# roitberg-group/lammps-ani

Hardware: AMD Instinct MI355X
Metric: MD ns/day for ANI-2x water box (0.5 fs steps; whole timestep loop: integrate + re-neighbour + ghost exchange + pair_style ani hot path) (higher is better)
Workload: dtype f32

## Files before the change

### include/ani_hip.h

```cpp
#ifndef ANI_HIP_H
#define ANI_HIP_H

#include <stdint.h>

#ifdef __cplusplus
extern "C" {
#endif

typedef struct ani_handle ani_handle;

#define ANI_HARTREE2KCALMOL 627.5094738898777

#define ANI_OK 0
#define ANI_ERR_ARG 1
#define ANI_ERR_MODEL 2
#define ANI_ERR_DEVICE 3
#define ANI_ERR_CAPACITY 4

int ani_create(const char* model_file, int local_rank, int use_num_models, int use_cuaev, int use_fullnbr,
               int use_single, ani_handle** out);

void ani_destroy(ani_handle* h);

const char* ani_last_error(const ani_handle* h);

int ani_num_models(const ani_handle* h);
int ani_use_num_models(const ani_handle* h);
int ani_num_species(const ani_handle* h);
int ani_aev_length(const ani_handle* h);
double ani_cutoff_radial(const ani_handle* h);
double ani_cutoff_angular(const ani_handle* h);

int ani_compute_full(ani_handle* h, int ntotal, int nlocal, const int64_t* species, const double* coordinates,
                     int64_t npairs, const int* ilist_unique, const int* jlist, const int* numneigh, int ago,
                     int eflag_atom, int vflag, double* out_energy, double* out_force, double* out_atomic_energies,
                     double* out_virial);

int ani_compute_half(ani_handle* h, int ntotal, int nlocal, const int64_t* species, const double* coordinates,
                     int64_t npairs_half, const int64_t* atom_index12, int ago, int eflag_atom, int vflag,
                     double* out_energy, double* out_force, double* out_atomic_energies, double* out_virial);

int ani_compute_full_device(ani_handle* h, int ntotal, int nlocal, const int* d_species, const double* d_x,
                            int64_t npairs, const int* d_ilist, const int* d_jlist, const int* d_numneigh, int ago,
                            int eflag_atom, int vflag, double* d_f, double* d_ev, double* d_eatom, void* stream);

int ani_request_atom_virial(ani_handle* h, double* out, int ncomp);

int ani_request_model_deviation(ani_handle* h, double* member_energy, double* atom_energy_dev, double* member_dforce,
                                double* atom_force_dev, double* summary);

int ani_set_ghost_fold(ani_handle* h, const int64_t* d_owner, const double* d_shift, int nghost, void* stream);
int ani_stage_ghost_fold(ani_handle* h, const int64_t* d_owner, const double* d_shift, int nghost);

int ani_step_begin(ani_handle* h, int ntotal, int nlocal, const double* d_x, int eflag_atom, int vflag, double* d_f, double* d_ev,
                   double* d_eatom, void* stream);
int ani_step_ghosts_ready(ani_handle* h, void* stream);
int ani_step_finish(ani_handle* h, void* stream);

int ani_build_list_device(ani_handle* h, int ntotal, int nlocal, const int* d_species, const double* d_x, double cutneigh,
                          const double* lo, const double* hi, int64_t* out_npairs, void* stream);

int ani_build_list(ani_handle* h, int ntotal, int nlocal, const int64_t* species, const double* coordinates, double cutneigh,
                   const double* lo, const double* hi, int64_t* out_npairs);
int ani_debug_list(ani_handle* h, const int** d_numneigh, const int** d_nbr_off, const int** d_jlist);

int ani_set_bond_table(ani_handle* h, const double* cut, int nspecies);
int ani_find_molecules_device(ani_handle* h, int ntotal, int nlocal, const double* d_x, const int64_t* d_owner, int* d_mol_of_atom,
                              int* d_formula, int formula_cap, int64_t* d_summary, void* stream);
int ani_find_molecules(ani_handle* h, int ntotal, int nlocal, const double* coordinates, const int64_t* owner, int* mol_of_atom,
                       int* formula, int formula_cap, int64_t* summary);
const char* ani_species_symbol(const ani_handle* h, int s);

int ani_rdf_configure(ani_handle* h, int nbins, double rmax, const int* pairs , int npair);
int ani_rdf_accumulate_device(ani_handle* h, int ntotal, int nlocal, const double* d_x, void* stream);
int ani_rdf_accumulate(ani_handle* h, int ntotal, int nlocal, const double* coordinates);
int ani_rdf_read(ani_handle* h, uint64_t* counts , uint64_t* centres , uint64_t* frames, int reset);

int ani_attach_comm(ani_handle* h, void* comm);

typedef struct {
  int nlocal, ntotal, nrows;
  int64_t npairs;
  const float* d_aev;
  const float* d_gaev;
  const int* d_row_of_centre;
  int species_count[16];
  int aev_stride;
  int aev_active_length;
  int error_flags;
} ani_debug_view;
int ani_host_register(const void* p, size_t bytes);
int ani_host_unregister(const void* p);

const char* ani_last_mlp_kernel(const ani_handle* h);
int ani_debug_get(ani_handle* h, ani_debug_view* out);
int ani_debug_colmap(ani_handle* h, int* out);
int ani_debug_deviation_parts(ani_handle* h, const void** d_parts, int64_t* member_stride);

int ani_set_option(ani_handle* h, const char* name, int value);
void ani_trace_push(const char* name);
void ani_trace_pop(void);
void ani_trace_mark(const char* name);

int ani_debug_fused_stamps(unsigned long long* out16, int reset);

int ani_debug_fused_schedule(int ntypes, const int* count, const double* cost, int bins, int* items_out, int* off_out,
                             double* makespan_out);
int ani_debug_fused_schedule_halves(int ntypes, const int* count, const double* cost, double half_ratio, int bins, int split_mode,
                                    int* split_out, int* items_out, int* off_out, int* n_items_out, double* makespan_out);

int ani_debug_read(ani_handle* h, const void* d_src, void* host_dst, uint64_t bytes);

int ani_phase_timing(ani_handle* h, int enable);
int ani_phase_times(ani_handle* h, double* ms5, int* ncalls);

#ifdef __cplusplus
}
#endif
#endif
```

### lammps-ani_amd/ani_hip.py

```python
from __future__ import annotations

import ctypes as C
import os
import subprocess

import numpy as np

_HERE = os.path.dirname(os.path.abspath(__file__))
_CSRC = os.path.join(_HERE, "csrc")
LIB_PATH = os.environ.get("ANI_HIP_LIB") or os.path.join(_CSRC, "libani_hip.so")
HARTREE2KCALMOL = 627.5094738898777

EXPORTS = ["ani_create", "ani_destroy", "ani_last_error", "ani_num_models", "ani_use_num_models", "ani_num_species",
           "ani_aev_length", "ani_cutoff_radial", "ani_cutoff_angular", "ani_compute_full", "ani_compute_half",
           "ani_compute_full_device", "ani_build_list_device", "ani_build_list", "ani_debug_list", "ani_debug_get", "ani_debug_read", "ani_debug_colmap", "ani_set_option", "ani_phase_timing", "ani_phase_times",
           "ani_trace_push", "ani_trace_pop", "ani_trace_mark", "ani_step_begin", "ani_step_ghosts_ready", "ani_step_finish",
           "ani_debug_fused_stamps", "ani_attach_comm", "ani_debug_fused_schedule", "ani_debug_fused_schedule_halves", "ani_last_mlp_kernel", "ani_host_register", "ani_host_unregister", "ani_set_ghost_fold", "ani_stage_ghost_fold",
           "ani_request_atom_virial", "ani_request_model_deviation", "ani_debug_deviation_parts",
           "ani_set_bond_table", "ani_find_molecules_device", "ani_find_molecules", "ani_species_symbol",
           "ani_rdf_configure", "ani_rdf_accumulate_device", "ani_rdf_accumulate", "ani_rdf_read"]
COMM_EXPORTS = ["ani_comm_get_unique_id", "ani_comm_create", "ani_comm_create_local", "ani_comm_destroy", "ani_comm_last_error", "ani_comm_rank",
                "ani_comm_size", "ani_comm_plan", "ani_comm_exchange_counts", "ani_comm_alltoallv", "ani_comm_set_epoch",
                "ani_comm_set_epoch_host", "ani_comm_set_ghost_order", "ani_comm_forward", "ani_comm_reverse", "ani_comm_reverse_send", "ani_comm_reverse_unpack",
                "ani_comm_allreduce_f64", "ani_comm_set_option", "ani_comm_get_stat"]


class AniError(RuntimeError):
    pass


class DebugView(C.Structure):
    _fields_ = [("nlocal", C.c_int), ("ntotal", C.c_int), ("nrows", C.c_int), ("npairs", C.c_int64),
                ("d_aev", C.c_void_p), ("d_gaev", C.c_void_p), ("d_row_of_centre", C.c_void_p),
                ("species_count", C.c_int * 16), ("aev_stride", C.c_int), ("aev_active_length", C.c_int), ("error_flags", C.c_int)]


class FireParams(C.Structure):
    _fields_ = [(n, C.c_double) for n in ("dt0", "dtmax", "dtmin", "dtgrow", "dtshrink", "alpha0", "alphashrink", "dmax", "etol",
                                          "ftol")] + [(n, C.c_int) for n in ("delaystep", "initialdelay", "halfstepback", "maxiter")]


FIRE_NSTATE = 16
FIRE_STATE_KEYS = ("iterations", "dt", "alpha", "last_negative", "e_prev", "e_cur", "P", "vv", "ff", "dtv", "uphill", "limited", "stop",
                   "e_first", "ff_first", "vmax")
FIRE_STOP_REASONS = ("running", "etol", "ftol", "maxiter", "non-finite")
SHAKE_NSTATS = 4
SHAKE_STATS_KEYS = ("unconverged", "max_iterations", "max_residual", "calls")
NH_NSTATE = 32
NH_MAXCHAIN = 8
NH_STATE_KEYS = ("half_steps", "k2", "s", "t_target", "ecouple", "tdof", "nonfinite")
THERMO_N = 16
THERMO_KEYS = ("pe", "ke", "temp", "press", "pxx", "pyy", "pzz", "pxy", "pxz", "pyz", "etotal", "ecouple", "econserve", "vol", "k2")


class NhParams(C.Structure):
    _fields_ = [("dt", C.c_double), ("t_period", C.c_double), ("drag", C.c_double), ("mtchain", C.c_int), ("nc_tchain", C.c_int)]


def nh_state_dict(rec, mtchain: int = NH_MAXCHAIN) -> dict:
    rec = np.asarray(rec, dtype=np.float64)
    out = dict(zip(NH_STATE_KEYS, rec[:7].tolist()))
    for k, name in enumerate(("eta", "eta_dot", "eta_dotdot")):
        out[name] = rec[8 + 8 * k: 8 + 8 * k + mtchain].copy()
    return out


NPT_NSTATE = 56
NPT_STATE_KEYS = ("half_steps", "omega_dot", "omega", "press", "p_target", "W", "fv", "mu")


class NptParams(C.Structure):
    _fields_ = [("dt", C.c_double), ("t_period", C.c_double), ("drag", C.c_double), ("p_period", C.c_double), ("mtchain", C.c_int),
                ("nc_tchain", C.c_int), ("mpchain", C.c_int), ("nc_pchain", C.c_int)]


def npt_state_dict(rec, mpchain: int = NH_MAXCHAIN) -> dict:
    rec = np.asarray(rec, dtype=np.float64)
    out = dict(zip(NPT_STATE_KEYS, rec[:8].tolist()))
    out.update(lo=rec[8:11].copy(), len=rec[11:14].copy(), ratio=rec[14:17].copy(), c=rec[17:20].copy(), v0=float(rec[20]),
               ecouple=float(rec[21]), nonfinite=float(rec[22]), natoms=float(rec[23]), ecouple_chain=float(rec[48]), vol=float(rec[49]))
    for k, name in enumerate(("eta", "eta_dot", "eta_dotdot")):
        out[name] = rec[24 + 8 * k: 24 + 8 * k + mpchain].copy()
    return out


RESTRAINT_NREC = 16
RESTRAINT_KINDS = {"distance": (0, 2), "angle": (1, 3), "torsion": (2, 4)}


def restraint_gather_table(atoms):
    atoms = np.asarray(atoms, dtype=np.int64).reshape(-1, 4)
    words = np.flatnonzero(atoms.reshape(-1) >= 0)
    owner = atoms.reshape(-1)[words]
    order = np.argsort(owner, kind="stable")
    touched, counts = np.unique(owner, return_counts=True)
    row_ptr = np.concatenate([[0], np.cumsum(counts)])
    return touched.astype(np.int32), row_ptr.astype(np.int32), words[order].astype(np.int32)


def restraint_state_dict(rec) -> dict:
    rec = np.asarray(rec, dtype=np.float64)
    return dict(evaluations=int(rec[0]), ebias=float(rec[1]), virial=rec[2:11].reshape(3, 3).copy(), nonfinite=int(rec[11]),
                max_delta=float(rec[12]), skipped=int(rec[13]))


def fire_params(dt0, etol, ftol, maxiter, **kw) -> FireParams:
    vals = dict(dt0=float(dt0), dtmax=10.0 * dt0, dtmin=0.02 * dt0, dtgrow=1.1, dtshrink=0.5, alpha0=0.25, alphashrink=0.99,
                dmax=0.1, etol=float(etol), ftol=float(ftol), delaystep=20, initialdelay=1, halfstepback=1, maxiter=int(maxiter))
    unknown = set(kw) - set(vals)
    if unknown:
        raise TypeError(f"unknown FIRE parameter(s): {sorted(unknown)}")
    vals.update(kw)
    p = FireParams()
    for name, ctype in FireParams._fields_:
        setattr(p, name, int(vals[name]) if ctype is C.c_int else float(vals[name]))
    return p


def build(force: bool = False) -> str:
    args = ["make", "-C", _CSRC, "-j8"]
    if force:
        args.append("-B")
    out = subprocess.run(args, check=True, stdout=subprocess.PIPE, stderr=subprocess.STDOUT, text=True).stdout
    build.last_commands = [ln for ln in out.splitlines() if ln.lstrip().startswith(("hipcc", "g++", "gcc"))]
    return LIB_PATH


build.last_commands = []


_lib = None


def lib():
    global _lib
    if _lib is None:
        if not os.path.exists(LIB_PATH):
            raise AniError(f"{LIB_PATH} is missing: build it (python -c 'import __graft_entry__ as g; g.build()'); "
                           "there is no fallback path")
        L = C.CDLL(LIB_PATH)
        L.ani_create.argtypes = [C.c_char_p, C.c_int, C.c_int, C.c_int, C.c_int, C.c_int, C.POINTER(C.c_void_p)]
        L.ani_destroy.argtypes = [C.c_void_p]
        L.ani_last_error.restype = C.c_char_p
        L.ani_last_error.argtypes = [C.c_void_p]
        for n in ("ani_num_models", "ani_use_num_models", "ani_num_species", "ani_aev_length"):
            getattr(L, n).argtypes = [C.c_void_p]
        for n in ("ani_cutoff_radial", "ani_cutoff_angular"):
            getattr(L, n).argtypes = [C.c_void_p]
            getattr(L, n).restype = C.c_double
        L.ani_compute_full.argtypes = [C.c_void_p, C.c_int, C.c_int, C.c_void_p, C.c_void_p, C.c_int64, C.c_void_p,
                                       C.c_void_p, C.c_void_p, C.c_int, C.c_int, C.c_int] + [C.c_void_p] * 4
        L.ani_compute_half.argtypes = [C.c_void_p, C.c_int, C.c_int, C.c_void_p, C.c_void_p, C.c_int64, C.c_void_p,
                                       C.c_int, C.c_int, C.c_int] + [C.c_void_p] * 4
        L.ani_compute_full_device.argtypes = [C.c_void_p, C.c_int, C.c_int, C.c_void_p, C.c_void_p, C.c_int64,
                                              C.c_void_p, C.c_void_p, C.c_void_p, C.c_int, C.c_int, C.c_int,
                                              C.c_void_p, C.c_void_p, C.c_void_p, C.c_void_p]
        L.ani_step_begin.argtypes = [C.c_void_p, C.c_int, C.c_int, C.c_void_p, C.c_int, C.c_int, C.c_void_p, C.c_void_p, C.c_void_p,
                                     C.c_void_p]
        L.ani_step_ghosts_ready.argtypes = [C.c_void_p, C.c_void_p]
        L.ani_step_finish.argtypes = [C.c_void_p, C.c_void_p]
        L.ani_build_list_device.argtypes = [C.c_void_p, C.c_int, C.c_int, C.c_void_p, C.c_void_p, C.c_double,
                                            C.c_void_p, C.c_void_p, C.POINTER(C.c_int64), C.c_void_p]
        L.ani_build_list.argtypes = [C.c_void_p, C.c_int, C.c_int, C.c_void_p, C.c_void_p, C.c_double, C.c_void_p,
                                     C.c_void_p, C.POINTER(C.c_int64)]
        L.ani_debug_list.argtypes = [C.c_void_p] + [C.POINTER(C.c_void_p)] * 3
        L.ani_debug_get.argtypes = [C.c_void_p, C.POINTER(DebugView)]
        L.ani_debug_read.argtypes = [C.c_void_p, C.c_void_p, C.c_void_p, C.c_uint64]
        L.ani_debug_colmap.argtypes = [C.c_void_p, C.c_void_p]
        L.ani_set_option.argtypes = [C.c_void_p, C.c_char_p, C.c_int]
        L.ani_last_mlp_kernel.argtypes = [C.c_void_p]
        L.ani_set_ghost_fold.argtypes = [C.c_void_p, C.c_void_p, C.c_void_p, C.c_int, C.c_void_p]
        L.ani_stage_ghost_fold.argtypes = [C.c_void_p, C.c_void_p, C.c_void_p, C.c_int]
        L.ani_request_atom_virial.argtypes = [C.c_void_p, C.c_void_p, C.c_int]
        L.ani_request_model_deviation.argtypes = [C.c_void_p] + [C.c_void_p] * 5
        L.ani_debug_deviation_parts.argtypes = [C.c_void_p, C.POINTER(C.c_void_p), C.POINTER(C.c_int64)]
        L.ani_set_bond_table.argtypes = [C.c_void_p, C.c_void_p, C.c_int]
        L.ani_find_molecules_device.argtypes = [C.c_void_p, C.c_int, C.c_int, C.c_void_p, C.c_void_p, C.c_void_p, C.c_void_p, C.c_int,
                                                C.c_void_p, C.c_void_p]
        L.ani_find_molecules.argtypes = [C.c_void_p, C.c_int, C.c_int, C.c_void_p, C.c_void_p, C.c_void_p, C.c_void_p, C.c_int,
                                         C.c_void_p]
        L.ani_species_symbol.argtypes = [C.c_void_p, C.c_int]
        L.ani_species_symbol.restype = C.c_char_p
        L.ani_rdf_configure.argtypes = [C.c_void_p, C.c_int, C.c_double, C.c_void_p, C.c_int]
        L.ani_rdf_accumulate_device.argtypes = [C.c_void_p, C.c_int, C.c_int, C.c_void_p, C.c_void_p]
        L.ani_rdf_accumulate.argtypes = [C.c_void_p, C.c_int, C.c_int, C.c_void_p]
        L.ani_rdf_read.argtypes = [C.c_void_p, C.c_void_p, C.c_void_p, C.c_void_p, C.c_int]
        L.ani_host_register.argtypes = [C.c_void_p, C.c_size_t]
        L.ani_host_unregister.argtypes = [C.c_void_p]
        L.ani_last_mlp_kernel.restype = C.c_char_p
        L.ani_md_initial_integrate.argtypes = [C.c_void_p, C.c_void_p, C.c_void_p, C.c_void_p, C.c_double, C.c_int, C.c_void_p,
                                               C.c_void_p, C.c_void_p]
        L.ani_md_final_integrate.argtypes = [C.c_void_p, C.c_void_p, C.c_void_p, C.c_int, C.c_int, C.c_void_p, C.c_void_p,
                                             C.c_void_p, C.c_uint64, C.c_uint64, C.c_void_p]
        L.ani_md_final_initial_integrate.argtypes = [C.c_void_p, C.c_void_p, C.c_void_p, C.c_void_p, C.c_double, C.c_int, C.c_int,
                                                     C.c_void_p, C.c_void_p, C.c_void_p, C.c_uint64, C.c_uint64, C.c_void_p,
                                                     C.c_void_p, C.c_void_p]
        L.ani_md_wrap_positions.argtypes = [C.c_void_p, C.c_int, C.c_void_p, C.c_void_p, C.c_int, C.c_void_p]
        L.ani_md_ghost_shell_count.argtypes = [C.c_void_p, C.c_int, C.c_void_p, C.c_void_p, C.c_int, C.c_void_p, C.c_void_p, C.c_void_p,
                                               C.c_void_p]
        L.ani_md_ghost_shell_fill.argtypes = [C.c_void_p, C.c_int, C.c_void_p, C.c_void_p, C.c_void_p, C.c_int, C.c_void_p, C.c_void_p,
                                              C.c_void_p, C.c_void_p]
        L.ani_md_append_ghosts.argtypes = [C.c_void_p, C.c_void_p, C.c_int, C.c_void_p, C.c_void_p, C.c_int, C.c_void_p]
        L.ani_md_check.argtypes = [C.c_void_p, C.c_void_p, C.c_void_p, C.c_void_p]
        L.ani_md_forward_ghosts.argtypes = [C.c_void_p, C.c_void_p, C.c_void_p, C.c_int, C.c_int, C.c_void_p]
        L.ani_md_reverse_ghosts.argtypes = [C.c_void_p, C.c_void_p, C.c_int, C.c_int, C.c_void_p]
        L.ani_md_reverse_ghosts_ordered.argtypes = [C.c_void_p, C.c_void_p, C.c_void_p, C.c_int, C.c_int, C.c_void_p]
        L.ani_md_pack_ghosts.argtypes = [C.c_void_p, C.c_void_p, C.c_void_p, C.c_int, C.c_void_p, C.c_void_p]
        L.ani_md_unpack_reverse.argtypes = [C.c_void_p, C.c_void_p, C.c_int, C.c_void_p, C.c_void_p]
        L.ani_md_fire_work_size.argtypes = [C.c_int]
        L.ani_md_fire_init.argtypes = [C.c_void_p, C.c_void_p, C.c_int, C.POINTER(FireParams), C.c_void_p]
        L.ani_md_fire_iterate.argtypes = [C.c_void_p, C.c_void_p, C.c_void_p, C.c_void_p, C.c_int, C.c_void_p, C.POINTER(FireParams),
                                          C.c_void_p, C.c_void_p, C.c_void_p, C.c_void_p, C.c_void_p]
        L.ani_md_fire_check.argtypes = [C.c_void_p, C.c_void_p, C.c_void_p, C.c_void_p, C.c_void_p]
        L.ani_md_shake_positions.argtypes = [C.c_void_p, C.c_void_p, C.c_void_p, C.c_void_p, C.c_int, C.c_void_p, C.c_double,
                                             C.c_double, C.c_int, C.c_void_p, C.c_int, C.c_void_p, C.c_void_p, C.c_void_p, C.c_void_p]
        L.ani_md_rattle_velocities.argtypes = [C.c_void_p, C.c_void_p, C.c_void_p, C.c_void_p, C.c_int, C.c_void_p, C.c_void_p,
                                               C.c_int, C.c_void_p]
        L.ani_md_nh_work_size.argtypes = [C.c_int]
        L.ani_md_nh_init.argtypes = [C.c_void_p, C.c_void_p]
        L.ani_md_nh_kinetic.argtypes = [C.c_void_p, C.c_void_p, C.c_int, C.c_void_p, C.c_void_p]
        L.ani_md_nh_chain.argtypes = [C.c_void_p, C.c_void_p, C.c_int, C.c_double, C.c_double, C.POINTER(NhParams), C.c_void_p]
        L.ani_md_nh_scale.argtypes = [C.c_void_p, C.c_int, C.c_void_p, C.c_void_p]
        L.ani_md_nh_initial_integrate.argtypes = [C.c_void_p, C.c_void_p, C.c_void_p, C.c_void_p, C.c_double, C.c_int, C.c_void_p,
                                                  C.c_void_p, C.c_void_p, C.c_void_p]
        L.ani_md_nh_final_integrate.argtypes = [C.c_void_p, C.c_void_p, C.c_void_p, C.c_void_p, C.c_int, C.c_void_p, C.c_void_p]
        L.ani_md_thermo_work_size.argtypes = [C.c_int]
        L.ani_md_thermo.argtypes = [C.c_void_p, C.c_void_p, C.c_int, C.c_void_p, C.c_int, C.c_double, C.c_double, C.c_void_p,
                                    C.c_void_p, C.c_void_p, C.c_void_p]
        L.ani_md_npt_init.argtypes = [C.c_void_p, C.c_void_p, C.c_void_p, C.c_int, C.c_void_p]
        L.ani_md_npt_chain.argtypes = [C.c_int, C.c_void_p, C.c_void_p, C.c_void_p, C.c_int, C.c_void_p, C.c_double, C.c_double,
                                       C.c_double, C.POINTER(NptParams), C.c_void_p]
        L.ani_md_npt_initial_integrate.argtypes = [C.c_void_p, C.c_void_p, C.c_void_p, C.c_void_p, C.c_double, C.c_int, C.c_void_p,
                                                   C.c_void_p, C.c_void_p, C.c_void_p, C.c_void_p, C.c_int, C.c_void_p]
        L.ani_md_npt_final_integrate.argtypes = [C.c_void_p, C.c_void_p, C.c_void_p, C.c_void_p, C.c_int, C.c_void_p, C.c_void_p,
                                                 C.c_void_p]
        L.ani_md_npt_check.argtypes = [C.c_void_p, C.c_void_p, C.c_void_p, C.c_void_p, C.c_void_p]
        L.ani_md_restraints_eval.argtypes = [C.c_void_p, C.c_int, C.c_void_p, C.c_void_p, C.c_void_p, C.c_void_p, C.c_int, C.c_void_p,
                                             C.c_void_p, C.c_int, C.c_void_p, C.c_void_p, C.c_void_p, C.c_void_p, C.c_void_p]
        L.ani_md_restraints_apply.argtypes = [C.c_void_p, C.c_int, C.c_void_p, C.c_int, C.c_void_p, C.c_void_p, C.c_void_p, C.c_int,
                                              C.c_void_p, C.c_void_p, C.c_void_p, C.c_void_p, C.c_void_p, C.c_void_p, C.c_int,
                                              C.c_void_p, C.c_double, C.c_void_p, C.c_void_p]
        L.ani_comm_get_unique_id.argtypes = [C.c_void_p]
        L.ani_comm_create.argtypes = [C.c_int, C.c_int, C.c_void_p, C.c_int, C.POINTER(C.c_void_p)]
        L.ani_comm_destroy.argtypes = [C.c_void_p]
        L.ani_comm_last_error.restype = C.c_char_p
        L.ani_comm_last_error.argtypes = [C.c_void_p]
        L.ani_comm_rank.argtypes = [C.c_void_p]
        L.ani_comm_size.argtypes = [C.c_void_p]
        L.ani_comm_plan.argtypes = [C.c_int] + [C.c_void_p] * 6
        L.ani_comm_exchange_counts.argtypes = [C.c_void_p] * 4
        L.ani_comm_alltoallv.argtypes = [C.c_void_p] * 5 + [C.c_int, C.c_void_p]
# ... 135 lines not shown
                                            f.ctypes.data, ea.ctypes.data, vir.ctypes.data)
        else:
            il = np.ascontiguousarray(inp.ilist, dtype=np.int32)
            nn = np.ascontiguousarray(inp.numneigh, dtype=np.int32)
            jl = np.ascontiguousarray(inp.jlist, dtype=np.int32)
            rc = self._lib.ani_compute_full(self._h, nt, nl, species.ctypes.data, x.ctypes.data, inp.npairs,
                                            il.ctypes.data, jl.ctypes.data, nn.ctypes.data, ago, int(eflag_atom),
                                            int(vflag), e.ctypes.data, f.ctypes.data, ea.ctypes.data, vir.ctypes.data)
        self._check(rc)
        out = dict(energy=float(e[0]), force=f, eatom=ea, virial=vir.reshape(3, 3))
        if av is not None:
            out["atom_virial"] = av
        if dv is not None:
            out["deviation"] = dv
        return out

    def compute_device(self, ntotal, nlocal, d_species, d_x, npairs, d_ilist, d_jlist, d_numneigh, ago, d_f, d_ev,
                       d_eatom=None, eflag_atom=False, vflag=False, stream=None, d_atom_virial=None, ncomp=9, d_deviation=None):
        if d_atom_virial is not None:
            self.request_atom_virial(d_atom_virial, ncomp)
        if d_deviation is not None:
            self.request_model_deviation(**d_deviation)
        rc = self._lib.ani_compute_full_device(self._h, ntotal, nlocal, d_species, d_x, npairs, d_ilist, d_jlist,
                                               d_numneigh, ago, int(eflag_atom), int(vflag), d_f, d_ev, d_eatom, stream)
        self._check(rc)

    def step_begin(self, ntotal, nlocal, d_x, d_f, d_ev, d_eatom=None, eflag_atom=False, vflag=False, stream=None,
                   d_atom_virial=None, ncomp=9):
        if d_atom_virial is not None:
            self.request_atom_virial(d_atom_virial, ncomp)
        self._check(self._lib.ani_step_begin(self._h, ntotal, nlocal, d_x, int(eflag_atom), int(vflag), d_f, d_ev, d_eatom, stream))

    def step_ghosts_ready(self, stream=None):
        self._check(self._lib.ani_step_ghosts_ready(self._h, stream))

    def step_finish(self, stream=None):
        self._check(self._lib.ani_step_finish(self._h, stream))

    def build_list_device(self, ntotal, nlocal, d_species, d_x, cutneigh, lo, hi, stream=None) -> int:
        lo = np.ascontiguousarray(lo, dtype=np.float64)
        hi = np.ascontiguousarray(hi, dtype=np.float64)
        n = C.c_int64()
        self._check(self._lib.ani_build_list_device(self._h, ntotal, nlocal, d_species, d_x, float(cutneigh),
                                                    lo.ctypes.data, hi.ctypes.data, C.byref(n), stream))
        return n.value

    def build_list(self, species, x, nlocal: int, cutneigh: float, lo=None, hi=None) -> int:
        species = np.ascontiguousarray(species, dtype=np.int64)
        x = np.ascontiguousarray(x, dtype=np.float64)
        if lo is None:
            lo = [x[:, k].min() - 0.25 for k in range(3)]
        if hi is None:
            hi = [x[:, k].max() + 0.25 for k in range(3)]
        lo = np.ascontiguousarray(lo, dtype=np.float64)
        hi = np.ascontiguousarray(hi, dtype=np.float64)
        n = C.c_int64()
        self._check(self._lib.ani_build_list(self._h, x.shape[0], nlocal, species.ctypes.data, x.ctypes.data, float(cutneigh),
                                             lo.ctypes.data, hi.ctypes.data, C.byref(n)))
        return n.value

    def debug_list(self, nlocal: int):
        pn, po, pj = C.c_void_p(), C.c_void_p(), C.c_void_p()
        self._check(self._lib.ani_debug_list(self._h, C.byref(pn), C.byref(po), C.byref(pj)))
        nn = self.debug_read(pn, (nlocal,), np.int32)
        if nlocal == 0:
            return nn, np.zeros(0, np.int32)
        off = self.debug_read(po, (nlocal + 1,), np.int32)
        span = self.debug_read(pj, (int((off[:-1] + nn).max()),), np.int32)
        if np.array_equal(off[1:] - off[:-1], nn):
            return nn, span[: int(nn.sum())]
        idx = np.repeat(off[:-1] - np.concatenate([[0], np.cumsum(nn)[:-1]]), nn) + np.arange(int(nn.sum()))
        return nn, span[idx]

    def debug_view(self) -> DebugView:
        v = DebugView()
        self._check(self._lib.ani_debug_get(self._h, C.byref(v)))
        return v

    def debug_read(self, d_ptr, shape, dtype) -> np.ndarray:
        out = np.empty(shape, dtype=dtype)
        self._check(self._lib.ani_debug_read(self._h, d_ptr, out.ctypes.data, out.nbytes))
        return out

    def colmap(self) -> np.ndarray:
        v = self.debug_view()
        out = np.zeros(v.aev_active_length, dtype=np.int32)
        self._check(self._lib.ani_debug_colmap(self._h, out.ctypes.data))
        return out

    def set_option(self, name: str, value: int):
        self._check(self._lib.ani_set_option(self._h, name.encode(), int(value)))

    def set_ghost_fold(self, d_owner, d_shift, nghost: int, stream=None):
        self._check(self._lib.ani_set_ghost_fold(self._h, d_owner, d_shift, int(nghost), stream))

    def stage_ghost_fold(self, d_owner, d_shift, nghost: int):
        self._check(self._lib.ani_stage_ghost_fold(self._h, d_owner, d_shift, int(nghost)))

    def species_symbols(self):
        return [self._lib.ani_species_symbol(self._h, s).decode() for s in range(self._lib.ani_num_species(self._h))]

    def set_bond_table(self, table):
        if table is None:
            self._check(self._lib.ani_set_bond_table(self._h, None, 0))
            return
        if isinstance(table, dict):
            sym = self.species_symbols()
            t = np.zeros((len(sym), len(sym)))
            for (a, b), v in table.items():
                if a not in sym or b not in sym:
                    raise AniError(f"set_bond_table: the model has no species {a if a not in sym else b!r} (it has {sym})")
                t[sym.index(a), sym.index(b)] = t[sym.index(b), sym.index(a)] = float(v)
            table = t
        t = np.ascontiguousarray(table, dtype=np.float64)
        if t.ndim != 2 or t.shape[0] != t.shape[1]:
            raise AniError(f"set_bond_table: a square table is needed, got shape {t.shape}")
        self._check(self._lib.ani_set_bond_table(self._h, t.ctypes.data, int(t.shape[0])))

    def find_molecules(self, inp_or_x, owner=None, formula_cap: int = 4096, nlocal=None):
        if hasattr(inp_or_x, "nlocal"):
            x, nl = inp_or_x.x, inp_or_x.nlocal
        else:
            x = inp_or_x
            nl = len(x) if nlocal is None else int(nlocal)
        x = np.ascontiguousarray(x, dtype=np.float64)
        nt = x.shape[0]
        S = self._lib.ani_num_species(self._h)
        own = None
        if owner is not None:
            own = np.ascontiguousarray(owner, dtype=np.int64)
            assert own.shape == (nt - nl,)
        mol = np.full(nl, -1, dtype=np.int32)
        rows = np.zeros((int(formula_cap), S + 1), dtype=np.int32)
        summ = np.zeros(6, dtype=np.int64)
        self._check(self._lib.ani_find_molecules(self._h, nt, nl, x.ctypes.data, own.ctypes.data if own is not None else None,
                                                 mol.ctypes.data, rows.ctypes.data, int(formula_cap), summ.ctypes.data))
        return mol, formula_dict(rows[: int(summ[1])], self.species_symbols()), summ

    def find_molecules_device(self, ntotal, nlocal, d_x, d_owner=None, d_mol_of_atom=None, d_formula=None, formula_cap: int = 0,
                              d_summary=None, stream=None):
        self._check(self._lib.ani_find_molecules_device(self._h, int(ntotal), int(nlocal), d_x, d_owner, d_mol_of_atom, d_formula,
                                                        int(formula_cap), d_summary, stream))

    def rdf_configure(self, nbins: int, rmax: float, pairs):
        if pairs is None or len(pairs) == 0:
            self._check(self._lib.ani_rdf_configure(self._h, int(nbins), float(rmax), None, 0))
            self._rdf = None
            return
        sym = None
        idx = []
        for pr in pairs:
            a, b = pr
            for v in (a, b):
                if isinstance(v, str):
                    sym = sym or self.species_symbols()
                    if v not in sym:
                        raise AniError(f"rdf_configure: the model has no species {v!r} (it has {sym})")
                    v = sym.index(v)
                idx.append(int(v))
        p = np.ascontiguousarray(idx, dtype=np.int32).reshape(-1, 2)
        self._check(self._lib.ani_rdf_configure(self._h, int(nbins), float(rmax), p.ctypes.data, int(p.shape[0])))
        self._rdf = (int(nbins), float(rmax), p)

    def rdf_config(self):
        return getattr(self, "_rdf", None)

# ... 162 lines not shown
```

### lammps-ani_amd/csrc/ani_handle.h

```cpp
#pragma once
#include "../../include/ani_hip.h"
#include "../../include/ani_comm.h"

#include <hip/hip_runtime.h>
#ifndef ANI_NO_ROCTX
#include <rocprofiler-sdk-roctx/roctx.h>
#else
static inline void roctxRangePushA(const char*) {}
static inline void roctxRangePop() {}
static inline void roctxMarkA(const char*) {}
#endif

#include <algorithm>
#include <atomic>
#include <chrono>
#include <cmath>
#include <cstdio>
#include <cstdlib>
#include <cstring>
#include <string>
#include <vector>

#include "ani_kernels.h"
#include "ani_model.h"

namespace ani_host __attribute__((visibility("hidden"))) {
using namespace ani;

inline int round_up(int v, int m) { return (v + m - 1) / m * m; }

template <typename T>
struct DevBuf {
  T* p = nullptr;
  size_t cap = 0;
  hipError_t reserve(size_t n, bool zero = false) {
    if (n <= cap && p) return hipSuccess;
    if (p) (void)hipFree(p);
    p = nullptr;
    size_t want = std::max<size_t>(n + n / 2, 64);
    hipError_t e = hipMalloc((void**)&p, want * sizeof(T));
    if (e != hipSuccess) { cap = 0; return e; }
    cap = want;
    if (zero) {
      e = hipMemset(p, 0, want * sizeof(T));
      if (e == hipSuccess) e = hipStreamSynchronize(nullptr);
    }
    return e;
  }
  void release() { if (p) (void)hipFree(p); p = nullptr; cap = 0; }
};

struct TraceRange {
  explicit TraceRange(const char* name) { roctxRangePushA(name); }
  ~TraceRange() { roctxRangePop(); }
  TraceRange(const TraceRange&) = delete;
  TraceRange& operator=(const TraceRange&) = delete;
};

struct SpeciesNet {
  std::vector<float*> W;
  std::vector<float*> b;
  std::vector<float*> WT;
  float* W0c = nullptr;
  float* WT0c = nullptr;
  float* w_out = nullptr;
  float* b_out = nullptr;
  std::vector<int> w;
  std::vector<double*> W64, b64, WT64;
  double *W0c64 = nullptr, *WT0c64 = nullptr, *w_out64 = nullptr, *b_out64 = nullptr;
  struct Planes {
    std::vector<unsigned short*> W, WT;
    unsigned short *W0c = nullptr, *WT0c = nullptr;
  } sp[2];
  std::vector<float> wscale;
  struct Fused {
    unsigned char* stream = nullptr;
    float* consts = nullptr;
    long long ppm = 0;
    int cpm = 0;
  } fu[4];
  int fused_shape = -1;
};
inline MlpArith planes_arith(int i) { return i == 0 ? MLP_BF16X3 : MLP_F16X2; }

struct Options {
  int prune = 1;
  int mlp_pipeline = 0;
  int aev_fused = 1;
  int aev_sym_radial = 1;
  int aev_tickets_min = 40000;
  int mlp_fused_sched = 1;
  int mlp_fused_halves = 1;
  int mlp_fused = 1;
  int mlp_fused_gen = 1;
  int mlp_fused_rows = 0;
  int mlp_chain = 1;
  int profiling = 0;
  int dev_overwrite = 0;
  int mlp_arith = MLP_BF16X3;
  int rdf_lanes = 16, rdf_lds = 1;
  int nbr_onepass = 1, nbr_sorted_rows = 1, nbr_half_cells = 0;
  int reuse_upload = 0;
  int out_force_accumulate = 0;
};

struct FusedState {
  int mask[4] = {-2, -2, -2, -2};
  DevBuf<int> counter;
  DevBuf<int> sched;
  int sched_key[4] = {-1, -1, -1, -1};
  int sched_nitems = 0;
  DevBuf<float> gaev_parts;
};

struct DevOut { double *member_energy, *atom_energy_dev, *member_dforce, *atom_force_dev, *summary; };

struct Armed {
  double* av_out = nullptr;
  int av_ncomp = 0;
  void* av_acc = nullptr;
  double* split_av = nullptr;
  int split_av_ncomp = 0;
  DevBuf<float> avir;
  DevBuf<double> avir64;
  DevBuf<double> avout;
  DevOut dv_req{}, dv{};
  bool dv_on = false, dv_force = false, dv_dsq = false, dv_fold = false;
  DevBuf<double> gaev_parts64;
  DevBuf<float> dv_fbuf;
  DevBuf<double> dv_fbuf64;
  DevBuf<double> dv_tmp;
  DevBuf<double> dv_stage;
  DevBuf<double> dv_part;
  DevBuf<unsigned> dv_ticket;
};

struct MolFinder {
  bool have_bonds = false;
  DevBuf<double> bond_cut2;
  DevBuf<int> ints;
  DevBuf<unsigned long long> words;
  DevBuf<long long> owner, summary;
  DevBuf<int> out;
};

struct Rdf {
  int npair = 0, nbins = 0;
  double rmax = 0.0;
  DevBuf<int> ints;
  DevBuf<unsigned long long> words;
};

struct NbrBuild {
  int cap_hint = 0;
  DevBuf<int> ovf;
  DevBuf<float4> xq;
  DevBuf<int> cell_id, cell_count, cell_start, cursor, order;
  DevBuf<double> xs;
};

struct HostStaging {
  std::vector<int> species32;
  double* pinned_ev = nullptr;
  int* pinned_ints = nullptr;
  double* stage_force = nullptr;
  size_t stage_force_cap = 0;
  static constexpr int kForceChunks = 16;
  unsigned* stage_flags = nullptr;
  DevBuf<unsigned long long> copy_ctr;
  unsigned copy_epoch = 0;
  unsigned long long step = 0;
  const double* x64_from = nullptr;
  std::vector<int> half_num, half_j;
};

struct PhaseTiming {
  bool on = false;
  std::vector<hipEvent_t> evt_pool;
  size_t evt_used = 0;
  hipEvent_t* evt = nullptr;
  double phase_ms[5] = {0, 0, 0, 0, 0};
  int phase_calls = 0;
};

}

using namespace ani;
using namespace ani_host;

struct ani_handle {
  HostModel model;
  AevParams ap{};
  AevParams ap_run{};
  SpeciesMap cmap{};
  int active_mask = -1;
  Options opt;
  FusedState fused;
  Armed armed;
  MolFinder mol;
  Rdf rdf;
  NbrBuild nb;
  HostStaging host;
  PhaseTiming timing;
  const char* last_mlp_kernel = "";
  ChainPlan chain_plan;
  std::vector<int> colmap;
  int device = 0;
  bool use_cuaev = true, use_fullnbr = true, use_single = true;
  hipStream_t stream = nullptr;
  std::string err;
  std::vector<SpeciesNet> nets;

  bool have_list = false;
  DevBuf<int> row_flag, row_list, row_count;
  int n_boundary = 0;
  bool classes_valid = false;
  int split_phase = 0;
  hipStream_t side = nullptr;
  hipEvent_t ev_mlp = nullptr, ev_side = nullptr;
  struct { const double* d_x; int eflag_atom, vflag; double *d_f, *d_ev, *d_eatom; } split{};
  int nlocal = 0, ntotal = 0, nrows = 0;
  long long npairs = 0;
  int count[kMaxSpecies] = {0}, row_start[kMaxSpecies] = {0};

  ani_comm* comm = nullptr;
  int sticky_flags = 0;
  int max_numneigh = 0;
  DevBuf<int> species, ilist, numneigh, jlist, jraw, nbr_off, row_of_centre, centre_of_row, bucket_info, err_flag;
  DevBuf<int> row_of_atom;
  DevBuf<unsigned> sym_acc;
  int jraw_stride = 0;
  int jlist_row_stride = 0;
  const int64_t* stage_owner = nullptr;
  const double* stage_shift = nullptr;
  int stage_nghost = -1;
  bool origin_from_box = false;
  GhostFold fold;
  int fold_nghost = -1;
  DevBuf<int> fold_head, fold_next, fold_bad;
  bool warned_asymmetric = false;
  bool list_is_ours = false;
  bool list_symmetric = true;
  DevBuf<int> row_ctr;
  DevBuf<float4> xyzs, cl_xyz;
  DevBuf<int4> row_info, cl_hdr;
  DevBuf<int> cl_j;
  int cl_stride = 0;
  DevBuf<double> x64, f64, ev, eatom, virial_acc;
  DevBuf<double> origin;
  bool need_origin = true;
  DevBuf<double> rep_tables, erep;
  DevBuf<float> aev, gaev, act, e_rows, fbuf;
  DevBuf<double> aev64, gaev64, act64, e_rows64, fbuf64;
  std::vector<std::vector<double*>> Hbuf64;
  std::vector<std::vector<float*>> Hbuf, Gbuf;
  bool arena_valid = false;
};

#define HIP_TRY(h, expr)                                                                              \
  do {                                                                                                \
    hipError_t _e = (expr);                                                                           \
    if (_e != hipSuccess) {                                                                           \
      (h)->err = std::string(#expr) + ": " + hipGetErrorString(_e);                                   \
      return ANI_ERR_DEVICE;                                                                          \
    }                                                                                                 \
  } while (0)

namespace ani_host __attribute__((visibility("hidden"))) {
int check_args(ani_handle* h, int ntotal, int nlocal, long long npairs, int ago);
int upload_model(ani_handle* h);
int specialize(ani_handle* h, int mask);
int compute_mlp(ani_handle* h, hipStream_t st);
void free_fused(ani_handle* h, int fi);
const int* forced_fused_split(const char* env, int ntypes, const int* count, int* split);
int rebuild(ani_handle* h, hipStream_t st);
int ingest_list(ani_handle* h, int ntotal, int nlocal, long long npairs, const int* species, const int* ilist, const int* numneigh,
                const int* jlist, hipMemcpyKind kind, hipStream_t st);
int ensure_row_classes(ani_handle* h, hipStream_t st);
struct DevStage {
  DevOut dev{};
  size_t off[5] = {0, 0, 0, 0, 0}, len[5] = {0, 0, 0, 0, 0};
};
double* take_atom_virial(ani_handle* h, int* ncomp);
int atom_virial_begin(ani_handle* h, bool armed);
void atom_virial_out(ani_handle* h, double* d_out, int ncomp, int accumulate, bool fold, hipStream_t st);
bool dv_any(const DevOut& d);
DevOut take_deviation(ani_handle* h);
int deviation_check(ani_handle* h, const DevOut& d, int ntotal, int nlocal, bool device, bool fold);
int deviation_begin(ani_handle* h, const DevOut& d, bool fold);
void deviation_end(ani_handle* h);
int deviation_stage(ani_handle* h, const DevOut& d, int ntotal, int nlocal, DevStage* sg);
int deviation_copy_home(ani_handle* h, const DevOut& d, const DevStage& sg, hipStream_t st);

template <typename Pass>
int deviation_run(ani_handle* h, Pass&& pass, hipStream_t st) {
  const HostModel& m = h->model;
  const int M = m.M, nl = h->nlocal;
  const bool fp64 = !h->use_single;
  double* dsq = h->armed.dv_dsq ? h->armed.dv_tmp.p : nullptr;
  double* sig = h->armed.dv.summary ? h->armed.dv_tmp.p + (size_t)nl : nullptr;
  double* dd = h->armed.dv.summary ? h->armed.dv_tmp.p + 2 * (size_t)nl : nullptr;
  if (h->armed.dv_force) {
    const long long per = (long long)std::max(h->nrows, 1) * h->ap_run.aev_stride;
    void* acc = fp64 ? static_cast<void*>(h->armed.dv_fbuf64.p) : static_cast<void*>(h->armed.dv_fbuf.p);
    HIP_TRY(h, hipMemsetAsync(acc, 0, (fp64 ? 3 * sizeof(double) : 4 * sizeof(float)) * (size_t)h->ntotal, st));
    const bool fold = h->armed.dv_fold;
    for (int a = 0; a < M; a++) {
      pass(a, per, acc);
      launch_dev_member(acc, fp64, fold ? nl : h->ntotal, nl, a, M, h->armed.dv.member_dforce, dsq, fold ? h->fold_head.p : nullptr,
                        fold ? h->fold_next.p : nullptr, nl, st);
    }
  }
  DevCloseArgs ca{};
  ca.e_rows = fp64 ? static_cast<const void*>(h->e_rows64.p) : static_cast<const void*>(h->e_rows.p);
  ca.M = M; ca.nrows = h->nrows; ca.nrows_ld = h->nrows; ca.nlocal = nl;
  ca.centre_of_row = h->centre_of_row.p; ca.ilist = h->ilist.p; ca.species = h->species.p;
  for (int s = 0; s < m.S; s++) ca.sae[s] = m.sae[s];
  ca.erep = m.has_rep ? h->erep.p : nullptr; ca.nslots = kVirialSlots;
  ca.dsq = dsq;
  ca.member_energy = h->armed.dv.member_energy; ca.atom_energy_dev = h->armed.dv.atom_energy_dev;
  ca.atom_force_dev = dsq ? h->armed.dv.atom_force_dev : nullptr;
  ca.sig = sig; ca.dd = dd;
  ca.partials = h->armed.dv_part.p; ca.ticket = h->armed.dv_ticket.p;
  launch_dev_close(ca, fp64, st);
  if (h->armed.dv.summary) launch_dev_summary(dd, sig, nl, h->armed.dv.summary, st);
  return ANI_OK;
}

template <typename T>
bool wait_host_word(const volatile T* w, T want) {
  const auto t0 = std::chrono::steady_clock::now();
  for (;;) {
    for (int k = 0; k < 512; k++) {
      if (*w == want) {
        std::atomic_thread_fence(std::memory_order_acquire);
        return true;
      }
      __builtin_ia32_pause();
    }
    if (std::chrono::steady_clock::now() - t0 > std::chrono::seconds(5)) return false;
  }
}
}
```

### lammps-ani_amd/csrc/ani_hip.cpp

```cpp
#include "ani_handle.h"

namespace ani {
static thread_local hipError_t g_launch_error = hipSuccess;
void note_launch_error(hipError_t e) { if (e != hipSuccess && g_launch_error == hipSuccess) g_launch_error = e; }
hipError_t take_launch_error() { const hipError_t e = g_launch_error; g_launch_error = hipSuccess; return e; }
}

namespace ani_host __attribute__((visibility("hidden"))) {
thread_local std::string g_create_error;
constexpr int kCopyOutBlocks = 32;

int run_step64(ani_handle* h, const double* d_x, int eflag_atom, int vflag, double* d_f, int f_accumulate, double* d_ev,
               double* d_eatom, hipStream_t st) {
  const HostModel& m = h->model;
  const int L = m.L, M = m.M;
  HIP_TRY(h, h->fbuf64.reserve((size_t)std::max(h->ntotal, 1) * 3));
  HIP_TRY(h, h->virial_acc.reserve(9 * kVirialSlots));
  HIP_TRY(h, h->err_flag.reserve(1, true));
  HIP_TRY(h, hipMemsetAsync(h->fbuf64.p, 0, sizeof(double) * 3 * (size_t)h->ntotal, st));
  HIP_TRY(h, hipMemsetAsync(h->virial_acc.p, 0, sizeof(double) * 9, st));
  HIP_TRY(h, hipMemsetAsync(h->e_rows64.p, 0, sizeof(double) * (size_t)M * std::max(h->nrows, 1), st));
  if (h->armed.av_acc) HIP_TRY(h, hipMemsetAsync(h->armed.av_acc, 0, sizeof(double) * 9 * (size_t)h->ntotal, st));
  Aev64Params p{};
  const AevParams& r = h->ap_run;
// ... 77 lines not shown
    launch_repulsion(ra, true, st, h->armed.av_acc);
  }
  Sae64 sae{};
  for (int s = 0; s < m.S; s++) sae.v[s] = m.sae[s];
  launch_finish64(h->e_rows64.p, M, h->nrows, h->centre_of_row.p, h->ilist.p, h->species.p, sae, h->fbuf64.p, h->ntotal,
                  vflag ? h->virial_acc.p : nullptr, d_f, f_accumulate, d_ev, eflag_atom ? d_eatom : nullptr, h->err_flag.p, st);
  if (m.has_rep) launch_repulsion_energy(h->erep.p, kVirialSlots, d_ev, st);
  if (h->armed.dv_on) {
    Aev64Args ad = a;
    ad.virial = nullptr;
    const int rcd = deviation_run(h, [&](int b, long long stride, void* acc) {
      ad.gaev = h->armed.gaev_parts64.p + b * stride; ad.fbuf = static_cast<double*>(acc);
      launch_aev64_backward(p, ad, st);
    }, st);
    if (rcd) return rcd;
  }
  HIP_TRY(h, hipGetLastError());
  HIP_TRY(h, take_launch_error());
  return ANI_OK;
}

struct StepCtx {
  const double* d_x = nullptr;
  int eflag_atom = 0, vflag = 0, f_accumulate = 0;
  double *d_f = nullptr, *d_ev = nullptr, *d_eatom = nullptr;
  bool fold = false;
};

int step_prologue(ani_handle* h, const StepCtx& c, bool timed, hipStream_t st) {
  if (h->ntotal >= (1 << 28)) {
    h->err = "more than 2^28 atoms (owned + ghost) on one rank";
    return ANI_ERR_ARG;
  }
  HIP_TRY(h, h->xyzs.reserve(h->ntotal));
  HIP_TRY(h, h->fbuf.reserve((size_t)h->ntotal * 4));
  HIP_TRY(h, h->virial_acc.reserve(9 * kVirialSlots));
  HIP_TRY(h, h->err_flag.reserve(1, true));
  HIP_TRY(h, h->row_ctr.reserve((size_t)3 * kTicketMaxGroups * kTicketStride, true));
  h->timing.evt = nullptr;
  if (timed && h->timing.on) {
    if (h->timing.evt_used + 6 > h->timing.evt_pool.size()) {
      const size_t old = h->timing.evt_pool.size();
      h->timing.evt_pool.resize(old + 6 * 64, nullptr);
      for (size_t i = old; i < h->timing.evt_pool.size(); i++) HIP_TRY(h, hipEventCreate(&h->timing.evt_pool[i]));
    }
    h->timing.evt = &h->timing.evt_pool[h->timing.evt_used];
    h->timing.evt_used += 6;
  }
  if (h->timing.evt) HIP_TRY(h, hipEventRecord(h->timing.evt[0], st));
  HIP_TRY(h, h->origin.reserve(3));
  if (h->need_origin) {
    launch_origin(c.d_x, h->ntotal, h->origin.p, st);
    h->need_origin = false;
  }
  if (h->model.has_rep) {
    HIP_TRY(h, h->erep.reserve(kVirialSlots));
    HIP_TRY(h, hipMemsetAsync(h->erep.p, 0, sizeof(double) * kVirialSlots, st));
  }
  return ANI_OK;
}

void step_pack(ani_handle* h, const StepCtx& c, int i0, int i1, bool first, hipStream_t st) {
  const bool fold = h->fold_nghost >= 0 && c.fold;
  launch_pack(c.d_x, h->species.p, i0, i1, h->cmap, h->xyzs.p, h->fbuf.p, first ? h->virial_acc.p : nullptr,
              first ? c.d_ev : nullptr, h->origin.p, st, fold ? &h->fold : nullptr);
}

AevArgs step_aev_args(ani_handle* h, const StepCtx& c, int rows) {
  AevArgs a{};
  a.xyzs = h->xyzs.p; a.ilist = h->ilist.p; a.numneigh = h->numneigh.p; a.nbr_off = h->nbr_off.p; a.jlist = h->jlist.p;
  a.centre_of_row = h->centre_of_row.p; a.row_info = h->row_info.p; a.nrows = h->nrows; a.aev = h->aev.p; a.gaev = h->gaev.p; a.fbuf = h->fbuf.p;
  a.virial = c.vflag ? h->virial_acc.p : nullptr;
  a.err_flag = h->err_flag.p;
  a.cl_hdr = h->cl_hdr.p; a.cl_xyz = h->cl_xyz.p; a.cl_j = h->cl_j.p; a.cl_stride = h->cl_stride;
  a.row_list = nullptr; a.k0 = 0; a.kcount = h->nrows;
  a.row_counter = h->row_ctr.p ? h->row_ctr.p + rows * kTicketMaxGroups * kTicketStride : nullptr;
  if (rows == 1) { a.row_list = h->row_list.p; a.k0 = 0; a.kcount = h->n_boundary; }
  if (rows == 2) { a.row_list = h->row_list.p; a.k0 = h->n_boundary; a.kcount = h->nrows - h->n_boundary; }
  if (a.kcount < h->opt.aev_tickets_min) a.row_counter = nullptr;
  a.row_of_atom = (rows == 0 && h->opt.aev_sym_radial && h->list_symmetric) ? h->row_of_atom.p : nullptr;
  return a;
}

int step_compact_forward(ani_handle* h, const AevArgs& a, hipStream_t st) {
  if (h->opt.aev_fused) {
    TraceRange tr("ani: neighbour compaction + AEV forward");
    if (h->timing.evt) HIP_TRY(h, hipEventRecord(h->timing.evt[5], st));
    if (launch_aev_forward_fused(h->ap_run, a, h->max_numneigh, st)) {
      if (h->timing.evt) HIP_TRY(h, hipEventRecord(h->timing.evt[1], st));
      return ANI_OK;
    }
  }
  {
    TraceRange tr("ani: neighbour compaction");
    launch_nbr_compact(h->ap_run, a, h->max_numneigh, st);
  }
  if (h->timing.evt) HIP_TRY(h, hipEventRecord(h->timing.evt[5], st));
  {
    TraceRange tr("ani: AEV forward");
    launch_aev_forward(h->ap_run, a, h->max_numneigh, st);
  }
  if (h->timing.evt) HIP_TRY(h, hipEventRecord(h->timing.evt[1], st));
  return ANI_OK;
}

int step_backward(ani_handle* h, const StepCtx& c, const AevArgs& a, hipStream_t st) {
  const HostModel& m = h->model;
  RepTab rt{};
  if (m.has_rep && h->ap_run.S <= 8) {
    rt.on = 1; rt.cutoff = (float)m.rep_cut; rt.erep = h->erep.p; rt.x64 = c.d_x;
    std::vector<int> act;
    for (int s = 0; s < m.S; s++) if (h->active_mask & (1 << s)) act.push_back(s);
    if ((int)act.size() != h->ap_run.S) { act.clear(); for (int s = 0; s < m.S; s++) act.push_back(s); }
    const size_t n2 = (size_t)m.S * m.S;
    for (size_t ca = 0; ca < act.size(); ca++)
      for (size_t cb = 0; cb < act.size(); cb++) {
        const size_t src = (size_t)act[ca] * m.S + act[cb];
        rt.y[8 * ca + cb] = (float)m.rep_tables[src];
        rt.sa[8 * ca + cb] = (float)m.rep_tables[n2 + src];
        rt.k[8 * ca + cb] = (float)m.rep_tables[2 * n2 + src];
      }
  }
  float* avir = static_cast<float*>(h->armed.av_acc);
  const bool rep_done = launch_aev_backward(h->ap_run, a, h->max_numneigh, st, rt.on ? &rt : nullptr, avir) && rt.on;
  if (m.has_rep && !rep_done) {
    RepArgs ra{};
    ra.row_info = h->row_info.p; ra.nrows = h->nrows; ra.jlist = h->jlist.p; ra.species = h->species.p;
    ra.pos = c.d_x; ra.fbuf = h->fbuf.p; ra.virial = c.vflag ? h->virial_acc.p : nullptr; ra.erep = h->erep.p;
    ra.tables = h->rep_tables.p; ra.S = m.S; ra.nslots = kVirialSlots; ra.vslots = kVirialSlots; ra.cutoff = m.rep_cut;
    launch_repulsion(ra, false, st, avir);
  }
  return ANI_OK;
}

void step_finish(ani_handle* h, const StepCtx& c, int atom0, int atom1, bool energy, hipStream_t st) {
  const HostModel& m = h->model;
  FinishArgs fa{};
  fa.e_rows = h->e_rows.p; fa.M = m.M; fa.nrows = h->nrows; fa.nrows_ld = h->nrows;
  fa.centre_of_row = h->centre_of_row.p; fa.ilist = h->ilist.p; fa.species = h->species.p;
  for (int s = 0; s < m.S; s++) fa.sae[s] = m.sae[s];
  fa.fbuf = h->fbuf.p; fa.atom0 = atom0; fa.atom1 = atom1; fa.energy = energy ? 1 : 0;
  fa.virial_acc = c.vflag ? h->virial_acc.p : nullptr;
  fa.f_out = c.d_f; fa.f_accumulate = c.f_accumulate; fa.ev_out = c.d_ev;
  fa.eatom_out = c.eflag_atom ? c.d_eatom : nullptr;
  fa.err_flag = h->err_flag.p;
  if (h->fold_nghost >= 0 && c.fold) {
    fa.fold_head = h->fold_head.p; fa.fold_next = h->fold_next.p; fa.fold_nlocal = h->nlocal;
    fa.atom1 = std::min(fa.atom1, h->nlocal);
  }
  launch_finish(fa, st);
  if (energy && m.has_rep) launch_repulsion_energy(h->erep.p, kVirialSlots, c.d_ev, st);
}

int run_step(ani_handle* h, const double* d_x, int eflag_atom, int vflag, double* d_f, int f_accumulate, double* d_ev,
             double* d_eatom, hipStream_t st, bool fold = false) {
  if (!h->use_single) return run_step64(h, d_x, eflag_atom, vflag, d_f, f_accumulate, d_ev, d_eatom, st);
  StepCtx c;
  c.fold = fold;
  c.d_x = d_x; c.eflag_atom = eflag_atom; c.vflag = vflag; c.f_accumulate = f_accumulate; c.d_f = d_f; c.d_ev = d_ev; c.d_eatom = d_eatom;
  TraceRange tr_step("ani: step");
  int rc = step_prologue(h, c, true, st);
  if (rc) return rc;
  step_pack(h, c, 0, h->ntotal, true, st);
  if (h->armed.av_acc) HIP_TRY(h, hipMemsetAsync(h->armed.av_acc, 0, sizeof(float) * 9 * (size_t)h->ntotal, st));
  const AevArgs a = step_aev_args(h, c, 0);
  rc = step_compact_forward(h, a, st);
  if (rc) return rc;
  {
    TraceRange tr("ani: MLP forward + backward");
    rc = compute_mlp(h, st);
    if (rc) return rc;
  }
  if (h->timing.evt) HIP_TRY(h, hipEventRecord(h->timing.evt[2], st));
  TraceRange tr_bwd("ani: AEV backward + finish");
  rc = step_backward(h, c, a, st);
  if (rc) return rc;
  if (h->timing.evt) HIP_TRY(h, hipEventRecord(h->timing.evt[3], st));
  step_finish(h, c, 0, h->ntotal, true, st);
  if (h->timing.evt) HIP_TRY(h, hipEventRecord(h->timing.evt[4], st));
  if (h->armed.dv_on) {
    AevArgs ad = a;
    ad.virial = nullptr;
    rc = deviation_run(h, [&](int b, long long stride, void* acc) {
      ad.gaev = h->fused.gaev_parts.p + b * stride; ad.fbuf = static_cast<float*>(acc);
      launch_aev_backward(h->ap_run, ad, h->max_numneigh, st);
    }, st);
    if (rc) return rc;
  }
  HIP_TRY(h, hipGetLastError());
  HIP_TRY(h, take_launch_error());
  return ANI_OK;
}

bool split_supported(const ani_handle* h) { return h->use_single && h->cl_stride > 0 && !(h->model.has_rep && h->ap_run.S > 8); }

int check_args(ani_handle* h, int ntotal, int nlocal, long long npairs, int ago) {
  if (!h) return ANI_ERR_ARG;
  if (ntotal < 0 || nlocal < 0 || nlocal > ntotal || npairs < 0) { h->err = "inconsistent ntotal/nlocal/npairs"; return ANI_ERR_ARG; }
  if (npairs >= (1LL << 31)) { h->err = "more than 2^31 neighbour pairs per rank is not supported"; return ANI_ERR_ARG; }
  if (ago != 0 && (!h->have_list || ntotal != h->ntotal || nlocal != h->nlocal)) {
    h->err = "ago != 0 but no neighbour list of matching size is cached (the first call, and every call after a rebuild, must pass ago = 0)";
    return ANI_ERR_ARG;
  }
  return ANI_OK;
}

int finish_host(ani_handle* h, int ntotal, int nlocal, int eflag_atom, int vflag, double* out_energy, double* out_force,
// ... 85 lines not shown

extern "C" {
int ani_create(const char* model_file, int local_rank, int use_num_models, int use_cuaev, int use_fullnbr, int use_single,
               ani_handle** out) {
  if (out) *out = nullptr;
  if (!model_file || !out) { g_create_error = "null argument"; return ANI_ERR_ARG; }
  if (local_rank < 0) {
    g_create_error = "device 'cpu' (local_rank = -1) is not available: libani_hip is the HIP/gfx950 path only and has no host fallback";
    return ANI_ERR_ARG;
  }
  int ndev = 0;
  if (hipGetDeviceCount(&ndev) != hipSuccess || ndev <= 0) { g_create_error = "no HIP device visible"; return ANI_ERR_DEVICE; }
  ani_handle* h = new ani_handle;
  h->device = local_rank % ndev;
  h->use_cuaev = use_cuaev != 0; h->use_fullnbr = use_fullnbr != 0; h->use_single = use_single != 0;
  std::string e = load_model(model_file, use_num_models, h->model);
  if (!e.empty()) { g_create_error = e; delete h; return ANI_ERR_MODEL; }
  if (hipSetDevice(h->device) != hipSuccess || hipStreamCreateWithFlags(&h->stream, hipStreamNonBlocking) != hipSuccess) {
    g_create_error = "cannot initialise HIP device " + std::to_string(h->device);
    delete h;
    return ANI_ERR_DEVICE;
  }
  if (const char* tf = getenv("LAMMPS_ANI_ALLOW_TF32")) {
    if (tf[0] && strcmp(tf, "0") != 0) h->opt.mlp_arith = MLP_F16X2;
  }
  if (const char* e = getenv("ANI_AEV_FUSED")) h->opt.aev_fused = atoi(e) != 0;
  if (const char* e = getenv("ANI_AEV_TICKETS_MIN")) h->opt.aev_tickets_min = atoi(e);
  int rc = upload_model(h);
  if (rc != ANI_OK) { g_create_error = h->err; ani_destroy(h); return rc; }
  printf("Successfully loaded the model \nfile: '%s' \ndevice: hip:%d \ndtype: %s \nnbrlist: %s \nani_aev: %s \nuse_num_models: %d/%d\n\n",
         model_file, h->device, h->use_single ? "float (FP32)" : "double (FP64)", h->use_fullnbr ? "full" : "half", h->use_cuaev ? "cuaev" : "pyaev", h->model.M, h->model.M_file);
  fflush(stdout);
  *out = h;
  return ANI_OK;
}

void ani_destroy(ani_handle* h) {
  if (!h) return;
  (void)hipSetDevice(h->device);
  if (h->stream) (void)hipStreamSynchronize(h->stream);
  if (h->host.pinned_ints) { (void)hipHostFree(h->host.pinned_ints); h->host.pinned_ints = nullptr; }
  if (h->host.stage_force) { (void)hipHostFree(h->host.stage_force); h->host.stage_force = nullptr; }
  if (h->host.pinned_ev) { (void)hipHostFree(h->host.pinned_ev); h->host.pinned_ev = nullptr; }
  if (h->host.stage_flags) { (void)hipHostFree(h->host.stage_flags); h->host.stage_flags = nullptr; }
  h->host.copy_ctr.release();
  if (h->side) { (void)hipStreamSynchronize(h->side); (void)hipStreamDestroy(h->side); }
  if (h->ev_mlp) (void)hipEventDestroy(h->ev_mlp);
  if (h->ev_side) (void)hipEventDestroy(h->ev_side);
  for (auto& n : h->nets) {
    for (float* p : n.W) if (p) (void)hipFree(p);
    for (float* p : n.b) if (p) (void)hipFree(p);
    for (float* p : n.WT) if (p) (void)hipFree(p);
    if (n.W0c) (void)hipFree(n.W0c);
    if (n.WT0c) (void)hipFree(n.WT0c);
    if (n.w_out) (void)hipFree(n.w_out);
    if (n.b_out) (void)hipFree(n.b_out);
    for (auto& sp : n.sp) {
      for (unsigned short* p : sp.W) if (p) (void)hipFree(p);
      for (unsigned short* p : sp.WT) if (p) (void)hipFree(p);
      if (sp.W0c) (void)hipFree(sp.W0c);
      if (sp.WT0c) (void)hipFree(sp.WT0c);
    }
    for (double* p : n.W64) if (p) (void)hipFree(p);
    for (double* p : n.b64) if (p) (void)hipFree(p);
    for (double* p : n.WT64) if (p) (void)hipFree(p);
    if (n.W0c64) (void)hipFree(n.W0c64);
    if (n.WT0c64) (void)hipFree(n.WT0c64);
    if (n.w_out64) (void)hipFree(n.w_out64);
    if (n.b_out64) (void)hipFree(n.b_out64);
  }
  h->species.release(); h->ilist.release(); h->numneigh.release(); h->jlist.release(); h->jraw.release(); h->nbr_off.release();
  h->fold_head.release(); h->fold_next.release(); h->fold_bad.release(); h->nb.ovf.release(); h->nb.xq.release(); h->row_of_centre.release(); h->centre_of_row.release(); h->bucket_info.release(); h->err_flag.release(); h->row_ctr.release(); h->row_of_atom.release();
  h->xyzs.release(); h->cl_xyz.release(); h->cl_hdr.release(); h->cl_j.release(); h->row_info.release(); h->row_flag.release(); h->row_list.release(); h->row_count.release(); h->x64.release(); h->f64.release(); h->ev.release(); h->eatom.release(); h->origin.release();
  h->rep_tables.release(); h->erep.release();
  h->nb.cell_id.release(); h->nb.cell_count.release(); h->nb.cell_start.release(); h->nb.cursor.release(); h->nb.order.release(); h->nb.xs.release();
  h->armed.avir.release(); h->armed.avir64.release(); h->armed.avout.release();
  h->armed.gaev_parts64.release(); h->armed.dv_fbuf.release(); h->armed.dv_fbuf64.release(); h->armed.dv_tmp.release(); h->armed.dv_stage.release();
  h->armed.dv_part.release(); h->armed.dv_ticket.release();
  h->mol.bond_cut2.release(); h->mol.ints.release(); h->mol.words.release(); h->mol.owner.release(); h->mol.summary.release(); h->mol.out.release();
  h->rdf.ints.release(); h->rdf.words.release();
  h->virial_acc.release(); h->aev.release(); h->gaev.release(); h->act.release(); h->aev64.release(); h->gaev64.release(); h->act64.release(); h->e_rows64.release(); h->fbuf64.release(); h->e_rows.release(); h->fbuf.release();
  for (int fi = 0; fi < 4; fi++) free_fused(h, fi);
  h->fused.counter.release(); h->fused.gaev_parts.release(); h->fused.sched.release();
  free_chain_plan(h->chain_plan);
  for (auto& e : h->timing.evt_pool) if (e) (void)hipEventDestroy(e);
  if (h->stream) (void)hipStreamDestroy(h->stream);
  delete h;
}

const char* ani_last_error(const ani_handle* h) { return h ? h->err.c_str() : g_create_error.c_str(); }
int ani_num_models(const ani_handle* h) { return h ? h->model.M_file : 0; }
int ani_use_num_models(const ani_handle* h) { return h ? h->model.M : 0; }
int ani_num_species(const ani_handle* h) { return h ? h->model.S : 0; }
int ani_aev_length(const ani_handle* h) { return h ? h->model.aev_len : 0; }
double ani_cutoff_radial(const ani_handle* h) { return h ? h->model.Rcr : 0; }
double ani_cutoff_angular(const ani_handle* h) { return h ? h->model.Rca : 0; }
const char* ani_species_symbol(const ani_handle* h, int s) {
  return h && s >= 0 && s < h->model.S ? h->model.symbols[s].c_str() : "";
}

int ani_compute_full_device(ani_handle* h, int ntotal, int nlocal, const int* d_species, const double* d_x, int64_t npairs,
                            const int* d_ilist, const int* d_jlist, const int* d_numneigh, int ago, int eflag_atom, int vflag,
                            double* d_f, double* d_ev, double* d_eatom, void* stream) {
  int av_ncomp = 0;
  double* const av_out = take_atom_virial(h, &av_ncomp);
  const DevOut dv = take_deviation(h);
  int rc = check_args(h, ntotal, nlocal, npairs, ago);
  if (rc) return rc;
  if (!d_x || !d_ev) { h->err = "null device pointer"; return ANI_ERR_ARG; }
  {
    const bool fold = ago == 0 ? (h->stage_nghost >= 0 && h->stage_owner && h->stage_nghost == ntotal - nlocal) : h->fold_nghost >= 0;
    rc = deviation_check(h, dv, ntotal, nlocal, true, fold);
    if (rc) return rc;
  }
  HIP_TRY(h, hipSetDevice(h->device));
  hipStream_t st = (hipStream_t)stream;
  if (ago == 0) {
    if (!d_species || !d_ilist || !d_jlist || !d_numneigh) { h->err = "null list pointer with ago == 0"; return ANI_ERR_ARG; }
    h->ap.full_cap = h->ap_run.full_cap = 1;
    rc = ingest_list(h, ntotal, nlocal, npairs, d_species, d_ilist, d_numneigh, d_jlist, hipMemcpyDeviceToDevice, st);
    if (rc) return rc;
  }
  const ArmedScope armed_scope{h};
  rc = atom_virial_begin(h, av_out != nullptr);
  if (!rc) rc = deviation_begin(h, dv, true);
  if (rc) return rc;
  rc = run_step(h, d_x, eflag_atom, vflag, d_f, h->opt.dev_overwrite ? 0 : 1, d_ev, d_eatom, st, true);
  if (rc == ANI_OK && av_out) atom_virial_out(h, av_out, av_ncomp, h->opt.dev_overwrite ? 0 : 1, true, st);
  if (rc == ANI_OK && h->opt.profiling) HIP_TRY(h, hipStreamSynchronize(st));
  return rc;
}

static StepCtx split_ctx(const ani_handle* h) {
  StepCtx c;
  c.d_x = h->split.d_x; c.eflag_atom = h->split.eflag_atom; c.vflag = h->split.vflag; c.f_accumulate = h->opt.dev_overwrite ? 0 : 1;
  c.d_f = h->split.d_f; c.d_ev = h->split.d_ev; c.d_eatom = h->split.d_eatom;
  return c;
}

int ani_step_begin(ani_handle* h, int ntotal, int nlocal, const double* d_x, int eflag_atom, int vflag, double* d_f, double* d_ev,
                   double* d_eatom, void* stream) {
  int av_ncomp = 0;
  double* const av_out = take_atom_virial(h, &av_ncomp);
  if (dv_any(take_deviation(h))) {
    h->err = "ani_request_model_deviation: the split step (ani_step_begin) cannot return a model deviation; use a whole-step entry";
    return ANI_ERR_ARG;
  }
  int rc = check_args(h, ntotal, nlocal, 0, 1);
  if (rc) return rc;
  if (!d_x || !d_ev) { h->err = "null device pointer"; return ANI_ERR_ARG; }
  if (h->split_phase != 0) { h->err = "ani_step_begin: the previous split step was not finished"; return ANI_ERR_ARG; }
  HIP_TRY(h, hipSetDevice(h->device));
  hipStream_t st = (hipStream_t)stream;
  h->split.d_x = d_x; h->split.eflag_atom = eflag_atom; h->split.vflag = vflag; h->split.d_f = d_f; h->split.d_ev = d_ev; h->split.d_eatom = d_eatom;
  rc = atom_virial_begin(h, av_out != nullptr);
  if (rc) return rc;
  h->armed.split_av = av_out;
  h->armed.split_av_ncomp = av_ncomp;
  h->split_phase = 1;
  if (!split_supported(h)) return ANI_OK;
  rc = ensure_row_classes(h, st);
  if (rc) { h->split_phase = 0; return rc; }
  const StepCtx c = split_ctx(h);
  TraceRange tr("ani: step, rows without ghosts: pack + compaction + AEV forward");
  rc = step_prologue(h, c, false, st);
  if (rc) { h->split_phase = 0; return rc; }
// ... 191 lines not shown
```

### lammps-ani_amd/csrc/ani_hip_list.cpp

```cpp
#include "ani_handle.h"

namespace ani_host __attribute__((visibility("hidden"))) {
constexpr int kRebuildRowsOverflow = -1000;
int rebuild(ani_handle* h, hipStream_t st) {
  const HostModel& m = h->model;
  roctxMarkA("neighbor list rebuilt");
  TraceRange tr("ani: list epoch set-up (offsets, species buckets, segment sort)");
  h->need_origin = !h->origin_from_box;
  h->fold_nghost = -1;
  h->classes_valid = false;
  h->split_phase = 0;
  const int nlocal = h->nlocal;
  const int nrows_cap = round_up(nlocal, kRowTile) + m.S * kRowTile;
  HIP_TRY(h, h->nbr_off.reserve((size_t)nlocal + 1));
  HIP_TRY(h, h->row_of_centre.reserve(prepare_scratch_ints(nlocal)));
  HIP_TRY(h, h->centre_of_row.reserve(nrows_cap));
  HIP_TRY(h, h->row_info.reserve(nrows_cap));
  HIP_TRY(h, h->bucket_info.reserve(kBucketInfoInts));
  HIP_TRY(h, h->err_flag.reserve(1, true));
  if (!h->host.pinned_ints) HIP_TRY(h, hipHostMalloc((void**)&h->host.pinned_ints, sizeof(int) * 32, hipHostMallocDefault));
  h->host.pinned_ints[0] = h->host.pinned_ints[1] = h->host.pinned_ints[2] = 0;
  HIP_TRY(h, hipMemcpyAsync(&h->host.pinned_ints[0], h->err_flag.p, sizeof(int), hipMemcpyDeviceToHost, st));
  HIP_TRY(h, hipMemsetAsync(h->err_flag.p, 0, sizeof(int), st));
  HIP_TRY(h, h->row_of_atom.reserve((size_t)std::max(h->ntotal, 1)));
  PrepOut o{h->nbr_off.p, h->row_of_centre.p, h->centre_of_row.p, h->row_info.p, h->bucket_info.p, h->row_of_atom.p};
  launch_prepare(h->species.p, h->ilist.p, h->numneigh.p, nlocal, h->ntotal, m.S, nrows_cap, o, st, h->jlist_row_stride);
  if (h->jlist_row_stride) HIP_TRY(h, hipMemcpyAsync(&h->host.pinned_ints[1], h->nb.ovf.p, sizeof(int), hipMemcpyDeviceToHost, st));
  const bool fold_staged = h->stage_nghost >= 0 && h->stage_owner && h->use_single && h->stage_nghost == h->ntotal - nlocal;
  if (fold_staged) {
    HIP_TRY(h, h->fold_head.reserve((size_t)std::max(nlocal, 1)));
    HIP_TRY(h, h->fold_next.reserve((size_t)std::max(h->stage_nghost, 1)));
    HIP_TRY(h, h->fold_bad.reserve(1));
    launch_ghost_chain(reinterpret_cast<const long long*>(h->stage_owner), h->stage_nghost, nlocal, h->fold_head.p, h->fold_next.p, h->fold_bad.p, st);
    HIP_TRY(h, hipMemcpyAsync(&h->host.pinned_ints[2], h->fold_bad.p, sizeof(int), hipMemcpyDeviceToHost, st));
  }
  int info[kBucketInfoInts];
  HIP_TRY(h, hipMemcpyAsync(info, h->bucket_info.p, sizeof(info), hipMemcpyDeviceToHost, st));
  HIP_TRY(h, hipStreamSynchronize(st));
  h->sticky_flags |= h->host.pinned_ints[0];
  HIP_TRY(h, take_launch_error());
  if (h->jlist_row_stride && h->host.pinned_ints[1]) return kRebuildRowsOverflow;
  if (h->jlist_row_stride) h->npairs = info[2 * kMaxSpecies + 4];
  if (fold_staged) {
    if (h->host.pinned_ints[2]) { h->stage_nghost = -1; h->err = "ani_stage_ghost_fold: an owner index lies outside [0, nlocal)"; return ANI_ERR_ARG; }
    h->fold.owner = reinterpret_cast<const long long*>(h->stage_owner); h->fold.shift = h->stage_shift; h->fold.nlocal = nlocal;
    h->fold_nghost = h->stage_nghost;
  }
  h->stage_nghost = -1;
  if (info[2 * kMaxSpecies + 1]) { h->err = "an atom has a species outside the model's species list (or ilist holds an index outside [0, ntotal))"; return ANI_ERR_ARG; }
  for (int s = 0; s < m.S; s++) { h->count[s] = info[s]; h->row_start[s] = info[kMaxSpecies + s]; }
  h->nrows = info[2 * kMaxSpecies];
  h->max_numneigh = info[2 * kMaxSpecies + 2];
  {
    const int rcs = specialize(h, info[2 * kMaxSpecies + 3]);
    if (rcs) return rcs;
  }
  h->list_symmetric = true;
  if (!h->list_is_ours && h->use_single && h->opt.aev_sym_radial && nlocal > 0) {
    HIP_TRY(h, h->sym_acc.reserve((size_t)std::max(h->ntotal, 1)));
    launch_list_symmetry(h->ilist.p, h->nbr_off.p, h->numneigh.p, h->jraw.p, h->row_of_atom.p, nlocal, h->ntotal, h->sym_acc.p,
                         h->bucket_info.p, st);
    int bad = 0;
    HIP_TRY(h, hipMemcpyAsync(&bad, h->bucket_info.p, sizeof(int), hipMemcpyDeviceToHost, st));
    HIP_TRY(h, hipStreamSynchronize(st));
    HIP_TRY(h, take_launch_error());
    if (bad) {
      h->list_symmetric = false;
      h->sticky_flags |= 8;
      if (!h->warned_asymmetric) {
        h->warned_asymmetric = true;
        fprintf(stderr, "libani_hip: the neighbour list is not symmetric between owned atoms (j in i's list without i in j's): "
                        "aev_symmetric_radial is off for such epochs, every radial term is scattered\n");
      }
    }
  }
  if (!h->jlist_row_stride) launch_sort_jlist(h->species.p, h->nbr_off.p, h->numneigh.p, h->jraw.p, h->jlist.p, nlocal, m.S, info[2 * kMaxSpecies + 3], st, h->jraw_stride);

  const size_t stride = h->ap_run.aev_stride;
  if (!h->use_single) {
    HIP_TRY(h, h->aev64.reserve((size_t)std::max(h->nrows, 1) * stride));
    HIP_TRY(h, h->gaev64.reserve((size_t)std::max(h->nrows, 1) * stride));
    HIP_TRY(h, hipMemsetAsync(h->aev64.p, 0, (size_t)h->nrows * stride * sizeof(double), st));
    HIP_TRY(h, h->e_rows64.reserve((size_t)m.M * std::max(h->nrows, 1)));
    size_t need64 = 0;
    for (int s = 0; s < m.S; s++)
      for (int k = 1; k < m.L; k++) need64 += (size_t)round_up(h->count[s], kRowTile) * m.M * h->nets[s].w[k];
    HIP_TRY(h, h->act64.reserve(std::max<size_t>(need64, 1)));
    HIP_TRY(h, hipMemsetAsync(h->act64.p, 0, need64 * sizeof(double), st));
    h->Hbuf64.assign(m.S, std::vector<double*>(m.L, nullptr));
    size_t off64 = 0;
    for (int s = 0; s < m.S; s++)
      for (int k = 1; k < m.L; k++) {
        h->Hbuf64[s][k] = h->act64.p + off64;
        off64 += (size_t)round_up(h->count[s], kRowTile) * m.M * h->nets[s].w[k];
      }
    return ANI_OK;
  }
  HIP_TRY(h, h->aev.reserve((size_t)std::max(h->nrows, 1) * stride));
  HIP_TRY(h, h->gaev.reserve((size_t)std::max(h->nrows, 1) * stride));
  HIP_TRY(h, hipMemsetAsync(h->aev.p, 0, (size_t)h->nrows * stride * sizeof(float), st));
  HIP_TRY(h, h->e_rows.reserve((size_t)m.M * std::max(h->nrows, 1)));
  h->cl_stride = aev_compact_stride(h->ap_run, h->max_numneigh);
  if (h->cl_stride > 0) {
    HIP_TRY(h, h->cl_hdr.reserve((size_t)2 * std::max(h->nrows, 1)));
    HIP_TRY(h, h->cl_xyz.reserve((size_t)std::max(h->nrows, 1) * h->cl_stride));
    HIP_TRY(h, h->cl_j.reserve((size_t)std::max(h->nrows, 1) * h->cl_stride));
  }

  h->arena_valid = false;
  return ANI_OK;
}

int ingest_list(ani_handle* h, int ntotal, int nlocal, long long npairs, const int* species, const int* ilist, const int* numneigh,
                const int* jlist, hipMemcpyKind kind, hipStream_t st) {
  h->ntotal = ntotal; h->nlocal = nlocal; h->npairs = npairs;
  HIP_TRY(h, h->species.reserve(ntotal));
  HIP_TRY(h, h->ilist.reserve(nlocal));
  HIP_TRY(h, h->numneigh.reserve(nlocal));
  HIP_TRY(h, h->jlist.reserve(npairs));
  HIP_TRY(h, h->jraw.reserve(npairs));
  HIP_TRY(h, hipMemcpyAsync(h->species.p, species, sizeof(int) * (size_t)ntotal, kind, st));
  HIP_TRY(h, hipMemcpyAsync(h->ilist.p, ilist, sizeof(int) * (size_t)nlocal, kind, st));
  HIP_TRY(h, hipMemcpyAsync(h->numneigh.p, numneigh, sizeof(int) * (size_t)nlocal, kind, st));
  HIP_TRY(h, hipMemcpyAsync(h->jraw.p, jlist, sizeof(int) * (size_t)npairs, kind, st));
  h->have_list = false;
  h->list_is_ours = false;
  h->jraw_stride = h->jlist_row_stride = 0;
  h->origin_from_box = false;
  const int rc = rebuild(h, st);
  if (rc) return rc;
  h->have_list = true;
  return ANI_OK;
}

int ensure_row_classes(ani_handle* h, hipStream_t st) {
  if (h->classes_valid) return ANI_OK;
  HIP_TRY(h, h->row_flag.reserve(std::max(h->nrows, 1)));
  HIP_TRY(h, h->row_list.reserve(std::max(h->nrows, 1)));
// ... 179 lines not shown
```

### lammps-ani_amd/csrc/ani_hip_model.cpp

```cpp
#include "ani_handle.h"

namespace ani_host __attribute__((visibility("hidden"))) {
int upload(ani_handle* h, float** dst, const std::vector<float>& src) {
  HIP_TRY(h, hipMalloc((void**)dst, std::max<size_t>(src.size(), 1) * sizeof(float)));
  HIP_TRY(h, hipMemcpy(*dst, src.data(), src.size() * sizeof(float), hipMemcpyHostToDevice));
  return ANI_OK;
}

int mirror64(ani_handle* h, double** dst, const float* src, size_t n) {
  if (h->use_single) return ANI_OK;
  if (*dst) (void)hipFree(*dst);
  HIP_TRY(h, hipMalloc((void**)dst, std::max<size_t>(n, 1) * sizeof(double)));
  launch_cvt_f32_f64(src, *dst, n, h->stream);
  HIP_TRY(h, hipStreamSynchronize(h->stream));
  return ANI_OK;
}

int make_split(ani_handle* h, unsigned short** dst3, unsigned short** dst2, const float* src, int batch, long long s_src, int N, int K,
               int ld, float wscale) {
  unsigned short** dst[2] = {dst3, dst2};
  for (int i = 0; i < 2; i++) {
    const MlpArith ar = planes_arith(i);
    const size_t elems = split_elems(N, K, ar) * (size_t)batch;
    HIP_TRY(h, hipMalloc((void**)dst[i], std::max<size_t>(elems, 1) * sizeof(unsigned short)));
// ... 91 lines not shown
  {
    const double dR = m.nR > 1 ? (m.ShfR[m.nR - 1] - m.ShfR[0]) / (m.nR - 1) : 0.0;
    const double dA = m.nA > 1 ? (m.ShfA[m.nA - 1] - m.ShfA[0]) / (m.nA - 1) : 0.0;
    bool equi = true;
    for (int k = 0; k < m.nR; k++) equi = equi && std::fabs(m.ShfR[0] + k * dR - m.ShfR[k]) < 1e-9;
    for (int k = 0; k < m.nA; k++) equi = equi && std::fabs(m.ShfA[0] + k * dA - m.ShfA[k]) < 1e-9;
    p.ShfR0 = (float)m.ShfR[0]; p.dShfR = (float)dR; p.ShfA0 = (float)m.ShfA[0]; p.dShfA = (float)dA;
    p.equi = equi ? 1 : 0;
  }
  if (aev_stride > 1024) { h->err = "AEV longer than 1024 is not supported"; return ANI_ERR_MODEL; }
  return ANI_OK;
}

int specialize(ani_handle* h, int mask) {
  const HostModel& m = h->model;
  if (!h->opt.prune) mask = (1 << m.S) - 1;
  if (mask == h->active_mask) return ANI_OK;
  for (auto& n : h->nets) {
    if (n.W0c) (void)hipFree(n.W0c);
    if (n.WT0c) (void)hipFree(n.WT0c);
    if (n.W0c64) (void)hipFree(n.W0c64);
    if (n.WT0c64) (void)hipFree(n.WT0c64);
    for (auto& sp : n.sp) {
      if (sp.W0c) (void)hipFree(sp.W0c);
      if (sp.WT0c) (void)hipFree(sp.WT0c);
      sp.W0c = sp.WT0c = nullptr;
    }
    n.W0c = n.WT0c = nullptr;
    n.W0c64 = n.WT0c64 = nullptr;
  }
  std::vector<int> act;
  for (int s = 0; s < m.S; s++) {
    h->cmap.m[s] = (int)act.size();
    if (mask & (1 << s)) act.push_back(s);
  }
  for (int s = m.S; s < kMaxSpecies; s++) h->cmap.m[s] = 0;
  const int na = (int)act.size();
  h->ap_run = h->ap;
  h->colmap.resize(m.aev_len);
  for (int c = 0; c < m.aev_len; c++) h->colmap[c] = c;
  h->active_mask = mask;
  if (na == m.S || na == 0) {
    for (int s = 0; s < m.S; s++) h->cmap.m[s] = s;
    return ANI_OK;
  }
  const int nAZ = m.nA * m.nZ;
  const int alen = na * m.nR + na * (na + 1) / 2 * nAZ;
  const int astride = round_up(alen, 4);
  AevParams& p = h->ap_run;
  p.S = na; p.radial_len = na * m.nR; p.aev_len = alen; p.aev_stride = astride;
  h->colmap.assign(alen, 0);
  for (int cs = 0; cs < na; cs++)
    for (int k = 0; k < m.nR; k++) h->colmap[cs * m.nR + k] = act[cs] * m.nR + k;
  {
    int b = 0;
    for (int c1 = 0; c1 < na; c1++)
      for (int c2 = c1; c2 < na; c2++, b++) {
        const int lo = act[c1], hi = act[c2];
        const int dense_b = lo * m.S - lo * (lo - 1) / 2 + (hi - lo);
        for (int t = 0; t < nAZ; t++) h->colmap[na * m.nR + b * nAZ + t] = m.radial_len + dense_b * nAZ + t;
      }
  }
  const int M = m.M;
  for (int s = 0; s < m.S; s++) {
    SpeciesNet& n = h->nets[s];
    const int out = m.dims[s][1], in = m.dims[s][0], w1 = n.w[1];
    std::vector<float> W((size_t)M * out * astride, 0.f), T((size_t)alen * M * w1, 0.f);
    for (int a = 0; a < M; a++)
      for (int o = 0; o < out; o++)
        for (int c = 0; c < alen; c++) {
          const float v = m.W[a][s][0][(size_t)o * in + h->colmap[c]];
          W[((size_t)a * out + o) * astride + c] = v;
          T[(size_t)c * M * w1 + (size_t)a * w1 + o] = v;
        }
    int rc = upload(h, &n.W0c, W); if (rc) return rc;
    rc = upload(h, &n.WT0c, T); if (rc) return rc;
    rc = mirror64(h, &n.W0c64, n.W0c, W.size()); if (rc) return rc;
    rc = mirror64(h, &n.WT0c64, n.WT0c, T.size()); if (rc) return rc;
    rc = make_split(h, &n.sp[0].W0c, &n.sp[1].W0c, n.W0c, M, (long long)out * astride, out, astride, astride, n.wscale[0]); if (rc) return rc;
    rc = make_split(h, &n.sp[0].WT0c, &n.sp[1].WT0c, n.WT0c, 1, 0, alen, M * w1, M * w1, n.wscale[0]); if (rc) return rc;
  }
  return ANI_OK;
}
}
```

### lammps-ani_amd/csrc/ani_hip_options.cpp

```cpp
#include "ani_handle.h"

extern "C" {
void ani_trace_push(const char* name) { if (name) roctxRangePushA(name); }
void ani_trace_pop(void) { roctxRangePop(); }
void ani_trace_mark(const char* name) { if (name) roctxMarkA(name); }

const char* ani_last_mlp_kernel(const ani_handle* h) { return h ? h->last_mlp_kernel : ""; }

int ani_debug_get(ani_handle* h, ani_debug_view* out) {
  if (!h || !out) return ANI_ERR_ARG;
  memset(out, 0, sizeof(*out));
  out->nlocal = h->nlocal; out->ntotal = h->ntotal; out->nrows = h->nrows; out->npairs = h->npairs;
  out->d_aev = h->aev.p; out->d_gaev = h->gaev.p; out->d_row_of_centre = h->row_of_centre.p;
  out->aev_stride = h->ap_run.aev_stride; out->aev_active_length = h->ap_run.aev_len;
  if (h->err_flag.p) {
    int flag = 0;
    if (hipSetDevice(h->device) == hipSuccess && hipDeviceSynchronize() == hipSuccess &&
        hipMemcpy(&flag, h->err_flag.p, sizeof(int), hipMemcpyDeviceToHost) == hipSuccess)
      h->sticky_flags |= flag;
  }
  out->error_flags = h->sticky_flags;
  for (int s = 0; s < kMaxSpecies && s < 16; s++) out->species_count[s] = h->count[s];
  return ANI_OK;
}

int ani_debug_deviation_parts(ani_handle* h, const void** d_parts, int64_t* member_stride) {
  if (!h || !d_parts || !member_stride) return ANI_ERR_ARG;
  *d_parts = h->use_single ? static_cast<const void*>(h->fused.gaev_parts.p) : static_cast<const void*>(h->armed.gaev_parts64.p);
  *member_stride = (int64_t)std::max(h->nrows, 1) * h->ap_run.aev_stride;
  return ANI_OK;
}

int ani_debug_list(ani_handle* h, const int** d_numneigh, const int** d_nbr_off, const int** d_jlist) {
  if (!h || !h->have_list) return ANI_ERR_ARG;
  if (d_numneigh) *d_numneigh = h->numneigh.p;
  if (d_nbr_off) *d_nbr_off = h->nbr_off.p;
  if (d_jlist) *d_jlist = h->jlist.p;
  return ANI_OK;
}

int ani_debug_colmap(ani_handle* h, int* out) {
  if (!h || !out) return ANI_ERR_ARG;
  for (int c = 0; c < h->ap_run.aev_len && c < (int)h->colmap.size(); c++) out[c] = h->colmap[c];
  return ANI_OK;
}

enum OptKind { kFlag, kRange, kSet };
enum OptInvalidates { kNothing, kSchedule, kList, kUpload };
struct OptRow { const char* name; int Options::*field; OptKind kind; int v[3]; const char* refusal; OptInvalidates invalidates; };
constexpr int kAny = 0x7fffffff;
static const OptRow kOptionRows[] = {
    {"prune_absent_species", &Options::prune, kFlag, {}, nullptr, kList},
    {"rdf_lanes", &Options::rdf_lanes, kSet, {16, 64, 64}, "ani_set_option: rdf_lanes is 16 or 64", kNothing},
    {"rdf_lds", &Options::rdf_lds, kFlag, {}, nullptr, kNothing},
    {"mlp_chain", &Options::mlp_chain, kRange, {-kAny - 1, kAny}, nullptr, kNothing},
    {"nbr_onepass", &Options::nbr_onepass, kFlag, {}, nullptr, kNothing},
    {"out_force_accumulate", &Options::out_force_accumulate, kFlag, {}, nullptr, kNothing},
    {"nbr_sorted_rows", &Options::nbr_sorted_rows, kFlag, {}, nullptr, kNothing},
    {"nbr_half_cells", &Options::nbr_half_cells, kFlag, {}, nullptr, kNothing},
    {"reuse_build_list_upload", &Options::reuse_upload, kFlag, {}, nullptr, kUpload},
    {"mlp_fused", &Options::mlp_fused, kRange, {0, 3}, "mlp_fused must be 0, 1, 2 or 3", kNothing},
    {"aev_symmetric_radial", &Options::aev_sym_radial, kFlag, {}, nullptr, kNothing},
    {"aev_tickets_min", &Options::aev_tickets_min, kRange, {0, kAny}, "aev_tickets_min must be >= 0", kNothing},
    {"aev_fused", &Options::aev_fused, kFlag, {}, nullptr, kNothing},
    {"mlp_fused_gen", &Options::mlp_fused_gen, kRange, {0, 1}, "mlp_fused_gen must be 0 or 1", kSchedule},
    {"mlp_fused_rows", &Options::mlp_fused_rows, kSet, {0, 64, 128}, "mlp_fused_rows must be 0, 64 or 128", kSchedule},
    {"mlp_fused_halves", &Options::mlp_fused_halves, kRange, {0, 2}, "mlp_fused_halves must be 0, 1 or 2", kSchedule},
    {"mlp_fused_schedule", &Options::mlp_fused_sched, kFlag, {}, nullptr, kSchedule},
    {"mlp_pipeline", &Options::mlp_pipeline, kRange, {0, 2}, "mlp_pipeline must be 0, 1 or 2", kNothing},
    {"mlp_arith", &Options::mlp_arith, kRange, {0, 2}, "mlp_arith must be 0 (fp32-input MFMA), 1 (bf16 x 3, exact) or 2 (fp16 x 2)", kNothing},
    {"mlp_split_bf16", &Options::mlp_arith, kFlag, {}, nullptr, kNothing},
    {"device_overwrite_forces", &Options::dev_overwrite, kFlag, {}, nullptr, kNothing},
    {"profiling", &Options::profiling, kFlag, {}, nullptr, kNothing},
    {"full_radial_capacity", nullptr, kFlag, {}, nullptr, kNothing},
};
static_assert(MLP_FP32 == 0 && MLP_BF16X3 == 1, "mlp_split_bf16 is a flag onto mlp_arith");

int ani_set_option(ani_handle* h, const char* name, int value) {
  if (!h || !name) return ANI_ERR_ARG;
  for (const OptRow& r : kOptionRows) {
    if (strcmp(name, r.name) != 0) continue;
    const bool ok = r.kind == kFlag || (r.kind == kRange ? value >= r.v[0] && value <= r.v[1] : value == r.v[0] || value == r.v[1] || value == r.v[2]);
    if (!ok) { h->err = r.refusal; return ANI_ERR_ARG; }
    const int stored = r.kind == kFlag ? value != 0 : value;
    if (r.field) h->opt.*r.field = stored;
    else h->ap.full_cap = h->ap_run.full_cap = stored;
    if (r.invalidates == kSchedule) h->fused.sched_key[0] = -1;
    if (r.invalidates == kList) { h->have_list = false; h->active_mask = -1; }
    if (r.invalidates == kUpload) h->host.x64_from = nullptr;
    return ANI_OK;
  }
  h->err = std::string("unknown option '") + name + "'";
  return ANI_ERR_ARG;
}

int ani_debug_fused_stamps(unsigned long long* out32, int reset) {
  const int r = fused_read_stamps(out32, reset);
  return r ? r : aev_read_stamps(out32, reset);
}

int ani_debug_fused_schedule_halves(int ntypes, const int* count, const double* cost, double half_ratio, int bins, int split_mode,
                                    int* split_out, int* items_out, int* off_out, int* n_items_out, double* makespan_out) {
  if (ntypes < 1 || ntypes > kMaxProblems || !count || !cost || bins < 1 || !items_out || !off_out || split_mode < 0 || split_mode > 2 ||
      !(half_ratio > 0.0))
    return ANI_ERR_ARG;
  for (int j = 0; j < ntypes; j++)
    if (count[j] < 0 || !(cost[j] > 0.0)) return ANI_ERR_ARG;
  int forced[kMaxProblems];
  const double T = fused_schedule_halves(ntypes, count, cost, half_ratio, bins, split_mode,
                                         forced_fused_split(getenv("ANI_FUSED_SPLIT"), ntypes, count, forced), split_out, items_out, off_out,
                                         n_items_out);
  if (makespan_out) *makespan_out = T;
  return ANI_OK;
}

int ani_debug_fused_schedule(int ntypes, const int* count, const double* cost, int bins, int* items_out, int* off_out,
                             double* makespan_out) {
  if (ntypes < 1 || ntypes > kMaxProblems || !count || !cost || bins < 1 || !items_out || !off_out) return ANI_ERR_ARG;
  for (int j = 0; j < ntypes; j++)
    if (count[j] < 0 || !(cost[j] > 0.0)) return ANI_ERR_ARG;
  (void)fused_schedule(ntypes, count, cost, bins, items_out, off_out);
  if (makespan_out) {
    std::vector<int> type_of;
    for (int j = 0; j < ntypes; j++) type_of.insert(type_of.end(), count[j], j);
    double worst = 0.0;
    for (int b = 0; b < bins; b++) {
      double load = 0.0;
      for (int i = off_out[b]; i < off_out[b + 1]; i++) load += cost[type_of[items_out[i]]];
      worst = std::max(worst, load);
    }
    *makespan_out = worst;
  }
  return ANI_OK;
}

int ani_debug_read(ani_handle* h, const void* d_src, void* host_dst, uint64_t bytes) {
  if (!h || !d_src || !host_dst) return ANI_ERR_ARG;
  HIP_TRY(h, hipSetDevice(h->device));
  HIP_TRY(h, hipStreamSynchronize(h->stream));
  HIP_TRY(h, hipMemcpy(host_dst, d_src, bytes, hipMemcpyDeviceToHost));
  return ANI_OK;
}

int ani_phase_timing(ani_handle* h, int enable) {
  if (!h) return ANI_ERR_ARG;
  h->timing.on = enable != 0;
  if (enable != 0 && h->timing.evt_pool.empty()) {
// ... 32 lines not shown
```

### lammps-ani_amd/csrc/ani_kernels.h

```cpp
#pragma once
#include <hip/hip_runtime.h>

#include <cstdint>
#include <vector>

#include "ani_fused_host.h"
#include "ani_model.h"

namespace ani {

constexpr int kRowTile = 128;
constexpr int kMaxRad = 256;
constexpr int kMaxAng = 96;
constexpr int kBucketInfoInts = 2 * kMaxSpecies + 5;
constexpr int kVirialSlots = 1024;

enum Epilogue { EPI_PLAIN = 0, EPI_CELU = 1, EPI_LAST = 2, EPI_BWD = 3 };

void note_launch_error(hipError_t e);
hipError_t take_launch_error();
int device_num_cus();
hipError_t raise_dynamic_lds(const void* kernel, int bytes);

struct GemmArgs {
// ... 60 lines not shown
  int member_items;
  float* gaev_parts;
  long long part_stride;
  float alpha, inv_alpha, scale;
  int* counter;
  const int* sched_items;
  const int* sched_off;
  int sched_blocks;
  int* err_flag;
};
void launch_build_stream(const float* src, int ld, int rows_valid, int k_valid, int NT, int KS, int chunk, int P, float scale,
                         unsigned short* dst, hipStream_t st);
hipError_t launch_mlp_fused(const FusedArgs& G, MlpArith arith, hipStream_t st);
hipError_t launch_mlp_fused16(const FusedArgs& G, MlpArith arith, int waves, hipStream_t st);
int fused16_b1_chunks(int nt0);
int fused16_b1_chunk_tiles(int nt0, int ci);
void launch_build_stream16(const float* src, int ld, int rows_valid, int k_valid, int NT, int KS, int order, int nt_off, int identity,
                           int P, float scale, unsigned short* dst, hipStream_t st);
void launch_sum_parts(const float* parts, long long part_stride, int M, float* dst, long long n, hipStream_t st);
int aev_read_stamps(unsigned long long* out32, int reset);
int fused_read_stamps(unsigned long long* out16, int reset);

void launch_split_planes(const float* src, int batch, long long s_src, int N, int K, int ld, MlpArith arith, float scale,
                         unsigned short* dst, hipStream_t st);
inline size_t split_elems(int N, int K, MlpArith arith) { return (size_t)N * ((K + 15) / 16) * 16 * mlp_planes(arith); }

struct SpeciesMap { int m[kMaxSpecies]; };
void launch_origin(const double* d_x, int ntotal, double* d_origin, hipStream_t st);
struct GhostFold {
  const long long* owner = nullptr;
  const double* shift = nullptr;
  int nlocal = 0;
};
void launch_ghost_chain(const long long* d_owner, int nghost, int nlocal, int* d_head, int* d_next, int* d_bad, hipStream_t st);
void launch_pack(const double* d_x, const int* d_species, int i0, int i1, const SpeciesMap& cmap, float4* xyzs, float* fbuf,
                 double* virial_acc, double* ev_zero, const double* d_origin, hipStream_t st, const GhostFold* gf = nullptr);
void launch_row_classes(const int4* row_info, const int* jlist, int nrows, int nlocal, int* flag, int* list, int* count, hipStream_t st);

void launch_step_tail(const double* d_ev, const int* d_flag, double* host_out, double stamp, hipStream_t st);
void launch_copy_out(const double* d_f, double* host, long long n, int nchunks, unsigned long long* d_ctr, unsigned* host_flags,
                     unsigned epoch, int nblocks, hipStream_t st);

struct PrepOut {
  int* nbr_off;
  int* row_of_centre;
  int* centre_of_row;
  int4* row_info;
  int* bucket_info;
  int* row_of_atom;
};
size_t prepare_scratch_ints(int nlocal);
void launch_prepare(const int* d_species, const int* d_ilist, const int* d_numneigh, int nlocal, int ntotal, int S, int nrows_cap,
                    const PrepOut& o, hipStream_t st, int row_stride = 0);
void launch_list_symmetry(const int* d_ilist, const int* d_nbr_off, const int* d_numneigh, const int* d_jraw, const int* d_row_of_atom,
                          int nlocal, int ntotal, unsigned* d_acc, int* d_out, hipStream_t st);

constexpr int kTicketGroups = 64;
constexpr int kTicketMaxGroups = 256;
static_assert(kTicketGroups <= kTicketMaxGroups, "kTicketGroups");
constexpr int kTicketStride = 64;
struct AevArgs {
  const float4* xyzs;
  const int* ilist;
  const int* numneigh;
  const int* nbr_off;
  const int* jlist;
  const int* centre_of_row;
  const int4* row_info;
  int nrows;
  float* aev;
  const float* gaev;
  float* fbuf;
  double* virial;
  int* err_flag;
  int4* cl_hdr;
  float4* cl_xyz;
  int* cl_j;
  int cl_stride;
  const int* row_list;
  int k0, kcount;
  const int* row_of_atom;
  int* row_counter;
};
int aev_compact_stride(const AevParams& p, int max_numneigh);
void launch_nbr_compact(const AevParams& p, const AevArgs& a, int max_numneigh, hipStream_t st);
void launch_aev_forward(const AevParams& p, const AevArgs& a, int max_numneigh, hipStream_t st);
bool launch_aev_forward_fused(const AevParams& p, const AevArgs& a, int max_numneigh, hipStream_t st);
struct RepTab {
  int on;
  float cutoff;
  float y[64], sa[64], k[64];
  double* erep;
  const double* x64;
};
bool launch_aev_backward(const AevParams& p, const AevArgs& a, int max_numneigh, hipStream_t st, const RepTab* rep = nullptr,
                         float* avir = nullptr);
bool aev_fast_path(const AevParams& p, int max_numneigh);
void launch_sort_jlist(const int* d_species, const int* d_nbr_off, const int* d_numneigh, const int* d_jin, int* d_jout,
                       int nlocal, int S, int present_mask, hipStream_t st, int in_stride = 0);

struct NbrGrid {
  double lo[3], inv[3];
  int nc[3], ncell;
  int reach = 1;
};
struct NbrScratch {
  int* cell_id;
  int* cell_count;
  int* cell_start;
  int* cursor;
  int* order;
  double* xs;
  float4* xq = nullptr;
};
void launch_nbr_bin(const double* d_x, int ntotal, const NbrGrid& g, const NbrScratch& s, hipStream_t st, const int* d_species = nullptr);
void launch_nbr_count(int nlocal, int ntotal, const NbrGrid& g, const NbrScratch& s, double cutneigh, int* d_numneigh,
                      int* d_nbr_off, hipStream_t st);
void launch_nbr_fill(int nlocal, int ntotal, const NbrGrid& g, const NbrScratch& s, double cutneigh, const int* d_nbr_off,
                     int* d_jlist, int* d_ilist, hipStream_t st);
void launch_nbr_onepass(int nlocal, int ntotal, const NbrGrid& g, const NbrScratch& s, double cutneigh, int cap, int* d_numneigh,
                        int* d_nbr_off, int* d_jrows, int* d_ilist, int* d_ovf, hipStream_t st);
bool nbr_sorted_rows_supported(int ntotal, int S, int cap);
void launch_nbr_sorted_rows(int nlocal, int ntotal, const NbrGrid& g, const NbrScratch& s, double cutneigh, int S, int cap,
                            int* d_numneigh, int* d_ilist, int* d_jrows, int* d_ovf, hipStream_t st);

struct RepArgs {
  const int4* row_info;
  int nrows;
  const int* jlist;
  const int* species;
  const double* pos;
  void* fbuf;
  double* virial;
  double* erep;
  const double* tables;
  int S, nslots, vslots;
  double cutoff;
};
void launch_repulsion(const RepArgs& a, bool fp64, hipStream_t st, void* avir = nullptr);
void launch_repulsion_energy(const double* erep, int nslots, double* d_ev, hipStream_t st);

struct FinishArgs {
  const float* e_rows;
  int M, nrows, nrows_ld;
  const int* centre_of_row;
  const int* ilist;
  const int* species;
  double sae[kMaxSpecies];
  const float* fbuf;
  int atom0, atom1;
  int energy;
  const double* virial_acc;
  double* f_out;
  int f_accumulate;
  double* ev_out;
  double* eatom_out;
  const int* err_flag;
  const int* fold_head = nullptr;
  const int* fold_next = nullptr;
  int fold_nlocal = 0;
};
void launch_finish(const FinishArgs& a, hipStream_t st);
void launch_atom_virial(const void* acc, bool fp64, int natoms, int ncomp, double* out, int accumulate, const int* fold_head,
                        const int* fold_next, int fold_nlocal, hipStream_t st);

void launch_dev_parts(float* parts, long long part_stride, int M, float* dst, long long n, int sum, hipStream_t st);
void launch_dev_parts64(double* parts, long long part_stride, int M, const double* dst, long long n, hipStream_t st);
void launch_dev_member(void* acc, bool fp64, int nrows_out, int nlocal, int m, int M, double* dforce, double* dsq, const int* fold_head,
                       const int* fold_next, int fold_nlocal, hipStream_t st);
constexpr int kDevEnergyParts = 32;
struct DevCloseArgs {
  const void* e_rows;
  int M, nrows, nrows_ld, nlocal;
  const int* centre_of_row;
  const int* ilist;
  const int* species;
  double sae[kMaxSpecies];
  const double* erep;
  int nslots;
// ... 98 lines not shown
```

### lammps-ani_amd/csrc/ani_kernels_aev.hip

```cpp
#include <algorithm>
#include <cstdlib>

#include <map>
#include <mutex>
#include <utility>

#include "ani_kernels.h"

namespace ani {

constexpr int kWaves = 4;
constexpr int kWavesB = 4;
constexpr int kBwdMinWaves = 4;
constexpr int kFwdMinWaves = 4;
constexpr int kFusedMinWaves = 4;
constexpr int kAevMax = 1024;
constexpr int kMaxBuckets = 36;

__device__ __forceinline__ void wave_sync() {
  __builtin_amdgcn_fence(__ATOMIC_ACQ_REL, "wavefront");
  __builtin_amdgcn_wave_barrier();
}
__device__ __forceinline__ int lanes_below(unsigned long long mask) {
  return __builtin_amdgcn_mbcnt_hi((unsigned)(mask >> 32), __builtin_amdgcn_mbcnt_lo((unsigned)mask, 0));
}
__device__ __forceinline__ int wave_incl_scan(int v) {
  v += __builtin_amdgcn_update_dpp(0, v, 0x111, 0xf, 0xf, false);
  v += __builtin_amdgcn_update_dpp(0, v, 0x112, 0xf, 0xf, false);
  v += __builtin_amdgcn_update_dpp(0, v, 0x114, 0xf, 0xf, false);
  v += __builtin_amdgcn_update_dpp(0, v, 0x118, 0xf, 0xf, false);
  v += __builtin_amdgcn_update_dpp(0, v, 0x142, 0xa, 0xf, false);
  v += __builtin_amdgcn_update_dpp(0, v, 0x143, 0xc, 0xf, false);
  return v;
}
__device__ __forceinline__ float fexp2(float x) { return __builtin_amdgcn_exp2f(x); }
__device__ __forceinline__ float flog2(float x) { return __builtin_amdgcn_logf(x); }
__device__ __forceinline__ float frcp(float x) { return __builtin_amdgcn_rcpf(x); }
__device__ __forceinline__ float frsq(float x) { return __builtin_amdgcn_rsqf(x); }
__device__ __forceinline__ float fcos_rev(float rev) { return __builtin_amdgcn_cosf(rev); }
__device__ __forceinline__ float fsin_rev(float rev) { return __builtin_amdgcn_sinf(rev); }
constexpr float kLog2e = 1.4426950408889634f;

#ifdef ABLB_STAMPS
__device__ unsigned long long g_bwd_stamps[32];
#define BWD_STAMP(k)                                                                          \
  do {                                                                                        \
    unsigned long long _t;                                                                    \
    asm volatile("s_waitcnt lgkmcnt(0)\n\ts_memtime %0\n\ts_waitcnt lgkmcnt(0)" : "=s"(_t)::"memory"); \
    stamp_acc[k] += _t - stamp_prev;                                                          \
    stamp_prev = _t;                                                                          \
  } while (0)
#define BWD_STAMP_VM(k)                                                                       \
  do {                                                                                        \
    asm volatile("s_waitcnt vmcnt(0)" ::: "memory");                                          \
    BWD_STAMP(k);                                                                             \
  } while (0)
#define BWD_STAMP_PARAMS , unsigned long long& stamp_prev, unsigned long long (&stamp_acc)[8]
#define BWD_STAMP_ARGS , stamp_prev, stamp_acc
#else
#define BWD_STAMP(k) do {} while (0)
#define BWD_STAMP_VM(k) do {} while (0)
#define BWD_STAMP_PARAMS
#define BWD_STAMP_ARGS
#endif

__device__ __forceinline__ void decode_pair(int t, int n, int& a, int& b) {
  const float fn = (float)(2 * n - 1);
  int aa = (int)((fn - __builtin_amdgcn_sqrtf(fn * fn - 8.f * (float)t)) * 0.5f);
  aa = max(0, min(aa, n - 2));
  const int n2 = 2 * n - 1;
  int s0 = __mul24(aa, n2 - aa) >> 1;
  const bool dn = s0 > t;
  aa -= dn ? 1 : 0;
  s0 = dn ? (__mul24(aa, n2 - aa) >> 1) : s0;
  const int s1 = __mul24(aa + 1, n2 - aa - 1) >> 1;
  const bool up = s1 <= t;
  aa += up ? 1 : 0;
  s0 = up ? s1 : s0;
  a = aa;
  b = aa + 1 + (t - s0);
}
__device__ __forceinline__ int triu_index(int s1, int s2, int S) {
  const int lo = s1 < s2 ? s1 : s2, hi = s1 < s2 ? s2 : s1;
  return lo * S - lo * (lo - 1) / 2 + (hi - lo);
}

__global__ __launch_bounds__(256) void sort_jlist_kernel(const int* __restrict__ species, const int* __restrict__ nbr_off,
// ... 349 lines not shown
  int a = 0, b = 0;
  if (valid) {
    if (e1.z) {
      decode_pair(u, e0.z, a, b);
    } else {
      a = (int)(((float)u + 0.5f) * frcp((float)e1.x));
      b = u - a * e1.x;
    }
  } else if (e1.z) {
    b = 1;
  }
  ia = e0.y + a;
  ib = e0.w + b;
}

template <int NA, int NZ>
__device__ __forceinline__ int build_pair_table(const AevParams& p, int lane, FastLds& L, int& nbk) {
  const int nb_all = p.S * (p.S + 1) / 2;
  int s1 = 0, s2 = 0, ns = 0, n1 = 0, n2 = 0;
  bool sw = false;
  if (lane < nb_all) {
    int rem = lane;
    while (rem >= p.S - s1) { rem -= p.S - s1; s1++; }
    s2 = s1 + rem;
    n1 = L.astart[s1 + 1] - L.astart[s1];
    n2 = L.astart[s2 + 1] - L.astart[s2];
    if (s1 == s2) {
      ns = (n1 * n1) >> 2;
    } else if (n1 > 0 && n2 > 0) {
      sw = n2 < n1;
      const int nr = sw ? n2 : n1, nc = sw ? n1 : n2;
      ns = ((nr + 1) >> 1) * nc;
    }
  }
  const int incl = wave_incl_scan(ns);
  const unsigned long long m = __ballot(ns > 0);
  if (ns > 0) {
    int* e = L.tb + 8 * lanes_below(m);
    e[0] = incl - ns; e[1] = L.astart[sw ? s2 : s1]; e[2] = sw ? n2 : n1; e[3] = L.astart[sw ? s1 : s2]; e[4] = sw ? n1 : n2;
    e[5] = p.radial_len + lane * (NA * NZ); e[6] = (s1 == s2) ? 1 : 0; e[7] = ns;
  }
  nbk = __popcll(m);
  return __builtin_amdgcn_readlane(incl, 63);
}
__device__ __forceinline__ void stream_pair_half(const FastLds& L, int nbk, int v, int h, int& ia, int& ib, int& outoff, int& pos,
                                                 bool& valid) {
  int e = 0;
  for (int k = 1; k < nbk; k++)
    if (v >= L.tb[8 * k]) e = k;
  const int4 e0 = *reinterpret_cast<const int4*>(L.tb + 8 * e);
  const int4 e1 = *reinterpret_cast<const int4*>(L.tb + 8 * e + 4);
  const int u = v - e0.x;
  outoff = e1.y;
  int a = 0, b = 0;
  pos = 0;
  valid = nbk > 0 && u < e1.w;
  if (valid) {
    if (e1.z) {
      const int n = e0.z;
      const float fn = (float)n;
      int k = (int)((fn - __builtin_amdgcn_sqrtf(fmaxf(fn * fn - 4.f * (float)u, 0.f))) * 0.5f);
      k = max(0, min(k, (n >> 1) - 1));
      if (__mul24(k, n - k) > u) k--;
      if (__mul24(k + 1, n - k - 1) <= u) k++;
      const int c = u - __mul24(k, n - k);
      a = 2 * k + h;
      b = 2 * k + 1 + c;
      pos = c - h;
      valid = h == 0 || c >= 1;
    } else {
      const int k = (int)(((float)u + 0.5f) * frcp((float)e1.x));
      const int c = u - k * e1.x;
      a = 2 * k + h;
      b = c;
      pos = c;
      valid = a < e0.z;
    }
  }
  if (!valid) { a = 0; b = e1.z ? 1 : 0; pos = 0; }
  ia = e0.y + a;
  ib = e0.w + b;
}

__device__ __forceinline__ void gd_add(double* p, float v) { atomicAdd(p, (double)v); }
template <int OFF>
__device__ __forceinline__ float xor_sum(float v) {
  const int x = __float_as_int(v);
  if constexpr (OFF == 1) {
    return v + __int_as_float(__builtin_amdgcn_mov_dpp(x, 0xB1, 0xf, 0xf, true));
  } else if constexpr (OFF == 2) {
    return v + __int_as_float(__builtin_amdgcn_mov_dpp(x, 0x4E, 0xf, 0xf, true));
  } else if constexpr (OFF == 4) {
    int y = __builtin_amdgcn_update_dpp(x, x, 0x104, 0xf, 0x5, false);
    y = __builtin_amdgcn_update_dpp(y, x, 0x114, 0xf, 0xa, false);
    return v + __int_as_float(y);
  } else if constexpr (OFF == 8) {
    return v + __int_as_float(__builtin_amdgcn_mov_dpp(x, 0x128, 0xf, 0xf, true));
  } else if constexpr (OFF == 16) {
    const auto r = __builtin_amdgcn_permlane16_swap((unsigned)x, (unsigned)x, false, false);
    return __uint_as_float(r[0]) + __uint_as_float(r[1]);
  } else {
    const auto r = __builtin_amdgcn_permlane32_swap((unsigned)x, (unsigned)x, false, false);
    return __uint_as_float(r[0]) + __uint_as_float(r[1]);
  }
}

template <int NA, int NZ>
__device__ __forceinline__ void forward_compute(const AevParams& p, const AevArgs& a, FastLds& L, int row, int lane BWD_STAMP_PARAMS);

template <int NA, int NZ, int NCH>
__device__ __forceinline__ void forward_centre(const AevParams& p, const AevArgs& a, FastLds& L, int row, const hdr_t& h,
                                               const Loaded<NCH, false, 1>& pf, int lane BWD_STAMP_PARAMS) {
  for (int e = lane; e < (p.aev_stride >> 2); e += 64) reinterpret_cast<float4*>(L.row)[e] = make_float4(0, 0, 0, 0);
  int nrad, nang;
  unpack_lists<NCH>(p, a, row, h, pf, lane, L, nrad, nang);
  wave_sync();
  BWD_STAMP(2);
  forward_compute<NA, NZ>(p, a, L, row, lane BWD_STAMP_ARGS);
}

template <int NA, int NZ>
__device__ __forceinline__ void forward_compute(const AevParams& p, const AevArgs& a, FastLds& L, int row, int lane BWD_STAMP_PARAMS) {
  constexpr int NR = 16, Q = 64 / NA;

  {
    const int q = lane >> 4, k = lane & 15;
    const float shf = fmaf((float)k, p.dShfR, p.ShfR0);
    const float c = -p.EtaR * kLog2e;
    for (int s = 0; s < p.S; s++) {
      const int b0 = L.rstart[s], b1 = L.rstart[s + 1];
      if (b1 <= b0) continue;
      float acc = 0.f, acc2 = 0.f;
      int t = b0 + q;
      for (; t + 4 < b1; t += 8) {
        const float r0 = L.rr[t], r1 = L.rr[t + 4], f0 = L.rfc[t], f1 = L.rfc[t + 4];
        const float d0 = r0 - shf, d1 = r1 - shf;
        acc = fmaf(fexp2(c * d0 * d0), f0, acc);
        acc2 = fmaf(fexp2(c * d1 * d1), f1, acc2);
      }
      if (t < b1) {
        const float dr = L.rr[t] - shf;
        acc = fmaf(fexp2(c * dr * dr), L.rfc[t], acc);
      }
      acc = xor_sum<32>(xor_sum<16>(acc + acc2));
      if (q == 0) L.row[s * NR + k] = 0.25f * acc;
    }
  }

  BWD_STAMP(3);
  int nbk;
  const int total = build_bucket_table<NA, NZ>(p, lane, L, nbk);
  wave_sync();
  BWD_STAMP(4);
  float acc[NZ];
#pragma unroll
  for (int z = 0; z < NZ; z++) acc[z] = 0.f;
  int cur_off = -1;
  const int la = lane % NA, lq = lane / NA;
  const float cA = -p.EtaA * kLog2e;

  auto flush = [&]() {
    if (cur_off >= 0) {
      float t[NZ / 2];
#pragma unroll
      for (int i = 0; i < NZ / 2; i++) {
        const auto r = __builtin_amdgcn_permlane32_swap(__float_as_uint(acc[i]), __float_as_uint(acc[i + NZ / 2]), false, false);
        t[i] = __uint_as_float(r[0]) + __uint_as_float(r[1]);
      }
      float u[NZ / 4];
#pragma unroll
      for (int i = 0; i < NZ / 4; i++) {
        const auto r = __builtin_amdgcn_permlane16_swap(__float_as_uint(t[i]), __float_as_uint(t[i + NZ / 4]), false, false);
        u[i] = __uint_as_float(r[0]) + __uint_as_float(r[1]);
      }
      float v;
      if constexpr (NA == 8) {
        v = xor_sum<8>(u[0]);
      } else {
        const bool odd = lane & 8;
        const float keep = odd ? u[1] : u[0], send = odd ? u[0] : u[1];
        v = keep + __int_as_float(__builtin_amdgcn_mov_dpp(__float_as_int(send), 0x128, 0xf, 0xf, true));
        v = xor_sum<4>(v);
      }
      if ((lane & NA) == 0) L.row[cur_off + la * NZ + (lane >> (NA == 8 ? 4 : 3))] = v;
    }
#pragma unroll
    for (int z = 0; z < NZ; z++) acc[z] = 0.f;
  };

  for (int base = 0; base < total; base += 64) {
    int outoff;
    {
      int ia, ib;
      bool valid;
      stream_pair(L, nbk, base + lane, ia, ib, outoff, valid);
      const float4 A = L.ad[ia], B = L.ad[ib];
      const float dot = A.x * B.x + A.y * B.y + A.z * B.z;
      const float cth = 0.95f * dot * frcp(fmaxf(A.w * B.w, 1e-10f));
      const float sth = __builtin_amdgcn_sqrtf(fmaxf(1.f - cth * cth, 0.f));
      const float w = valid ? 2.f * L.afc[ia] * L.afc[ib] : 0.f;
      const float rho = 0.5f * (A.w + B.w);
      float t1[NZ], t2[NA];
#pragma unroll
      for (int z = 0; z < NZ; z++) {
        const float basez = fmaxf(0.5f * (1.f + cth * p.cosZ[z] + sth * p.sinZ[z]), 0.f);
        t1[z] = w * fexp2(p.Zeta * flog2(basez));
      }
      float dr = rho - p.ShfA0;
#pragma unroll
      for (int s = 0; s < NA; s++) {
        t2[s] = fexp2(cA * dr * dr);
        dr -= p.dShfA;
      }
#pragma unroll
      for (int z = 0; z < NZ; z += 4)
        *reinterpret_cast<float4*>(L.pf1 + lane * NZ + z) = make_float4(t1[z], t1[z + 1], t1[z + 2], t1[z + 3]);
#pragma unroll
      for (int s = 0; s < NA; s += 4)
        *reinterpret_cast<float4*>(L.pf2 + lane * NA + s) = make_float4(t2[s], t2[s + 1], t2[s + 2], t2[s + 3]);
    }
    wave_sync();
    const int ngroups = min(NA, (total - base + Q - 1) / Q);
    float f2n = L.pf2[lq * NA + la];
    float4 qn[NZ / 4];
#pragma unroll
    for (int z4 = 0; z4 < NZ / 4; z4++) qn[z4] = *reinterpret_cast<const float4*>(L.pf1 + lq * NZ + 4 * z4);
#pragma unroll
    for (int g = 0; g < NA; g++) {
      if (g < ngroups) {
        const float f2 = f2n;
        float4 q[NZ / 4];
#pragma unroll
        for (int z4 = 0; z4 < NZ / 4; z4++) q[z4] = qn[z4];
        if (g + 1 < NA && g + 1 < ngroups) {
          const int slot = (g + 1) * Q + lq;
          f2n = L.pf2[slot * NA + la];
#pragma unroll
          for (int z4 = 0; z4 < NZ / 4; z4++) qn[z4] = *reinterpret_cast<const float4*>(L.pf1 + slot * NZ + 4 * z4);
        }
        const int off = __builtin_amdgcn_readlane(outoff, g * Q);
        if (off != cur_off) { flush(); cur_off = off; }
#pragma unroll
        for (int z4 = 0; z4 < NZ / 4; z4++) {
          acc[4 * z4] = fmaf(f2, q[z4].x, acc[4 * z4]); acc[4 * z4 + 1] = fmaf(f2, q[z4].y, acc[4 * z4 + 1]);
          acc[4 * z4 + 2] = fmaf(f2, q[z4].z, acc[4 * z4 + 2]); acc[4 * z4 + 3] = fmaf(f2, q[z4].w, acc[4 * z4 + 3]);
        }
      }
    }
    wave_sync();
  }
  flush();
  wave_sync();
  BWD_STAMP(5);

  float4* dst = reinterpret_cast<float4*>(a.aev + (long long)row * p.aev_stride);
  const int n4 = p.aev_stride >> 2;
  for (int e = lane; e < n4; e += 64) dst[e] = reinterpret_cast<const float4*>(L.row)[e];
  wave_sync();
  BWD_STAMP(6);
}

#define ANI_TICKETS_BEGIN(KW)                                                                              \
  const int nw = gridDim.x * KW;                                                                          \
  const int tk_ngrp = min((int)gridDim.x, kTicketGroups), tk_grp = blockIdx.x % tk_ngrp;                  \
  const int tk_share = (a.kcount + tk_ngrp - 1) / tk_ngrp, tk_base = tk_grp * tk_share;                   \
  int* const tk_ctr = a.row_counter ? a.row_counter + kTicketStride * tk_grp : nullptr;                   \
  const int kend = tk_ctr ? min(a.kcount, tk_base + tk_share) : a.kcount;                                 \
  int k = blockIdx.x * KW + wave, k1 = k + nw, tk_pending = 0;                                            \
  if (tk_ctr) {                                                                                           \
    int t0 = 0, t1 = 0;                                                                                   \
    if (lane == 0) { t0 = atomicAdd(tk_ctr, 1); t1 = atomicAdd(tk_ctr, 1); tk_pending = atomicAdd(tk_ctr, 1); } \
    k = tk_base + __builtin_amdgcn_readfirstlane(t0);                                                     \
    k1 = tk_base + __builtin_amdgcn_readfirstlane(t1);                                                    \
  }
#define ANI_TICKET_DRAW(tn)                                                                                \
  int tn = 0;                                                                                             \
  if (tk_ctr && lane == 0) tn = atomicAdd(tk_ctr, 1);
#define ANI_TICKET_TAKE(k2)                                                                                \
  touch(tk_pending);                                                                                      \
  const int k2 = tk_base + __builtin_amdgcn_readfirstlane(tk_pending);
#define ANI_TICKET_NEXT(tn, k2)                                                                            \
  k = k1;                                                                                                 \
  k1 = tk_ctr ? k2 : k1 + nw;                                                                             \
  tk_pending = tn;
#define ANI_TICKETS_END(KW)                                                                                \
  if (tk_ctr && lane == 0 && atomicAdd(tk_ctr + 1, 1) == ((int)gridDim.x - tk_grp + tk_ngrp - 1) / tk_ngrp * KW - 1) { \
    __atomic_store_n(tk_ctr, 0, __ATOMIC_RELAXED);                                                        \
    __atomic_store_n(tk_ctr + 1, 0, __ATOMIC_RELAXED);                                                    \
  }
#define ANI_PERSISTENT_LOOP(KW, NCH, BWD, GR, CENTRE)                                                      \
  ANI_TICKETS_BEGIN(KW)                                                                                   \
  while (k < ((tk_ctr && BWD) ? tk_base + tk_share : kend)) {                                             \
    ANI_TICKET_DRAW(tk_tn)                                                                                \
    const int kk = (tk_ctr && BWD) ? (k - tk_base) * tk_ngrp + tk_grp : k;    \
    const int kc = kk < a.kcount ? kk : a.kcount - 1;                                                     \
    const int row = a.row_list ? __builtin_amdgcn_readfirstlane(a.row_list[a.k0 + kc]) : a.k0 + kc;       \
    const hdr_t hc = load_header(a, row);                                                                 \
    ANI_TICKET_TAKE(tk_k2)                                                                                \
    if (hc[0] >= 0 && kk < a.kcount) {                                                                    \
      Loaded<NCH, BWD, GR> cur;                                                                           \
      load_lists(p, a, row, hdr_nrad(hc), hdr_nang(hc), lane, cur);                                       \
      CENTRE;                                                                                             \
    }                                                                                                     \
    ANI_TICKET_NEXT(tk_tn, tk_k2)                                                                         \
  }                                                                                                       \
  ANI_TICKETS_END(KW)

template <int NA, int NZ, int NCH>
__global__ __launch_bounds__(64 * kWaves, kFwdMinWaves) void aev_forward_fast(AevParams p, AevArgs a, int cap, int rowf) {
  extern __shared__ float4 smem4[];
  const int wave = __builtin_amdgcn_readfirstlane(threadIdx.x >> 6), lane = threadIdx.x & 63;
  FastLds L = carve<NA, NZ>(reinterpret_cast<float*>(smem4) + wave * fast_wave_floats_row(cap, false, rowf, p.S), cap, false, rowf);
#ifdef ABLB_STAMPS
  unsigned long long stamp_prev, stamp_acc[8] = {0, 0, 0, 0, 0, 0, 0, 0};
  asm volatile("s_memtime %0\n\ts_waitcnt lgkmcnt(0)" : "=s"(stamp_prev)::"memory");
  const int nw = gridDim.x * kWaves;
  for (int k = blockIdx.x * kWaves + wave; k < a.kcount; k += nw) {
    const int row = a.row_list ? __builtin_amdgcn_readfirstlane(a.row_list[a.k0 + k]) : a.k0 + k;
    const hdr_t hc = load_header(a, row);
    BWD_STAMP(0);
    if (hc[0] < 0) continue;
    Loaded<NCH, false, 1> cur;
    load_lists(p, a, row, hdr_nrad(hc), hdr_nang(hc), lane, cur);
    BWD_STAMP(1);
    forward_centre<NA, NZ, NCH>(p, a, L, row, hc, cur, lane, stamp_prev, stamp_acc);
    stamp_acc[7] += 1;
  }
  if (wave == 0 && lane == 0) {
    for (int q = 0; q < 7; q++) atomicAdd(&g_bwd_stamps[16 + q], stamp_acc[q]);
    atomicAdd(&g_bwd_stamps[24], stamp_acc[7]);
  }
#else
  ANI_PERSISTENT_LOOP(kWaves, NCH, false, 1, (forward_centre<NA, NZ, NCH>(p, a, L, row, hc, cur, lane)))
#endif
}

template <int NA, int NZ, int NCHC>
__global__ __launch_bounds__(64 * kWaves, kFusedMinWaves) void aev_forward_fused(AevParams p, AevArgs a, int cap, int rowf) {
  extern __shared__ float4 smem4[];
  const int wave = __builtin_amdgcn_readfirstlane(threadIdx.x >> 6), lane = threadIdx.x & 63;
  FastLds L = carve<NA, NZ>(reinterpret_cast<float*>(smem4) + wave * fast_wave_floats_row(cap, false, rowf, p.S), cap, false, rowf);
  ANI_TICKETS_BEGIN(kWaves)
  const int cap2 = a.cl_stride - kMaxAng;
  const float half_inv_Rcr = 0.5f * p.pi_over_Rcr * 0.3183098861837907f;
  const float half_inv_Rca = 0.5f * p.pi_over_Rca * 0.3183098861837907f;
  int4 info = load_info(a, k);
  int jj[NCHC];
  load_j(a, info, lane, jj);
  while (k < kend) {
    ANI_TICKET_DRAW(tn)
    const int4 info1 = load_info(a, k1);
    float4 xi, xx[NCHC];
    gather_x(a, info, jj, xi, xx);
    int jj1[NCHC];
    load_j(a, info1, lane, jj1);
    const int4 inf = uniform4(info);
    const int row = inf.w, i = inf.x, n = inf.x < 0 ? 0 : inf.z;
    for (int e = lane; e < (p.aev_stride >> 2); e += 64) reinterpret_cast<float4*>(L.row)[e] = make_float4(0, 0, 0, 0);
    int4* hdr = a.cl_hdr + 2 * (size_t)row;
    float4* oxyz = a.cl_xyz + (size_t)row * a.cl_stride;
    int* oj = a.cl_j + (size_t)row * a.cl_stride;
    int nA = 0, nR = 0;
    int cc = 0;
    int spc[NCHC];
    float4 dd[NCHC];
    int pos[NCHC];
#pragma unroll
    for (int c = 0; c < NCHC; c++) {
      pos[c] = -1;
      spc[c] = 0;
      dd[c] = make_float4(0.f, 0.f, 0.f, 1.f);
      if (64 * c < n) {
        const bool valid = 64 * c + lane < n;
        const float4 xj = xx[c];
        float4 d;
        d.x = xj.x - xi.x; d.y = xj.y - xi.y; d.z = xj.z - xi.z;
        d.w = __builtin_amdgcn_sqrtf(d.x * d.x + d.y * d.y + d.z * d.z);
        const int sp = __float_as_int(xj.w);
        const bool in_a = valid && d.w <= p.Rca;
        const bool in_2 = valid && !in_a && (p.compat || d.w <= p.Rcr);
        const unsigned long long mA = __ballot(in_a), m2 = __ballot(in_2);
        const int pA = nA + lanes_below(mA), p2 = nR + lanes_below(m2);
        for (int s = 0; s < p.S; s++) {
          const unsigned long long ms = __ballot(sp == s);
          const int k12 = __popcll(mA & ms) | (__popcll(m2 & ms) << 16);
          if (lane == s) cc += k12;
        }
        nA += __popcll(mA);
        nR += __popcll(m2);
        spc[c] = sp;
        dd[c] = d;
        pos[c] = (in_a && pA < kMaxAng) ? pA : ((in_2 && p2 < cap2) ? kMaxAng + p2 : -1);
      }
    }
#pragma unroll
    for (int c = 0; c < NCHC; c++) touch(jj1[c]);
    ANI_TICKET_TAKE(k2)
    const bool over = nA > kMaxAng || nR > cap2 || nA + nR > cap;
#pragma unroll
    for (int c = 0; c < NCHC; c++)
      if (pos[c] >= 0) { oxyz[pos[c]] = dd[c]; oj[pos[c]] = cl_pack(jj[c], spc[c]); }
    if (lane < 8) {
      reinterpret_cast<unsigned char*>(hdr)[8 + lane] = (unsigned char)(cc & 0xffff);
      reinterpret_cast<unsigned short*>(hdr)[8 + lane] = (unsigned short)(cc >> 16);
    }
    if (lane == 0) {
      reinterpret_cast<int*>(hdr)[0] = (over || inf.x < 0) ? -1 : i;
      reinterpret_cast<int*>(hdr)[1] = (nA + nR) | (nA << 16) | (__float_as_int(xi.w) << 24);
      if (over) atomicOr(a.err_flag, 1);
    }
    if (!over && inf.x >= 0) {
      int inc = cc;
      inc += __builtin_amdgcn_update_dpp(0, inc, 0x111, 0xf, 0xf, true);
      inc += __builtin_amdgcn_update_dpp(0, inc, 0x112, 0xf, 0xf, true);
      inc += __builtin_amdgcn_update_dpp(0, inc, 0x114, 0xf, 0xf, true);
      const int exc = inc - cc;
      if (lane <= p.S) { L.rstart[lane] = (exc & 0xffff) + (exc >> 16); L.astart[lane] = exc & 0xffff; }
      const int tab = (exc >> 16) | (inc << 16);
#pragma unroll
      for (int c = 0; c < NCHC; c++) {
        const int t = __shfl(tab, spc[c]);
        if (pos[c] >= 0) {
          const bool ang = pos[c] < kMaxAng;
          const int w = ang ? pos[c] : pos[c] - kMaxAng;
          const int pr = w + (ang ? (t & 0xffff) : ((unsigned)t >> 16));
          const float4 v = dd[c];
          L.rr[pr] = v.w;
          L.rfc[pr] = 0.5f * fcos_rev(v.w * half_inv_Rcr) + 0.5f;
          if (ang) {
            L.ad[w] = v;
            L.afc[w] = 0.5f * fcos_rev(v.w * half_inv_Rca) + 0.5f;
          }
        }
      }
      wave_sync();
#ifdef ABLB_STAMPS
      unsigned long long stamp_prev = 0, stamp_acc[8] = {0, 0, 0, 0, 0, 0, 0, 0};
      forward_compute<NA, NZ>(p, a, L, row, lane, stamp_prev, stamp_acc);
#else
      forward_compute<NA, NZ>(p, a, L, row, lane);
#endif
    }
    info = info1;
#pragma unroll
    for (int c = 0; c < NCHC; c++) jj[c] = jj1[c];
    ANI_TICKET_NEXT(tn, k2)
  }
  ANI_TICKETS_END(kWaves)
}

template <typename T>
__device__ __forceinline__ void scatter_neighbours(const AevArgs& a, const T* g, const int* jx, int cnt, int lane) {
  for (int base = 0; base < cnt; base += 16) {
    const int q = base + (lane >> 2), k = lane & 3;
    if (q < cnt && k < 3) atomicAdd(&a.fbuf[4 * jx[q] + k], -(float)g[3 * q + k]);
  }
}

template <typename T, typename D>
__device__ __forceinline__ void scatter_atom_virial(float* __restrict__ avir, const T* g, const D* d, int vs, const int* jx, int cnt,
                                                    int lane) {
  const int qs = lane / 9, k = lane - 9 * qs, ca = k / 3, cb = k - 3 * ca;
  for (int base = 0; base < cnt; base += 7) {
    const int q = base + qs;
    if (qs < 7 && q < cnt) atomicAdd(&avir[9 * (long long)jx[q] + k], (float)d[vs * q + ca] * (float)g[3 * q + cb]);
  }
}

template <int NA, int NZ, int NCH, int GR, bool VIR, bool AV, typename PF>
__device__ __forceinline__ void backward_centre(const AevParams& p, const AevArgs& a, FastLds& L, int row, const hdr_t h,
                                                const Loaded<NCH, true, GR> pf, int lane, float (&wv)[9],
                                                const RepTab& rep, float* __restrict__ avir, float* vt, float& er,
                                                PF&& before_final_scatter BWD_STAMP_PARAMS) {
  constexpr int NR = 16;
  const int centre = h[0];
  const int nrad = hdr_nrad(h), nang = hdr_nang(h);
  int rjp[NCH];
#pragma unroll
  for (int k = 0; k < NCH; k++) {
    rjp[k] = -1;
    if (a.row_of_atom && 64 * k + lane < nrad) rjp[k] = a.row_of_atom[cl_index(pf.jj[k])];
  }
#pragma unroll
  for (int c = 0; c < GR; c++)
    if (lane + 64 * c < (p.aev_stride >> 2)) reinterpret_cast<float4*>(L.row)[lane + 64 * c] = pf.grow[c];
  {
    const int word = lane < 4 ? h[2] : h[3];
    const int ca = lane < 8 ? (word >> (8 * (lane & 3))) & 0xff : 0;
    int inc = ca;
    inc += __builtin_amdgcn_update_dpp(0, inc, 0x111, 0xf, 0xf, true);
    inc += __builtin_amdgcn_update_dpp(0, inc, 0x112, 0xf, 0xf, true);
    inc += __builtin_amdgcn_update_dpp(0, inc, 0x114, 0xf, 0xf, true);
    if (lane <= p.S) L.astart[lane] = inc - ca;
  }
  wave_sync();

  float fx = 0.f, fy = 0.f, fz = 0.f;
  float ov[9] = {0.f, 0.f, 0.f, 0.f, 0.f, 0.f, 0.f, 0.f, 0.f};
  const float cR = -p.EtaR * kLog2e;
  const float rev = 0.5f * p.pi_over_Rcr * 0.3183098861837907f;
  const float revA = 0.5f * p.pi_over_Rca * 0.3183098861837907f;
  const float4* __restrict__ px = a.cl_xyz + (size_t)row * a.cl_stride;
  const int* __restrict__ pj = a.cl_j + (size_t)row * a.cl_stride;
  for (int base = 0; base < nrad; base += 64) {
    const int c = base >> 6, t0 = base + lane;
    const bool live = t0 < nrad, ang = t0 < nang;
    const int w = ang ? t0 : t0 - nang;
    float4 v = make_float4(0.f, 0.f, 0.f, 1.f);
    int j = 0;
    if (c < NCH) {
#pragma unroll
      for (int k = 0; k < NCH; k++)
        if (c == k) { v = pf.xx[k]; j = pf.jj[k]; }
    } else if (live) {
      v = px[slot_index(t0, nang)];
      j = pj[slot_index(t0, nang)];
    }
    const int t = w;
    float gx = 0.f, gy = 0.f, gz = 0.f;
    const int s = cl_species(j);
    j = cl_index(j);
    float gsx = 0.f, gsy = 0.f, gsz = 0.f;
    int rj = -1;
    if (c < NCH) {
#pragma unroll
      for (int k = 0; k < NCH; k++)
        if (c == k) rj = rjp[k];
    } else if (a.row_of_atom && live) rj = a.row_of_atom[j];
    const bool sym = rj >= 0;
    if (live) {
      const float4* gg4 = reinterpret_cast<const float4*>(L.row + s * NR);
      const float4* qq4 = reinterpret_cast<const float4*>(a.gaev + (size_t)(sym ? rj : row) * p.aev_stride + hdr_species(h) * NR);
      const float r = v.w;
      const float fc = 0.5f * fcos_rev(r * rev) + 0.5f;
      const float dfc = -0.5f * p.pi_over_Rcr * fsin_rev(r * rev);
      float dEdr = 0.f, dEdn = 0.f;
      {
        const float cd = cR * p.dShfR * p.dShfR;
        const float C0 = fexp2(0.25f * cd), C1 = fexp2(2.25f * cd), C2 = fexp2(6.25f * cd), C3 = fexp2(12.25f * cd);
        const float kf = -2.f * p.EtaR * fc;
#pragma unroll
        for (int hf = 0; hf < 2; hf++) {
          const float dc = r - (p.ShfR0 + (3.5f + 8.f * hf) * p.dShfR);
          const float x = cR * dc;
          const float E = fexp2(x * dc), H = fexp2(-x * p.dShfR), Hi = fexp2(x * p.dShfR);
          const float R = H * H, Ri = Hi * Hi;
          float e[8];
          float up = E * H, dn = E * Hi;
          e[4] = up * C0; up *= R; e[5] = up * C1; up *= R; e[6] = up * C2; up *= R; e[7] = up * C3;
          e[3] = dn * C0; dn *= Ri; e[2] = dn * C1; dn *= Ri; e[1] = dn * C2; dn *= Ri; e[0] = dn * C3;
          const float4 ga = gg4[2 * hf], gb = gg4[2 * hf + 1];
          const float gk[8] = {ga.x, ga.y, ga.z, ga.w, gb.x, gb.y, gb.z, gb.w};
          float4 qa = make_float4(0.f, 0.f, 0.f, 0.f), qb = qa;
          if (sym) { qa = qq4[2 * hf]; qb = qq4[2 * hf + 1]; }
          const float qk[8] = {qa.x, qa.y, qa.z, qa.w, qb.x, qb.y, qb.z, qb.w};
          float dr = dc + 3.5f * p.dShfR;
#pragma unroll
          for (int kk = 0; kk < 8; kk++) {
            const float tk = e[kk] * fmaf(kf, dr, dfc);
            dEdr = fmaf(gk[kk], tk, dEdr);
            dEdn = fmaf(qk[kk], tk, dEdn);
            dr -= p.dShfR;
          }
        }
      }
      const float inv_r = frcp(r);
      const float sc = 0.25f * dEdr * inv_r, scn = 0.25f * dEdn * inv_r;
      gx = sc * v.x; gy = sc * v.y; gz = sc * v.z;
      gsx = scn * v.x; gsy = scn * v.y; gsz = scn * v.z;
      if (rep.on && r < rep.cutoff) {
        const int ti = 8 * hdr_species(h) + s;
        const double* xj = rep.x64 + 3 * (long long)j;
        const double* xc = rep.x64 + 3 * (long long)centre;
        const double ddx = xj[0] - xc[0], ddy = xj[1] - xc[1], ddz = xj[2] - xc[2];
        const double r64 = sqrt(ddx * ddx + ddy * ddy + ddz * ddz);
        const float rr = (float)r64;
        const float x = rr * frcp(rep.cutoff), den = 1.f - x * x;
        if (den > 1e-10f) {
          const float fcr = fexp2((1.f - frcp(den)) * kLog2e);
          const float dfcr = fcr * (-(2.f * x * frcp(rep.cutoff)) * frcp(den * den));
          const float db = rr * 1.8897261258369282f, al = rep.sa[ti], kk = rep.k[ti];
          const float pk1 = fexp2((kk - 1.f) * flog2(db));
          const float g = rep.y[ti] * frcp(db) * fexp2(-al * pk1 * db * kLog2e);
          const float dg = 1.8897261258369282f * g * (-frcp(db) - al * kk * pk1);
          er += 0.5f * g * fcr;
          const float sr = 0.5f * (dg * fcr + g * dfcr);
          const double inv = 1.0 / r64;
          const float rx = sr * (float)(ddx * inv), ry = sr * (float)(ddy * inv), rz = sr * (float)(ddz * inv);
          gx += rx; gy += ry; gz += rz;
          if (sym) { gsx += rx; gsy += ry; gsz += rz; }
        }
      }
    }
    if constexpr (AV) {
      ov[0] += v.x * gsx; ov[1] += v.x * gsy; ov[2] += v.x * gsz;
      ov[3] += v.y * gsx; ov[4] += v.y * gsy; ov[5] += v.y * gsz;
      ov[6] += v.z * gsx; ov[7] += v.z * gsy; ov[8] += v.z * gsz;
    }
    if (live && ang) {
      L.ad[t] = v;
      L.afc[t] = 0.5f * fcos_rev(v.w * revA) + 0.5f;
      L.aj[t] = j;
      if (sym) {
        fx += gx + gsx; fy += gy + gsy; fz += gz + gsz;
        if constexpr (VIR) {
          wv[0] += gx * v.x; wv[1] += gx * v.y; wv[2] += gx * v.z;
          wv[3] += gy * v.x; wv[4] += gy * v.y; wv[5] += gy * v.z;
          wv[6] += gz * v.x; wv[7] += gz * v.y; wv[8] += gz * v.z;
        }
        gx = gy = gz = 0.f;
      }
      L.gd[3 * t] = gx; L.gd[3 * t + 1] = gy; L.gd[3 * t + 2] = gz;
    }
    const int lo = min(max(nang - base, 0), 64), hi = min(nrad - base, 64);
    if (hi > lo) {
      const bool out = live && !ang && !sym;
      const unsigned long long mout = __ballot(out);
      if (live && !ang) {
        fx += gx + gsx; fy += gy + gsy; fz += gz + gsz;
        if constexpr (VIR) {
          wv[0] += gx * v.x; wv[1] += gx * v.y; wv[2] += gx * v.z;
          wv[3] += gy * v.x; wv[4] += gy * v.y; wv[5] += gy * v.z;
          wv[6] += gz * v.x; wv[7] += gz * v.y; wv[8] += gz * v.z;
        }
        if (out) {
          const int q = lanes_below(mout);
          L.gt[3 * q] = gx; L.gt[3 * q + 1] = gy; L.gt[3 * q + 2] = gz;
          L.jt[q] = j;
          if constexpr (AV) { vt[3 * q] = v.x; vt[3 * q + 1] = v.y; vt[3 * q + 2] = v.z; }
        }
      }
      wave_sync();
      scatter_neighbours(a, L.gt, L.jt, __popcll(mout), lane);
      if constexpr (AV) scatter_atom_virial(avir, L.gt, vt, 3, L.jt, __popcll(mout), lane);
      wave_sync();
    }
  }
  BWD_STAMP(2);
  int nbk;
  const int total_pairs = build_pair_table<NA, NZ>(p, lane, L, nbk);
  wave_sync();
  BWD_STAMP(3);
  const float cA = -p.EtaA * kLog2e;
  for (int base = 0; base < total_pairs; base += 32) {
    int ia, ib, outoff, pos;
    bool valid;
    stream_pair_half(L, nbk, base + (lane & 31), lane >> 5, ia, ib, outoff, pos, valid);
    const float4 A = L.ad[ia], B = L.ad[ib];
    const float inv_ra = frcp(A.w), inv_rb = frcp(B.w);
    const float inv_rr = inv_ra * inv_rb;
    const float cosv = (A.x * B.x + A.y * B.y + A.z * B.z) * inv_rr;
    const float c = 0.95f * cosv;
    const float s2 = fmaxf(1.f - c * c, 1e-12f);
    const float inv_s = frsq(s2);
    const float sn = s2 * inv_s;
    const float fa = L.afc[ia], fb = L.afc[ib];
    const float dfa = -0.5f * p.pi_over_Rca * fsin_rev(A.w * revA);
    const float dfb = -0.5f * p.pi_over_Rca * fsin_rev(B.w * revA);
    const float rho = 0.5f * (A.w + B.w);
    float f1[NZ], df1[NZ];
#pragma unroll
    for (int z = 0; z < NZ; z++) {
      const float bz = fmaxf(0.5f * (1.f + c * p.cosZ[z] + sn * p.sinZ[z]), 0.f);
      const float pm1 = fexp2((p.Zeta - 1.f) * flog2(bz));
      f1[z] = pm1 * bz;
      df1[z] = p.Zeta * pm1 * 0.5f * (sn * p.cosZ[z] - c * p.sinZ[z]) * inv_s;
    }
    const float4* gg4 = reinterpret_cast<const float4*>(L.row + outoff);
    float Aq = 0.f, Bq = 0.f, Cq = 0.f;
    float drA = rho - p.ShfA0;
#pragma unroll
    for (int sa = 0; sa < NA; sa++) {
      const float dr = drA;
      drA -= p.dShfA;
      const float f2 = fexp2(cA * dr * dr);
      const float df2 = -2.f * p.EtaA * dr * f2;
      float g1 = 0.f, gd1 = 0.f;
#pragma unroll
      for (int z4 = 0; z4 < NZ / 4; z4++) {
        const float4 gv = gg4[sa * (NZ / 4) + z4];
        g1 = fmaf(gv.x, f1[4 * z4], g1); gd1 = fmaf(gv.x, df1[4 * z4], gd1);
        g1 = fmaf(gv.y, f1[4 * z4 + 1], g1); gd1 = fmaf(gv.y, df1[4 * z4 + 1], gd1);
        g1 = fmaf(gv.z, f1[4 * z4 + 2], g1); gd1 = fmaf(gv.z, df1[4 * z4 + 2], gd1);
        g1 = fmaf(gv.w, f1[4 * z4 + 3], g1); gd1 = fmaf(gv.w, df1[4 * z4 + 3], gd1);
      }
      Aq = fmaf(f2, gd1, Aq);
      Cq = fmaf(f2, g1, Cq);
      Bq = fmaf(df2, g1, Bq);
    }
    const float P = valid ? fa * fb : 0.f;
    Aq *= 2.f * P * 0.95f;
    Bq *= P;
    Cq *= valid ? 2.f : 0.f;
    const float cc = Aq * inv_rr;
    const float ta = (Bq + Cq * dfa * fb) * inv_ra - Aq * cosv * inv_ra * inv_ra;
    const float tb = (Bq + Cq * fa * dfb) * inv_rb - Aq * cosv * inv_rb * inv_rb;
    const float va[3] = {cc * B.x + ta * A.x, cc * B.y + ta * A.y, cc * B.z + ta * A.z};
    const float vb[3] = {cc * A.x + tb * B.x, cc * A.y + tb * B.y, cc * A.z + tb * B.z};
    if (valid) { gd_add(&L.gd[3 * ib], vb[0]); gd_add(&L.gd[3 * ib + 1], vb[1]); gd_add(&L.gd[3 * ib + 2], vb[2]); }
    float rs[3] = {va[0], va[1], va[2]};
#pragma unroll
    for (int k = 0; k < 3; k++) {
      float t;
      t = __int_as_float(__builtin_amdgcn_update_dpp(0, __float_as_int(rs[k]), 0x111, 0xf, 0xf, true)); rs[k] += pos >= 1 ? t : 0.f;
      t = __int_as_float(__builtin_amdgcn_update_dpp(0, __float_as_int(rs[k]), 0x112, 0xf, 0xf, true)); rs[k] += pos >= 2 ? t : 0.f;
      t = __int_as_float(__builtin_amdgcn_update_dpp(0, __float_as_int(rs[k]), 0x114, 0xf, 0xf, true)); rs[k] += pos >= 4 ? t : 0.f;
      t = __int_as_float(__builtin_amdgcn_update_dpp(0, __float_as_int(rs[k]), 0x118, 0xf, 0xf, true)); rs[k] += pos >= 8 ? t : 0.f;
    }
    const int pos_next = __builtin_amdgcn_update_dpp(0, pos, 0x101, 0xf, 0xf, true);
    if (valid && pos_next == 0) { gd_add(&L.gd[3 * ia], rs[0]); gd_add(&L.gd[3 * ia + 1], rs[1]); gd_add(&L.gd[3 * ia + 2], rs[2]); }
  }
  wave_sync();
  BWD_STAMP(4);
  for (int q = lane; q < nang; q += 64) {
    const float gx = (float)L.gd[3 * q], gy = (float)L.gd[3 * q + 1], gz = (float)L.gd[3 * q + 2];
    fx += gx; fy += gy; fz += gz;
    if constexpr (VIR) {
      const float4 d = L.ad[q];
      wv[0] += gx * d.x; wv[1] += gx * d.y; wv[2] += gx * d.z;
      wv[3] += gy * d.x; wv[4] += gy * d.y; wv[5] += gy * d.z;
      wv[6] += gz * d.x; wv[7] += gz * d.y; wv[8] += gz * d.z;
    }
  }
  before_final_scatter();
  scatter_neighbours(a, L.gd, L.aj, nang, lane);
  if constexpr (AV) {
    scatter_atom_virial(avir, L.gd, reinterpret_cast<const float*>(L.ad), 4, L.aj, nang, lane);
    float mine = 0.f;
#pragma unroll
    for (int k = 0; k < 9; k++) {
      const float t = xor_sum<32>(xor_sum<16>(xor_sum<8>(xor_sum<4>(xor_sum<2>(xor_sum<1>(ov[k]))))));
      if (lane == k) mine = t;
    }
    if (lane < 9) atomicAdd(&avir[9 * (long long)centre + lane], mine);
  }
  fx = xor_sum<32>(xor_sum<16>(xor_sum<8>(xor_sum<4>(xor_sum<2>(xor_sum<1>(fx))))));
  fy = xor_sum<32>(xor_sum<16>(xor_sum<8>(xor_sum<4>(xor_sum<2>(xor_sum<1>(fy))))));
  fz = xor_sum<32>(xor_sum<16>(xor_sum<8>(xor_sum<4>(xor_sum<2>(xor_sum<1>(fz))))));
  if (lane < 3) atomicAdd(&a.fbuf[4 * centre + lane], lane == 0 ? fx : (lane == 1 ? fy : fz));
  wave_sync();
  BWD_STAMP(5);
}

__host__ __device__ constexpr int bwd_wave_floats(int cap, int rowf, int S, bool av) {
  return fast_wave_floats_row(cap, true, rowf, S) + (av ? 3 * 64 : 0);
}
static_assert((fast_wave_floats(0, true) + 3 * 64) * 4 * kWavesB <= 160 * 1024, "armed backward LDS");

template <int NA, int NZ, int NCH, int GR, bool VIR, typename... AVP>
__global__ __launch_bounds__(64 * kWavesB, kBwdMinWaves) void aev_backward_fast(AevParams p, AevArgs a, int cap, int rowf, RepTab rep,
                                                                                AVP... avp) {
  constexpr bool AV = sizeof...(AVP) > 0;
  float* avir = nullptr;
  if constexpr (AV) avir = (avp, ...);
  extern __shared__ float4 smem4[];
  const int wave = __builtin_amdgcn_readfirstlane(threadIdx.x >> 6), lane = threadIdx.x & 63;
  float* wbase = reinterpret_cast<float*>(smem4) + wave * bwd_wave_floats(cap, rowf, p.S, AV);
  FastLds L = carve<NA, NZ>(wbase, cap, true, rowf);
  float* vt = AV ? wbase + fast_wave_floats_row(cap, true, rowf, p.S) : nullptr;
  float wv[9] = {0.f, 0.f, 0.f, 0.f, 0.f, 0.f, 0.f, 0.f, 0.f};
  float er = 0.f;
#ifdef ABLB_STAMPS
  unsigned long long stamp_prev, stamp_acc[8] = {0, 0, 0, 0, 0, 0, 0, 0};
  asm volatile("s_memtime %0\n\ts_waitcnt lgkmcnt(0)" : "=s"(stamp_prev)::"memory");
  const int nw = gridDim.x * kWavesB;
  for (int k = blockIdx.x * kWavesB + wave; k < a.kcount; k += nw) {
    const int row = a.row_list ? __builtin_amdgcn_readfirstlane(a.row_list[a.k0 + k]) : a.k0 + k;
    const hdr_t hc = load_header(a, row);
    BWD_STAMP(0);
    if (hc[0] < 0) continue;
    Loaded<NCH, true, GR> cur;
    load_lists(p, a, row, hdr_nrad(hc), hdr_nang(hc), lane, cur);
#ifdef ABLB_STAMPS_VM
    BWD_STAMP_VM(1);
#else
    BWD_STAMP(1);
#endif
    backward_centre<NA, NZ, NCH, GR, VIR, AV>(p, a, L, row, hc, cur, lane, wv, rep, avir, vt, er, [] {}, stamp_prev, stamp_acc);
    stamp_acc[6] += 1;
  }
  if (wave == 0 && lane == 0) {
    for (int q = 0; q < 6; q++) atomicAdd(&g_bwd_stamps[q], stamp_acc[q]);
    atomicAdd(&g_bwd_stamps[8], stamp_acc[6]);
  }
#else
  ANI_TICKETS_BEGIN(kWavesB)
  const int kstop = tk_ctr ? tk_base + tk_share : kend;
  auto rank_of = [&](int kx) -> int { return tk_ctr ? (kx - tk_base) * tk_ngrp + tk_grp : kx; };
  auto row_of = [&](int kk) -> int {
    const int kc = kk < a.kcount ? kk : a.kcount - 1;
    return a.row_list ? __builtin_amdgcn_readfirstlane(a.row_list[a.k0 + kc]) : a.k0 + kc;
  };
  bool have = false;
  hdr_t hc;
  Loaded<NCH, true, GR> cur;
  while (k < kstop) {
    ANI_TICKET_DRAW(tk_tn)
    const int kk = rank_of(k);
    const int row = row_of(kk);
    const bool in_range = kk < a.kcount;
    if (!have) {
      hc = load_header_scalar(a, row);
      if (hc[0] >= 0 && in_range) load_lists(p, a, row, hdr_nrad(hc), hdr_nang(hc), lane, cur);
    }
    have = false;
    ANI_TICKET_TAKE(tk_k2)
    if (hc[0] >= 0 && in_range) {
      backward_centre<NA, NZ, NCH, GR, VIR, AV>(p, a, L, row, hc, cur, lane, wv, rep, avir, vt, er, [&]() {
        const int kk1 = rank_of(k1);
        if (k1 < kstop && kk1 < a.kcount) {
          const int row1 = row_of(kk1);
          hc = load_header_scalar(a, row1);
          if (hc[0] >= 0) load_lists(p, a, row1, hdr_nrad(hc), hdr_nang(hc), lane, cur);
          have = true;
        }
      });
    }
    ANI_TICKET_NEXT(tk_tn, tk_k2)
  }
  ANI_TICKETS_END(kWavesB)
#endif
  if (rep.on) {
    double se = (double)er;
#pragma unroll
    for (int off = 32; off > 0; off >>= 1) se += __shfl_xor(se, off);
    if (lane == 0) atomicAdd(&rep.erep[(blockIdx.x * kWavesB + wave) & (kVirialSlots - 1)], se);
  }
  if constexpr (VIR) {
    if (a.virial) {
#pragma unroll
      for (int k = 0; k < 9; k++) {
        double sv = (double)wv[k];
#pragma unroll
        for (int off = 32; off > 0; off >>= 1) sv += __shfl_xor(sv, off);
        if (lane == 0) atomicAdd(&a.virial[9 * ((blockIdx.x * kWavesB + wave) & (kVirialSlots - 1)) + k], -sv);
      }
    }
  }
}

struct WaveLds {
  float dx[kMaxRad], dy[kMaxRad], dz[kMaxRad], r[kMaxRad], fc[kMaxRad];
  int sp[kMaxRad], j[kMaxRad];
  int ang[kMaxAng];
  float fca[kMaxAng];
  float row[kAevMax];
  float gd[3 * kMaxRad];
};

__device__ __forceinline__ void compact_neighbours(const AevParams& p, const AevArgs& a, int ii, int lane, WaveLds& L,
                                                   int& nrad, int& nang, bool& over) {
  const int i = a.ilist[ii];
  const float4 xi = a.xyzs[i];
  const int beg = a.nbr_off[ii];
  const int n = a.numneigh[ii];
  nrad = 0;
  nang = 0;
  over = false;
  for (int base = 0; base < n; base += 64) {
    const int q = base + lane;
    const bool valid = q < n;
    const int j = valid ? a.jlist[beg + q] : i;
    const float4 xj = a.xyzs[j];
    const float dx = xj.x - xi.x, dy = xj.y - xi.y, dz = xj.z - xi.z;
    const float r = sqrtf(dx * dx + dy * dy + dz * dz);
    const bool in_r = valid && (p.compat || r <= p.Rcr);
    const bool in_a = valid && r <= p.Rca;
    const unsigned long long mr = __ballot(in_r);
    const unsigned long long ma = __ballot(in_a);
    const int pos = nrad + lanes_below(mr);
    if (in_r && pos < kMaxRad) {
      L.dx[pos] = dx; L.dy[pos] = dy; L.dz[pos] = dz; L.r[pos] = r;
      L.fc[pos] = 0.5f * cosf(r * p.pi_over_Rcr) + 0.5f;
      L.sp[pos] = __float_as_int(xj.w);
      L.j[pos] = j;
    }
    const int posa = nang + lanes_below(ma);
    if (in_a && posa < kMaxAng && pos < kMaxRad) {
      L.ang[posa] = pos;
      L.fca[posa] = 0.5f * cosf(r * p.pi_over_Rca) + 0.5f;
    }
    nrad += __popcll(mr);
    nang += __popcll(ma);
  }
  if (nrad > kMaxRad) { nrad = kMaxRad; over = true; }
  if (nang > kMaxAng) { nang = kMaxAng; over = true; }
}

__global__ __launch_bounds__(64 * kWaves) void aev_forward_generic(AevParams p, AevArgs a) {
  __shared__ WaveLds lds[kWaves];
  const int wave = threadIdx.x >> 6, lane = threadIdx.x & 63;
  const int row = blockIdx.x * kWaves + wave;
  if (row >= a.nrows) return;
  const int ii = a.centre_of_row[row];
  if (ii < 0) return;
  WaveLds& L = lds[wave];
// ... 189 lines not shown
  return 0;
#endif
}

static int fast_kind(const AevParams& p) {
  if (p.nR != 16 || p.S > 8 || (p.aev_stride & 3) || !p.equi) return 0;
  {
    const float d = fabsf(p.dShfR), c0 = p.ShfR0 + 3.5f * p.dShfR, c1 = p.ShfR0 + 11.5f * p.dShfR;
    const float dmax = fmaxf(fmaxf(fabsf(p.Rcr - c0), fabsf(c0)), fmaxf(fabsf(p.Rcr - c1), fabsf(c1)));
    const float q = sqrtf(87.f / p.EtaR) - 3.5f * d;
    if (2.f * p.EtaR * dmax * d > 80.f || p.EtaR * 12.25f * d * d > 80.f || q <= 0.f || p.EtaR * q * q < 20.f) return 0;
  }
  if (p.nA == 8 && p.nZ == 4) return 1;
  if (p.nA == 4 && p.nZ == 8) return 2;
  return 0;
}

constexpr int kCapGrain = 64;
static int radial_cap(const AevParams& p, int max_numneigh) {
  int full = (max_numneigh + 63) / 64 * 64;
  if (full < 64) full = 64;
  if (p.compat || p.full_cap) return full;
  int est = (3 * max_numneigh + 3) / 4;
  if (est < 128) est = 128;
  est = (est + kCapGrain - 1) / kCapGrain * kCapGrain;
  return est < full ? est : full;
}

bool aev_fast_path(const AevParams& p, int max_numneigh) {
  if (!fast_kind(p)) return false;
  const int c = radial_cap(p, max_numneigh);
  return (size_t)fast_wave_floats(c, true) * 4 * kWavesB <= 160 * 1024 && (size_t)fast_wave_floats(c, false) * 4 * kWaves <= 160 * 1024;
}

static const char* waves_env() { return "ANI_AEV_WAVES_PER_CU"; }
template <typename K>
static int persistent_blocks(K kernel, int nrows, int waves_per_block, size_t lds_bytes) {
  static std::map<std::pair<const void*, size_t>, int> cache;
  static std::mutex mtx;
  int per_cu = 0;
  {
    std::lock_guard<std::mutex> lock(mtx);
    const auto key = std::make_pair((const void*)kernel, lds_bytes);
    const auto it = cache.find(key);
    if (it != cache.end()) per_cu = it->second;
    else {
      if (hipOccupancyMaxActiveBlocksPerMultiprocessor(&per_cu, kernel, 64 * waves_per_block, lds_bytes) != hipSuccess || per_cu < 1)
        per_cu = (int)((160 * 1024) / (lds_bytes ? lds_bytes : 1));
      cache[key] = per_cu;
    }
  }
  if (per_cu > 8) per_cu = 8;
  static const int forced = [] { const char* e = getenv(waves_env()); return e ? atoi(e) : 0; }();
  if (forced > 0 && forced * waves_per_block / 2 >= 1) per_cu = std::min(per_cu, std::max(1, forced / waves_per_block));
  if (per_cu < 1) per_cu = 1;
  const int need = (nrows + waves_per_block - 1) / waves_per_block;
  const int fit = device_num_cus() * per_cu;
  return need < fit ? need : fit;
}

template <typename K, typename... Extra>
static void launch_fast(K kernel, const AevParams& p, const AevArgs& a, int waves, size_t lds, int cap, int rowf, hipStream_t st,
                        Extra... extra) {
  note_launch_error(raise_dynamic_lds((const void*)kernel, 160 * 1024));
  hipLaunchKernelGGL(kernel, dim3(persistent_blocks(kernel, a.kcount, waves, lds)), dim3(64 * waves), lds, st, p, a, cap, rowf,
                     extra...);
}

int aev_compact_stride(const AevParams& p, int max_numneigh) {
  return aev_fast_path(p, max_numneigh) ? kMaxAng + radial_cap(p, max_numneigh) : 0;
}

void launch_nbr_compact(const AevParams& p, const AevArgs& a, int max_numneigh, hipStream_t st) {
  if (a.kcount <= 0 || !aev_fast_path(p, max_numneigh)) return;
  const int cap = radial_cap(p, max_numneigh);
  auto go = [&](auto kernel) {
    hipLaunchKernelGGL(kernel, dim3(persistent_blocks(kernel, a.kcount, kWavesC, 0)), dim3(64 * kWavesC), 0, st, p, a, cap);
  };
  if (max_numneigh <= 128) go(nbr_compact_kernel<2>);
  else if (max_numneigh <= 192) go(nbr_compact_kernel<3>);
  else go(nbr_compact_kernel<4>);
}

void launch_aev_forward(const AevParams& p, const AevArgs& a, int max_numneigh, hipStream_t st) {
  if (a.nrows <= 0) return;
  const dim3 grid((a.nrows + kWaves - 1) / kWaves), block(64 * kWaves);
  if (aev_fast_path(p, max_numneigh)) {
    if (a.kcount <= 0) return;
    const int cap = radial_cap(p, max_numneigh);
    const int rowf = (p.aev_stride + 63) / 64 * 64;
    const size_t lds = (size_t)fast_wave_floats_row(cap, false, rowf, p.S) * 4 * kWaves;
    const bool k1 = fast_kind(p) == 1, n2 = !p.compat;
    if (k1 && n2) launch_fast(aev_forward_fast<8, 4, 1>, p, a, kWaves, lds, cap, rowf, st);
    else if (k1) launch_fast(aev_forward_fast<8, 4, 3>, p, a, kWaves, lds, cap, rowf, st);
    else if (n2) launch_fast(aev_forward_fast<4, 8, 1>, p, a, kWaves, lds, cap, rowf, st);
    else launch_fast(aev_forward_fast<4, 8, 3>, p, a, kWaves, lds, cap, rowf, st);
  } else {
    hipLaunchKernelGGL(aev_forward_generic, grid, block, 0, st, p, a);
  }
}

bool launch_aev_forward_fused(const AevParams& p, const AevArgs& a, int max_numneigh, hipStream_t st) {
  if (a.nrows <= 0 || a.kcount <= 0 || !aev_fast_path(p, max_numneigh) || max_numneigh > 256) return false;
  const int cap = radial_cap(p, max_numneigh);
  const int rowf = (p.aev_stride + 63) / 64 * 64;
  const size_t lds = (size_t)fast_wave_floats_row(cap, false, rowf, p.S) * 4 * kWaves;
  const bool k1 = fast_kind(p) == 1;
  const int nch = max_numneigh <= 128 ? 2 : (max_numneigh <= 192 ? 3 : 4);
  if (k1) {
    if (nch == 2) launch_fast(aev_forward_fused<8, 4, 2>, p, a, kWaves, lds, cap, rowf, st);
    else if (nch == 3) launch_fast(aev_forward_fused<8, 4, 3>, p, a, kWaves, lds, cap, rowf, st);
    else launch_fast(aev_forward_fused<8, 4, 4>, p, a, kWaves, lds, cap, rowf, st);
  } else {
    if (nch == 2) launch_fast(aev_forward_fused<4, 8, 2>, p, a, kWaves, lds, cap, rowf, st);
    else if (nch == 3) launch_fast(aev_forward_fused<4, 8, 3>, p, a, kWaves, lds, cap, rowf, st);
    else launch_fast(aev_forward_fused<4, 8, 4>, p, a, kWaves, lds, cap, rowf, st);
  }
  return true;
}

bool launch_aev_backward(const AevParams& p, const AevArgs& a, int max_numneigh, hipStream_t st, const RepTab* rep, float* avir) {
  if (a.nrows <= 0) return true;
  RepTab rt{};
  if (rep) rt = *rep;
  const dim3 grid((a.nrows + kWaves - 1) / kWaves), block(64 * kWaves);
  if (aev_fast_path(p, max_numneigh)) {
    if (a.kcount <= 0) return true;
    const int cap = radial_cap(p, max_numneigh);
    const int rowf = (p.aev_stride + 63) / 64 * 64;
    const size_t lds = (size_t)bwd_wave_floats(cap, rowf, p.S, avir != nullptr) * 4 * kWavesB;
    const bool k1 = fast_kind(p) == 1, n2 = !p.compat, g1 = p.aev_stride <= 256;
#define ANI_BWD_CASE(NA, NZ, NCH, GR)                                                                              \
  do {                                                                                                             \
    if (avir) launch_fast(aev_backward_fast<NA, NZ, NCH, GR, true, float*>, p, a, kWavesB, lds, cap, rowf, st, rt, avir);  \
    else if (a.virial) launch_fast(aev_backward_fast<NA, NZ, NCH, GR, true>, p, a, kWavesB, lds, cap, rowf, st, rt);      \
    else launch_fast(aev_backward_fast<NA, NZ, NCH, GR, false>, p, a, kWavesB, lds, cap, rowf, st, rt);                   \
  } while (0)
    if (k1) {
      if (n2 && g1) ANI_BWD_CASE(8, 4, 1, 1);
      else if (n2) ANI_BWD_CASE(8, 4, 1, 4);
      else if (g1) ANI_BWD_CASE(8, 4, 3, 1);
      else ANI_BWD_CASE(8, 4, 3, 4);
    } else {
      if (n2 && g1) ANI_BWD_CASE(4, 8, 1, 1);
      else if (n2) ANI_BWD_CASE(4, 8, 1, 4);
      else if (g1) ANI_BWD_CASE(4, 8, 3, 1);
      else ANI_BWD_CASE(4, 8, 3, 4);
    }
#undef ANI_BWD_CASE
    return true;
  }
  if (avir) hipLaunchKernelGGL(aev_backward_generic<float*>, grid, block, 0, st, p, a, avir);
  else hipLaunchKernelGGL(aev_backward_generic<>, grid, block, 0, st, p, a);
  return false;
}

}
```

Before: 61.39.

## Precompute per-neighbour-count stream tables to drive AEV forward/backward kernels

Adds a one-time build of per-species-count descriptor and word tables, produced by a new kernel and stored on the handle. The fast AEV forward, fused and backward kernels can then stream precomputed work descriptors per centre, indexed by its radial and angular neighbour counts, instead of deriving them on the fly. The goal is to cut per-centre index and bucket setup work in the AEV hot path. In exchange it adds table memory, scalar loads per centre, more template instantiations, and a host-synchronised rebuild whenever the species mask changes. It only applies when S is 1 or 2, and in the backward kernel only on the single-group, single-chunk variants.

```diff
diff --git a/include/ani_hip.h b/include/ani_hip.h
--- a/include/ani_hip.h
+++ b/include/ani_hip.h
@@ -95,6 +95,15 @@
 const char* ani_last_mlp_kernel(const ani_handle* h);
 int ani_debug_get(ani_handle* h, ani_debug_view* out);
 int ani_debug_colmap(ani_handle* h, int* out);
+typedef struct ani_stream_tables_view {
+  int32_t species, bound, tuples;
+  int32_t builds;
+  int64_t words_bwd, words_fwd;
+  const void *d_words_bwd, *d_words_fwd;
+  double build_ms;
+} ani_stream_tables_view;
+int ani_debug_stream_tables(ani_handle* h, ani_stream_tables_view* view, int32_t* desc_bwd, uint32_t* words_bwd, int32_t* desc_fwd,
+                            uint32_t* words_fwd);
 int ani_debug_deviation_parts(ani_handle* h, const void** d_parts, int64_t* member_stride);
 
 int ani_set_option(ani_handle* h, const char* name, int value);
diff --git a/lammps-ani_amd/ani_hip.py b/lammps-ani_amd/ani_hip.py
--- a/lammps-ani_amd/ani_hip.py
+++ b/lammps-ani_amd/ani_hip.py
@@ -13,7 +13,7 @@
 
 EXPORTS = ["ani_create", "ani_destroy", "ani_last_error", "ani_num_models", "ani_use_num_models", "ani_num_species",
            "ani_aev_length", "ani_cutoff_radial", "ani_cutoff_angular", "ani_compute_full", "ani_compute_half",
-           "ani_compute_full_device", "ani_build_list_device", "ani_build_list", "ani_debug_list", "ani_debug_get", "ani_debug_read", "ani_debug_colmap", "ani_set_option", "ani_phase_timing", "ani_phase_times",
+           "ani_compute_full_device", "ani_build_list_device", "ani_build_list", "ani_debug_list", "ani_debug_get", "ani_debug_read", "ani_debug_colmap", "ani_debug_stream_tables", "ani_set_option", "ani_phase_timing", "ani_phase_times",
            "ani_trace_push", "ani_trace_pop", "ani_trace_mark", "ani_step_begin", "ani_step_ghosts_ready", "ani_step_finish",
            "ani_debug_fused_stamps", "ani_attach_comm", "ani_debug_fused_schedule", "ani_debug_fused_schedule_halves", "ani_last_mlp_kernel", "ani_host_register", "ani_host_unregister", "ani_set_ghost_fold", "ani_stage_ghost_fold",
            "ani_request_atom_virial", "ani_request_model_deviation", "ani_debug_deviation_parts",
@@ -33,6 +33,12 @@
     _fields_ = [("nlocal", C.c_int), ("ntotal", C.c_int), ("nrows", C.c_int), ("npairs", C.c_int64),
                 ("d_aev", C.c_void_p), ("d_gaev", C.c_void_p), ("d_row_of_centre", C.c_void_p),
                 ("species_count", C.c_int * 16), ("aev_stride", C.c_int), ("aev_active_length", C.c_int), ("error_flags", C.c_int)]
+
+
+class StreamTablesView(C.Structure):
+    _fields_ = [("species", C.c_int32), ("bound", C.c_int32), ("tuples", C.c_int32), ("builds", C.c_int32),
+                ("words_bwd", C.c_int64), ("words_fwd", C.c_int64), ("d_words_bwd", C.c_void_p), ("d_words_fwd", C.c_void_p),
+                ("build_ms", C.c_double)]
 
 
 class FireParams(C.Structure):
@@ -167,6 +173,7 @@
         L.ani_debug_get.argtypes = [C.c_void_p, C.POINTER(DebugView)]
         L.ani_debug_read.argtypes = [C.c_void_p, C.c_void_p, C.c_void_p, C.c_uint64]
         L.ani_debug_colmap.argtypes = [C.c_void_p, C.c_void_p]
+        L.ani_debug_stream_tables.argtypes = [C.c_void_p, C.POINTER(StreamTablesView)] + [C.c_void_p] * 4
         L.ani_set_option.argtypes = [C.c_void_p, C.c_char_p, C.c_int]
         L.ani_last_mlp_kernel.argtypes = [C.c_void_p]
         L.ani_set_ghost_fold.argtypes = [C.c_void_p, C.c_void_p, C.c_void_p, C.c_int, C.c_void_p]
@@ -468,6 +475,18 @@
         self._check(self._lib.ani_debug_read(self._h, d_ptr, out.ctypes.data, out.nbytes))
         return out
 
+    def stream_tables(self, contents: bool = True) -> dict:
+        v = StreamTablesView()
+        self._check(self._lib.ani_debug_stream_tables(self._h, C.byref(v), None, None, None, None))
+        out = {n: getattr(v, n) for n, _ in StreamTablesView._fields_}
+        if contents and v.species:
+            db, df = np.zeros((v.tuples, 4), np.int32), np.zeros((v.tuples, 4), np.int32)
+            wb, wf = np.zeros(max(v.words_bwd, 1), np.uint32), np.zeros(max(v.words_fwd, 1), np.uint32)
+            self._check(self._lib.ani_debug_stream_tables(self._h, C.byref(v), db.ctypes.data, wb.ctypes.data, df.ctypes.data,
+                                                          wf.ctypes.data))
+            out.update(desc_bwd=db, words_bwd=wb[: v.words_bwd], desc_fwd=df, words_fwd=wf[: v.words_fwd])
+        return out
+
     def colmap(self) -> np.ndarray:
         v = self.debug_view()
         out = np.zeros(v.aev_active_length, dtype=np.int32)
diff --git a/lammps-ani_amd/csrc/ani_handle.h b/lammps-ani_amd/csrc/ani_handle.h
--- a/lammps-ani_amd/csrc/ani_handle.h
+++ b/lammps-ani_amd/csrc/ani_handle.h
@@ -89,6 +89,7 @@
   int aev_fused = 1;
   int aev_sym_radial = 1;
   int aev_tickets_min = 40000;
+  int aev_stream_tables = 1;
   int mlp_fused_sched = 1;
   int mlp_fused_halves = 1;
   int mlp_fused = 1;
@@ -111,6 +112,18 @@
   int sched_key[4] = {-1, -1, -1, -1};
   int sched_nitems = 0;
   DevBuf<float> gaev_parts;
+};
+
+struct StreamTables {
+  int mask = -2;
+  int S = 0, nt = 0;
+  int tuples = 0;
+  size_t nwords_b = 0, nwords_f = 0;
+  int builds = 0;
+  double build_ms = 0;
+  DevBuf<int4> desc_b, desc_f;
+  DevBuf<unsigned> words_b, words_f;
+  StreamTab view() const { return StreamTab{desc_b.p, words_b.p, desc_f.p, words_f.p, nt}; }
 };
 
 struct DevOut { double *member_energy, *atom_energy_dev, *member_dforce, *atom_force_dev, *summary; };
@@ -196,6 +209,7 @@
   int active_mask = -1;
   Options opt;
   FusedState fused;
+  StreamTables stab;
   Armed armed;
   MolFinder mol;
   Rdf rdf;
@@ -270,6 +284,7 @@
 int check_args(ani_handle* h, int ntotal, int nlocal, long long npairs, int ago);
 int upload_model(ani_handle* h);
 int specialize(ani_handle* h, int mask);
+int build_stream_tables(ani_handle* h, hipStream_t st);
 int compute_mlp(ani_handle* h, hipStream_t st);
 void free_fused(ani_handle* h, int fi);
 const int* forced_fused_split(const char* env, int ntypes, const int* count, int* split);
diff --git a/lammps-ani_amd/csrc/ani_hip.cpp b/lammps-ani_amd/csrc/ani_hip.cpp
--- a/lammps-ani_amd/csrc/ani_hip.cpp
+++ b/lammps-ani_amd/csrc/ani_hip.cpp
@@ -183,11 +183,19 @@
   return a;
 }
 
+static const StreamTab* step_stream_tab(const ani_handle* h, StreamTab& view) {
+  if (!h->opt.aev_stream_tables || h->stab.S == 0 || h->stab.S != h->ap_run.S || h->stab.mask != h->active_mask) return nullptr;
+  view = h->stab.view();
+  return &view;
+}
+
 int step_compact_forward(ani_handle* h, const AevArgs& a, hipStream_t st) {
+  StreamTab tab_view;
+  const StreamTab* tab = step_stream_tab(h, tab_view);
   if (h->opt.aev_fused) {
     TraceRange tr("ani: neighbour compaction + AEV forward");
     if (h->timing.evt) HIP_TRY(h, hipEventRecord(h->timing.evt[5], st));
-    if (launch_aev_forward_fused(h->ap_run, a, h->max_numneigh, st)) {
+    if (launch_aev_forward_fused(h->ap_run, a, h->max_numneigh, st, tab)) {
       if (h->timing.evt) HIP_TRY(h, hipEventRecord(h->timing.evt[1], st));
       return ANI_OK;
     }
@@ -199,7 +207,7 @@
   if (h->timing.evt) HIP_TRY(h, hipEventRecord(h->timing.evt[5], st));
   {
     TraceRange tr("ani: AEV forward");
-    launch_aev_forward(h->ap_run, a, h->max_numneigh, st);
+    launch_aev_forward(h->ap_run, a, h->max_numneigh, st, tab);
   }
   if (h->timing.evt) HIP_TRY(h, hipEventRecord(h->timing.evt[1], st));
   return ANI_OK;
@@ -223,7 +231,8 @@
       }
   }
   float* avir = static_cast<float*>(h->armed.av_acc);
-  const bool rep_done = launch_aev_backward(h->ap_run, a, h->max_numneigh, st, rt.on ? &rt : nullptr, avir) && rt.on;
+  StreamTab tab_view;
+  const bool rep_done = launch_aev_backward(h->ap_run, a, h->max_numneigh, st, rt.on ? &rt : nullptr, avir, step_stream_tab(h, tab_view)) && rt.on;
   if (m.has_rep && !rep_done) {
     RepArgs ra{};
     ra.row_info = h->row_info.p; ra.nrows = h->nrows; ra.jlist = h->jlist.p; ra.species = h->species.p;
@@ -475,6 +484,7 @@
   h->virial_acc.release(); h->aev.release(); h->gaev.release(); h->act.release(); h->aev64.release(); h->gaev64.release(); h->act64.release(); h->e_rows64.release(); h->fbuf64.release(); h->e_rows.release(); h->fbuf.release();
   for (int fi = 0; fi < 4; fi++) free_fused(h, fi);
   h->fused.counter.release(); h->fused.gaev_parts.release(); h->fused.sched.release();
+  h->stab.desc_b.release(); h->stab.desc_f.release(); h->stab.words_b.release(); h->stab.words_f.release();
   free_chain_plan(h->chain_plan);
   for (auto& e : h->timing.evt_pool) if (e) (void)hipEventDestroy(e);
   if (h->stream) (void)hipStreamDestroy(h->stream);
diff --git a/lammps-ani_amd/csrc/ani_hip_list.cpp b/lammps-ani_amd/csrc/ani_hip_list.cpp
--- a/lammps-ani_amd/csrc/ani_hip_list.cpp
+++ b/lammps-ani_amd/csrc/ani_hip_list.cpp
@@ -54,6 +54,8 @@
   {
     const int rcs = specialize(h, info[2 * kMaxSpecies + 3]);
     if (rcs) return rcs;
+    const int rct = build_stream_tables(h, st);
+    if (rct) return rct;
   }
   h->list_symmetric = true;
   if (!h->list_is_ours && h->use_single && h->opt.aev_sym_radial && nlocal > 0) {
diff --git a/lammps-ani_amd/csrc/ani_hip_model.cpp b/lammps-ani_amd/csrc/ani_hip_model.cpp
--- a/lammps-ani_amd/csrc/ani_hip_model.cpp
+++ b/lammps-ani_amd/csrc/ani_hip_model.cpp
@@ -197,4 +197,42 @@
   }
   return ANI_OK;
 }
-}
+
+int build_stream_tables(ani_handle* h, hipStream_t st) {
+  StreamTables& t = h->stab;
+  if (t.mask == h->active_mask) return ANI_OK;
+  const auto t0 = std::chrono::steady_clock::now();
+  t.mask = h->active_mask;
+  t.S = 0; t.nt = 0; t.tuples = 0; t.nwords_b = t.nwords_f = 0;
+  const AevParams& p = h->ap_run;
+  if (!h->use_single || !stream_tab_supported(p)) return ANI_OK;
+  std::vector<int4> db, df;
+  for (int nt = p.S == 1 ? kMaxAng : kStreamTabNT; nt >= 1; nt /= 2) {
+    const int n = stream_tab_tuples(p.S, nt);
+    HIP_TRY(h, t.desc_b.reserve(n));
+    HIP_TRY(h, t.desc_f.reserve(n));
+    launch_stream_table(p, nt, true, t.desc_b.p, nullptr, 0, st);
+    launch_stream_table(p, nt, false, t.desc_f.p, nullptr, 0, st);
+    db.resize(n); df.resize(n);
+    HIP_TRY(h, hipMemcpyAsync(db.data(), t.desc_b.p, sizeof(int4) * n, hipMemcpyDeviceToHost, st));
+    HIP_TRY(h, hipMemcpyAsync(df.data(), t.desc_f.p, sizeof(int4) * n, hipMemcpyDeviceToHost, st));
+    HIP_TRY(h, hipStreamSynchronize(st));
+    size_t nb = 0, nf = 0;
+    for (int i = 0; i < n; i++) { db[i].x = (int)nb; nb += db[i].w; df[i].x = (int)nf; nf += df[i].w; }
+    if ((nb + nf) * sizeof(unsigned) + 2 * sizeof(int4) * (size_t)n > kStreamTabMaxBytes) continue;
+    HIP_TRY(h, t.words_b.reserve(std::max<size_t>(nb, 1)));
+    HIP_TRY(h, t.words_f.reserve(std::max<size_t>(nf, 1)));
+    HIP_TRY(h, hipMemcpyAsync(t.desc_b.p, db.data(), sizeof(int4) * n, hipMemcpyHostToDevice, st));
+    HIP_TRY(h, hipMemcpyAsync(t.desc_f.p, df.data(), sizeof(int4) * n, hipMemcpyHostToDevice, st));
+    launch_stream_table(p, nt, true, t.desc_b.p, t.words_b.p, 1, st);
+    launch_stream_table(p, nt, false, t.desc_f.p, t.words_f.p, 1, st);
+    HIP_TRY(h, hipStreamSynchronize(st));
+    HIP_TRY(h, hipGetLastError());
+    t.S = p.S; t.nt = nt; t.tuples = n; t.nwords_b = nb; t.nwords_f = nf;
+    break;
+  }
+  t.builds++;
+  t.build_ms = std::chrono::duration<double, std::milli>(std::chrono::steady_clock::now() - t0).count();
+  return ANI_OK;
+}
+}
diff --git a/lammps-ani_amd/csrc/ani_hip_options.cpp b/lammps-ani_amd/csrc/ani_hip_options.cpp
--- a/lammps-ani_amd/csrc/ani_hip_options.cpp
+++ b/lammps-ani_amd/csrc/ani_hip_options.cpp
@@ -36,6 +36,27 @@
   if (d_numneigh) *d_numneigh = h->numneigh.p;
   if (d_nbr_off) *d_nbr_off = h->nbr_off.p;
   if (d_jlist) *d_jlist = h->jlist.p;
+  return ANI_OK;
+}
+
+int ani_debug_stream_tables(ani_handle* h, ani_stream_tables_view* view, int32_t* desc_bwd, uint32_t* words_bwd, int32_t* desc_fwd,
+                            uint32_t* words_fwd) {
+  if (!h || !view) return ANI_ERR_ARG;
+  memset(view, 0, sizeof(*view));
+  const StreamTables& t = h->stab;
+  view->builds = t.builds;
+  view->build_ms = t.build_ms;
+  if (t.S == 0 || t.mask != h->active_mask) return ANI_OK;
+  view->species = t.S; view->bound = t.nt; view->tuples = t.tuples;
+  view->words_bwd = (int64_t)t.nwords_b; view->words_fwd = (int64_t)t.nwords_f;
+  view->d_words_bwd = t.words_b.p; view->d_words_fwd = t.words_f.p;
+  if (!desc_bwd && !words_bwd && !desc_fwd && !words_fwd) return ANI_OK;
+  HIP_TRY(h, hipSetDevice(h->device));
+  HIP_TRY(h, hipStreamSynchronize(h->stream));
+  if (desc_bwd) HIP_TRY(h, hipMemcpy(desc_bwd, t.desc_b.p, sizeof(int4) * t.tuples, hipMemcpyDeviceToHost));
+  if (desc_fwd) HIP_TRY(h, hipMemcpy(desc_fwd, t.desc_f.p, sizeof(int4) * t.tuples, hipMemcpyDeviceToHost));
+  if (words_bwd && t.nwords_b) HIP_TRY(h, hipMemcpy(words_bwd, t.words_b.p, sizeof(unsigned) * t.nwords_b, hipMemcpyDeviceToHost));
+  if (words_fwd && t.nwords_f) HIP_TRY(h, hipMemcpy(words_fwd, t.words_f.p, sizeof(unsigned) * t.nwords_f, hipMemcpyDeviceToHost));
   return ANI_OK;
 }
 
@@ -63,6 +84,7 @@
     {"aev_symmetric_radial", &Options::aev_sym_radial, kFlag, {}, nullptr, kNothing},
     {"aev_tickets_min", &Options::aev_tickets_min, kRange, {0, kAny}, "aev_tickets_min must be >= 0", kNothing},
     {"aev_fused", &Options::aev_fused, kFlag, {}, nullptr, kNothing},
+    {"aev_stream_tables", &Options::aev_stream_tables, kFlag, {}, nullptr, kNothing},
     {"mlp_fused_gen", &Options::mlp_fused_gen, kRange, {0, 1}, "mlp_fused_gen must be 0 or 1", kSchedule},
     {"mlp_fused_rows", &Options::mlp_fused_rows, kSet, {0, 64, 128}, "mlp_fused_rows must be 0, 64 or 128", kSchedule},
     {"mlp_fused_halves", &Options::mlp_fused_halves, kRange, {0, 2}, "mlp_fused_halves must be 0, 1 or 2", kSchedule},
diff --git a/lammps-ani_amd/csrc/ani_kernels.h b/lammps-ani_amd/csrc/ani_kernels.h
--- a/lammps-ani_amd/csrc/ani_kernels.h
+++ b/lammps-ani_amd/csrc/ani_kernels.h
@@ -166,10 +166,23 @@
   const int* row_of_atom;
   int* row_counter;
 };
+struct StreamTab {
+  const int4* desc_b;
+  const unsigned* words_b;
+  const int4* desc_f;
+  const unsigned* words_f;
+  int nt;
+};
+constexpr int kStreamTabNT = 32;
+constexpr size_t kStreamTabMaxBytes = 8u << 20;
+inline int stream_tab_tuples(int S, int nt) { return S == 1 ? nt + 1 : (S == 2 ? (nt + 1) * (nt + 1) : 0); }
+bool stream_tab_supported(const AevParams& p);
+void launch_stream_table(const AevParams& p, int nt, bool backward, int4* d_desc, unsigned* d_words, int fill, hipStream_t st);
+
 int aev_compact_stride(const AevParams& p, int max_numneigh);
 void launch_nbr_compact(const AevParams& p, const AevArgs& a, int max_numneigh, hipStream_t st);
-void launch_aev_forward(const AevParams& p, const AevArgs& a, int max_numneigh, hipStream_t st);
-bool launch_aev_forward_fused(const AevParams& p, const AevArgs& a, int max_numneigh, hipStream_t st);
+void launch_aev_forward(const AevParams& p, const AevArgs& a, int max_numneigh, hipStream_t st, const StreamTab* tab = nullptr);
+bool launch_aev_forward_fused(const AevParams& p, const AevArgs& a, int max_numneigh, hipStream_t st, const StreamTab* tab = nullptr);
 struct RepTab {
   int on;
   float cutoff;
@@ -178,7 +191,7 @@
   const double* x64;
 };
 bool launch_aev_backward(const AevParams& p, const AevArgs& a, int max_numneigh, hipStream_t st, const RepTab* rep = nullptr,
-                         float* avir = nullptr);
+                         float* avir = nullptr, const StreamTab* tab = nullptr);
 bool aev_fast_path(const AevParams& p, int max_numneigh);
 void launch_sort_jlist(const int* d_species, const int* d_nbr_off, const int* d_numneigh, const int* d_jin, int* d_jout,
                        int nlocal, int S, int present_mask, hipStream_t st, int in_stride = 0);
diff --git a/lammps-ani_amd/csrc/ani_kernels_aev.hip b/lammps-ani_amd/csrc/ani_kernels_aev.hip
--- a/lammps-ani_amd/csrc/ani_kernels_aev.hip
+++ b/lammps-ani_amd/csrc/ani_kernels_aev.hip
@@ -3,6 +3,7 @@
 
 #include <map>
 #include <mutex>
+#include <type_traits>
 #include <utility>
 
 #include "ani_kernels.h"
@@ -518,6 +519,75 @@
   ib = e0.w + b;
 }
 
+struct StreamCur {
+  const unsigned* wp = nullptr;
+  int total = 0;
+  unsigned w0 = 0, w1 = 0;
+  bool on = false;
+};
+__device__ __forceinline__ int stream_tuple(const AevParams& p, const StreamTab& t, int n0, int n1) {
+  if (p.S == 1) return (unsigned)n0 <= (unsigned)t.nt ? n0 : -1;
+  return ((unsigned)n0 <= (unsigned)t.nt && (unsigned)n1 <= (unsigned)t.nt) ? n0 * (t.nt + 1) + n1 : -1;
+}
+template <int STEP>
+__device__ __forceinline__ StreamCur stream_begin(const int4* desc, const unsigned* words, int tix, int lane) {
+  StreamCur c;
+  if (tix < 0) return c;
+  int4 d;
+  asm volatile("s_load_dwordx4 %0, %1, 0x0\n\ts_waitcnt lgkmcnt(0)" : "=s"(d) : "s"(desc + tix) : "memory");
+  c.on = true;
+  c.total = d.y;
+  c.wp = words + d.x;
+  if (d.y > 0) c.w0 = c.wp[lane & (STEP - 1)];
+  if (STEP == 32 && d.y > STEP) c.w1 = c.wp[STEP + (lane & 31)];
+  return c;
+}
+
+template <int NA, int NZ, bool BWD>
+__global__ __launch_bounds__(64) void stream_table_kernel(AevParams p, int nt, int4* desc, unsigned* words, int fill) {
+  __shared__ int s_astart[24];
+  __shared__ int s_tb[kMaxBuckets * 8];
+  constexpr int STEP = BWD ? 32 : 64;
+  const int lane = threadIdx.x, t = blockIdx.x;
+  FastLds L{};
+  L.astart = s_astart;
+  L.tb = s_tb;
+  const int n0 = p.S == 1 ? t : t / (nt + 1), n1 = p.S == 1 ? 0 : t % (nt + 1);
+  if (lane <= p.S) s_astart[lane] = lane == 0 ? 0 : (lane == 1 ? n0 : n0 + n1);
+  wave_sync();
+  int nbk;
+  const int total = BWD ? build_pair_table<NA, NZ>(p, lane, L, nbk) : build_bucket_table<NA, NZ>(p, lane, L, nbk);
+  wave_sync();
+  const int reserved = (total + STEP - 1) / STEP * STEP;
+  if (!fill) {
+    if (lane == 0) desc[t] = make_int4(0, total, nbk, reserved);
+    return;
+  }
+  unsigned* out = words + desc[t].x;
+  for (int v = lane; v < reserved; v += 64) {
+    unsigned w;
+    if constexpr (BWD) {
+      int ia0, ib0, off0, pos0, ia1, ib1, off1, pos1;
+      bool v0, v1;
+      stream_pair_half(L, nbk, v, 0, ia0, ib0, off0, pos0, v0);
+      stream_pair_half(L, nbk, v, 1, ia1, ib1, off1, pos1, v1);
+      int e = 0;
+      for (int k = 1; k < nbk; k++)
+        if (v >= L.tb[8 * k]) e = k;
+      const int tri = L.tb[8 * e + 6], bk = (off0 - p.radial_len) / (NA * NZ);
+      w = (unsigned)ia0 | ((unsigned)ib0 << 8) | ((unsigned)pos0 << 16) | ((unsigned)bk << 24) | ((unsigned)(tri ? 1 : 0) << 29) |
+          ((unsigned)(v0 ? 1 : 0) << 30) | ((unsigned)(v1 ? 1 : 0) << 31);
+    } else {
+      int ia, ib, off;
+      bool valid;
+      stream_pair(L, nbk, v, ia, ib, off, valid);
+      const int bk = (off - p.radial_len) / (NA * NZ);
+      w = (unsigned)ia | ((unsigned)ib << 8) | ((unsigned)bk << 16) | ((unsigned)(valid ? 1 : 0) << 24);
+    }
+    out[v] = w;
+  }
+}
+
 __device__ __forceinline__ void gd_add(double* p, float v) { atomicAdd(p, (double)v); }
 template <int OFF>
 __device__ __forceinline__ float xor_sum(float v) {
@@ -541,22 +611,27 @@
   }
 }
 
-template <int NA, int NZ>
-__device__ __forceinline__ void forward_compute(const AevParams& p, const AevArgs& a, FastLds& L, int row, int lane BWD_STAMP_PARAMS);
-
-template <int NA, int NZ, int NCH>
+template <int NA, int NZ, bool TAB>
+__device__ __forceinline__ void forward_compute(const AevParams& p, const AevArgs& a, FastLds& L, int row, int lane,
+                                                StreamCur sc BWD_STAMP_PARAMS);
+
+template <int NA, int NZ, int NCH, bool TAB>
 __device__ __forceinline__ void forward_centre(const AevParams& p, const AevArgs& a, FastLds& L, int row, const hdr_t& h,
-                                               const Loaded<NCH, false, 1>& pf, int lane BWD_STAMP_PARAMS) {
+                                               const Loaded<NCH, false, 1>& pf, int lane, const StreamTab& tab BWD_STAMP_PARAMS) {
+  StreamCur sc;
+  if constexpr (TAB)
+    sc = stream_begin<64>(tab.desc_f, tab.words_f, stream_tuple(p, tab, h[2] & 0xff, (h[2] >> 8) & 0xff), lane);
   for (int e = lane; e < (p.aev_stride >> 2); e += 64) reinterpret_cast<float4*>(L.row)[e] = make_float4(0, 0, 0, 0);
   int nrad, nang;
   unpack_lists<NCH>(p, a, row, h, pf, lane, L, nrad, nang);
   wave_sync();
   BWD_STAMP(2);
-  forward_compute<NA, NZ>(p, a, L, row, lane BWD_STAMP_ARGS);
-}
-
-template <int NA, int NZ>
-__device__ __forceinline__ void forward_compute(const AevParams& p, const AevArgs& a, FastLds& L, int row, int lane BWD_STAMP_PARAMS) {
+  forward_compute<NA, NZ, TAB>(p, a, L, row, lane, sc BWD_STAMP_ARGS);
+}
+
+template <int NA, int NZ, bool TAB>
+__device__ __forceinline__ void forward_compute(const AevParams& p, const AevArgs& a, FastLds& L, int row, int lane,
+                                                StreamCur sc BWD_STAMP_PARAMS) {
   constexpr int NR = 16, Q = 64 / NA;
 
   {
@@ -584,9 +659,15 @@
   }
 
   BWD_STAMP(3);
-  int nbk;
-  const int total = build_bucket_table<NA, NZ>(p, lane, L, nbk);
-  wave_sync();
+  int nbk = 0, total;
+  bool tabbed = false;
+  if constexpr (TAB) tabbed = sc.on;
+  if (tabbed) {
+    total = sc.total;
+  } else {
+    total = build_bucket_table<NA, NZ>(p, lane, L, nbk);
+    wave_sync();
+  }
   BWD_STAMP(4);
   float acc[NZ];
 #pragma unroll
@@ -629,7 +710,16 @@
     {
       int ia, ib;
       bool valid;
-      stream_pair(L, nbk, base + lane, ia, ib, outoff, valid);
+      if (tabbed) {
+        const unsigned w = sc.w0;
+        if (base + 64 < total) sc.w0 = sc.wp[base + 64 + lane];
+        ia = w & 0xff;
+        ib = (w >> 8) & 0xff;
+        outoff = p.radial_len + (int)((w >> 16) & 0xff) * (NA * NZ);
+        valid = (w >> 24) & 1;
+      } else {
+        stream_pair(L, nbk, base + lane, ia, ib, outoff, valid);
+      }
       const float4 A = L.ad[ia], B = L.ad[ib];
       const float dot = A.x * B.x + A.y * B.y + A.z * B.z;
       const float cth = 0.95f * dot * frcp(fmaxf(A.w * B.w, 1e-10f));
@@ -742,8 +832,17 @@
   }                                                                                                       \
   ANI_TICKETS_END(KW)
 
-template <int NA, int NZ, int NCH>
-__global__ __launch_bounds__(64 * kWaves, kFwdMinWaves) void aev_forward_fast(AevParams p, AevArgs a, int cap, int rowf) {
+template <typename... TBP>
+__device__ __forceinline__ StreamTab tab_of(const TBP&... tbp) {
+  StreamTab t{};
+  if constexpr (sizeof...(TBP) > 0) t = (tbp, ...);
+  return t;
+}
+
+template <int NA, int NZ, int NCH, typename... TBP>
+__global__ __launch_bounds__(64 * kWaves, kFwdMinWaves) void aev_forward_fast(AevParams p, AevArgs a, int cap, int rowf, TBP... tbp) {
+  constexpr bool TAB = sizeof...(TBP) > 0;
+  const StreamTab tab = tab_of(tbp...);
   extern __shared__ float4 smem4[];
   const int wave = __builtin_amdgcn_readfirstlane(threadIdx.x >> 6), lane = threadIdx.x & 63;
   FastLds L = carve<NA, NZ>(reinterpret_cast<float*>(smem4) + wave * fast_wave_floats_row(cap, false, rowf, p.S), cap, false, rowf);
@@ -759,7 +858,7 @@
     Loaded<NCH, false, 1> cur;
     load_lists(p, a, row, hdr_nrad(hc), hdr_nang(hc), lane, cur);
     BWD_STAMP(1);
-    forward_centre<NA, NZ, NCH>(p, a, L, row, hc, cur, lane, stamp_prev, stamp_acc);
+    forward_centre<NA, NZ, NCH, TAB>(p, a, L, row, hc, cur, lane, tab, stamp_prev, stamp_acc);
     stamp_acc[7] += 1;
   }
   if (wave == 0 && lane == 0) {
@@ -767,12 +866,14 @@
     atomicAdd(&g_bwd_stamps[24], stamp_acc[7]);
   }
 #else
-  ANI_PERSISTENT_LOOP(kWaves, NCH, false, 1, (forward_centre<NA, NZ, NCH>(p, a, L, row, hc, cur, lane)))
+  ANI_PERSISTENT_LOOP(kWaves, NCH, false, 1, (forward_centre<NA, NZ, NCH, TAB>(p, a, L, row, hc, cur, lane, tab)))
 #endif
 }
 
-template <int NA, int NZ, int NCHC>
-__global__ __launch_bounds__(64 * kWaves, kFusedMinWaves) void aev_forward_fused(AevParams p, AevArgs a, int cap, int rowf) {
+template <int NA, int NZ, int NCHC, typename... TBP>
+__global__ __launch_bounds__(64 * kWaves, kFusedMinWaves) void aev_forward_fused(AevParams p, AevArgs a, int cap, int rowf, TBP... tbp) {
+  constexpr bool TAB = sizeof...(TBP) > 0;
+  const StreamTab tab = tab_of(tbp...);
   extern __shared__ float4 smem4[];
   const int wave = __builtin_amdgcn_readfirstlane(threadIdx.x >> 6), lane = threadIdx.x & 63;
   FastLds L = carve<NA, NZ>(reinterpret_cast<float*>(smem4) + wave * fast_wave_floats_row(cap, false, rowf, p.S), cap, false, rowf);
@@ -829,6 +930,12 @@
         pos[c] = (in_a && pA < kMaxAng) ? pA : ((in_2 && p2 < cap2) ? kMaxAng + p2 : -1);
       }
     }
+    StreamCur sc;
+    if constexpr (TAB) {
+      const int c0 = __builtin_amdgcn_readlane(cc, 0) & 0xffff, c1 = __builtin_amdgcn_readlane(cc, 1) & 0xffff;
+      const bool live = inf.x >= 0 && !(nA > kMaxAng || nR > cap2 || nA + nR > cap);
+      sc = stream_begin<64>(tab.desc_f, tab.words_f, live ? stream_tuple(p, tab, c0, c1) : -1, lane);
+    }
 #pragma unroll
     for (int c = 0; c < NCHC; c++) touch(jj1[c]);
     ANI_TICKET_TAKE(k2)
@@ -872,9 +979,9 @@
       wave_sync();
 #ifdef ABLB_STAMPS
       unsigned long long stamp_prev = 0, stamp_acc[8] = {0, 0, 0, 0, 0, 0, 0, 0};
-      forward_compute<NA, NZ>(p, a, L, row, lane, stamp_prev, stamp_acc);
+      forward_compute<NA, NZ, TAB>(p, a, L, row, lane, sc, stamp_prev, stamp_acc);
 #else
-      forward_compute<NA, NZ>(p, a, L, row, lane);
+      forward_compute<NA, NZ, TAB>(p, a, L, row, lane, sc);
 #endif
     }
     info = info1;
@@ -903,10 +1010,10 @@
   }
 }
 
-template <int NA, int NZ, int NCH, int GR, bool VIR, bool AV, typename PF>
+template <int NA, int NZ, int NCH, int GR, bool VIR, bool AV, bool TAB, typename PF>
 __device__ __forceinline__ void backward_centre(const AevParams& p, const AevArgs& a, FastLds& L, int row, const hdr_t h,
                                                 const Loaded<NCH, true, GR> pf, int lane, float (&wv)[9],
-                                                const RepTab& rep, float* __restrict__ avir, float* vt, float& er,
+                                                const RepTab& rep, float* __restrict__ avir, float* vt, float& er, StreamCur sc,
                                                 PF&& before_final_scatter BWD_STAMP_PARAMS) {
   constexpr int NR = 16;
   const int centre = h[0];
@@ -1073,15 +1180,34 @@
     }
   }
   BWD_STAMP(2);
-  int nbk;
-  const int total_pairs = build_pair_table<NA, NZ>(p, lane, L, nbk);
-  wave_sync();
+  int nbk = 0, total_pairs;
+  bool tabbed = false;
+  if constexpr (TAB) tabbed = sc.on;
+  if (tabbed) {
+    total_pairs = sc.total;
+  } else {
+    total_pairs = build_pair_table<NA, NZ>(p, lane, L, nbk);
+    wave_sync();
+  }
   BWD_STAMP(3);
   const float cA = -p.EtaA * kLog2e;
   for (int base = 0; base < total_pairs; base += 32) {
     int ia, ib, outoff, pos;
     bool valid;
-    stream_pair_half(L, nbk, base + (lane & 31), lane >> 5, ia, ib, outoff, pos, valid);
+    if (tabbed) {
+      const unsigned w = sc.w0;
+      sc.w0 = sc.w1;
+      if (base + 64 < total_pairs) sc.w1 = sc.wp[base + 64 + (lane & 31)];
+      const int hh = lane >> 5;
+      valid = (w >> (30 + hh)) & 1;
+      const int up = valid ? hh : 0;
+      ia = (int)(w & 0xff) + up;
+      ib = (w >> 8) & 0xff;
+      pos = valid ? (int)((w >> 16) & 0xff) - (int)((w >> 29) & (unsigned)up) : 0;
+      outoff = p.radial_len + (int)((w >> 24) & 0x1f) * (NA * NZ);
+    } else {
+      stream_pair_half(L, nbk, base + (lane & 31), lane >> 5, ia, ib, outoff, pos, valid);
+    }
     const float4 A = L.ad[ia], B = L.ad[ib];
     const float inv_ra = frcp(A.w), inv_rb = frcp(B.w);
     const float inv_rr = inv_ra * inv_rb;
@@ -1183,14 +1309,26 @@
 }
 static_assert((fast_wave_floats(0, true) + 3 * 64) * 4 * kWavesB <= 160 * 1024, "armed backward LDS");
 
+__device__ __forceinline__ void take_extra(StreamTab&, float*&) {}
+template <typename... R>
+__device__ __forceinline__ void take_extra(StreamTab& t, float*& av, float* x, R... r) { av = x; take_extra(t, av, r...); }
+template <typename... R>
+__device__ __forceinline__ void take_extra(StreamTab& t, float*& av, StreamTab x, R... r) { t = x; take_extra(t, av, r...); }
+template <typename T, typename... P> constexpr bool pack_has = (std::is_same<T, P>::value || ...);
+
 template <int NA, int NZ, int NCH, int GR, bool VIR, typename... AVP>
 __global__ __launch_bounds__(64 * kWavesB, kBwdMinWaves) void aev_backward_fast(AevParams p, AevArgs a, int cap, int rowf, RepTab rep,
                                                                                 AVP... avp) {
-  constexpr bool AV = sizeof...(AVP) > 0;
+  constexpr bool AV = pack_has<float*, AVP...>, TAB = pack_has<StreamTab, AVP...>;
   float* avir = nullptr;
-  if constexpr (AV) avir = (avp, ...);
+  StreamTab tab{};
+  take_extra(tab, avir, avp...);
   extern __shared__ float4 smem4[];
   const int wave = __builtin_amdgcn_readfirstlane(threadIdx.x >> 6), lane = threadIdx.x & 63;
+  auto stream_of = [&](const hdr_t& hx) -> StreamCur {
+    if constexpr (TAB) return stream_begin<32>(tab.desc_b, tab.words_b, stream_tuple(p, tab, hx[2] & 0xff, (hx[2] >> 8) & 0xff), lane);
+    else return StreamCur{};
+  };
   float* wbase = reinterpret_cast<float*>(smem4) + wave * bwd_wave_floats(cap, rowf, p.S, AV);
   FastLds L = carve<NA, NZ>(wbase, cap, true, rowf);
   float* vt = AV ? wbase + fast_wave_floats_row(cap, true, rowf, p.S) : nullptr;
@@ -1212,7 +1350,8 @@
 #else
     BWD_STAMP(1);
 #endif
-    backward_centre<NA, NZ, NCH, GR, VIR, AV>(p, a, L, row, hc, cur, lane, wv, rep, avir, vt, er, [] {}, stamp_prev, stamp_acc);
+    backward_centre<NA, NZ, NCH, GR, VIR, AV, TAB>(p, a, L, row, hc, cur, lane, wv, rep, avir, vt, er, stream_of(hc), [] {}, stamp_prev,
+                                                   stamp_acc);
     stamp_acc[6] += 1;
   }
   if (wave == 0 && lane == 0) {
@@ -1230,6 +1369,7 @@
   bool have = false;
   hdr_t hc;
   Loaded<NCH, true, GR> cur;
+  StreamCur sc;
   while (k < kstop) {
     ANI_TICKET_DRAW(tk_tn)
     const int kk = rank_of(k);
@@ -1237,17 +1377,23 @@
     const bool in_range = kk < a.kcount;
     if (!have) {
       hc = load_header_scalar(a, row);
-      if (hc[0] >= 0 && in_range) load_lists(p, a, row, hdr_nrad(hc), hdr_nang(hc), lane, cur);
+      if (hc[0] >= 0 && in_range) {
+        load_lists(p, a, row, hdr_nrad(hc), hdr_nang(hc), lane, cur);
+        sc = stream_of(hc);
+      }
     }
     have = false;
     ANI_TICKET_TAKE(tk_k2)
     if (hc[0] >= 0 && in_range) {
-      backward_centre<NA, NZ, NCH, GR, VIR, AV>(p, a, L, row, hc, cur, lane, wv, rep, avir, vt, er, [&]() {
+      backward_centre<NA, NZ, NCH, GR, VIR, AV, TAB>(p, a, L, row, hc, cur, lane, wv, rep, avir, vt, er, sc, [&]() {
         const int kk1 = rank_of(k1);
         if (k1 < kstop && kk1 < a.kcount) {
           const int row1 = row_of(kk1);
           hc = load_header_scalar(a, row1);
-          if (hc[0] >= 0) load_lists(p, a, row1, hdr_nrad(hc), hdr_nang(hc), lane, cur);
+          if (hc[0] >= 0) {
+            load_lists(p, a, row1, hdr_nrad(hc), hdr_nang(hc), lane, cur);
+            sc = stream_of(hc);
+          }
           have = true;
         }
       });
@@ -1603,7 +1749,25 @@
   else go(nbr_compact_kernel<4>);
 }
 
-void launch_aev_forward(const AevParams& p, const AevArgs& a, int max_numneigh, hipStream_t st) {
+bool stream_tab_supported(const AevParams& p) { return fast_kind(p) != 0 && (p.S == 1 || p.S == 2); }
+
+void launch_stream_table(const AevParams& p, int nt, bool backward, int4* d_desc, unsigned* d_words, int fill, hipStream_t st) {
+  const int n = stream_tab_tuples(p.S, nt);
+  if (n <= 0 || !stream_tab_supported(p)) return;
+  auto go = [&](auto kernel) { hipLaunchKernelGGL(kernel, dim3(n), dim3(64), 0, st, p, nt, d_desc, d_words, fill); };
+  const bool k1 = fast_kind(p) == 1;
+  if (k1 && backward) go(stream_table_kernel<8, 4, true>);
+  else if (k1) go(stream_table_kernel<8, 4, false>);
+  else if (backward) go(stream_table_kernel<4, 8, true>);
+  else go(stream_table_kernel<4, 8, false>);
+}
+
+static const StreamTab* usable_tab(const AevParams& p, const StreamTab* tab) {
+  return (tab && tab->desc_b && tab->desc_f && (p.S == 1 || p.S == 2)) ? tab : nullptr;
+}
+
+void launch_aev_forward(const AevParams& p, const AevArgs& a, int max_numneigh, hipStream_t st, const StreamTab* tab) {
+  tab = usable_tab(p, tab);
   if (a.nrows <= 0) return;
   const dim3 grid((a.nrows + kWaves - 1) / kWaves), block(64 * kWaves);
   if (aev_fast_path(p, max_numneigh)) {
@@ -1612,36 +1776,45 @@
     const int rowf = (p.aev_stride + 63) / 64 * 64;
     const size_t lds = (size_t)fast_wave_floats_row(cap, false, rowf, p.S) * 4 * kWaves;
     const bool k1 = fast_kind(p) == 1, n2 = !p.compat;
-    if (k1 && n2) launch_fast(aev_forward_fast<8, 4, 1>, p, a, kWaves, lds, cap, rowf, st);
-    else if (k1) launch_fast(aev_forward_fast<8, 4, 3>, p, a, kWaves, lds, cap, rowf, st);
-    else if (n2) launch_fast(aev_forward_fast<4, 8, 1>, p, a, kWaves, lds, cap, rowf, st);
-    else launch_fast(aev_forward_fast<4, 8, 3>, p, a, kWaves, lds, cap, rowf, st);
+#define ANI_FWD_CASE(K, ...)                                                                       \
+  do {                                                                                             \
+    if (tab) launch_fast(K<__VA_ARGS__, StreamTab>, p, a, kWaves, lds, cap, rowf, st, *tab);       \
+    else launch_fast(K<__VA_ARGS__>, p, a, kWaves, lds, cap, rowf, st);                            \
+  } while (0)
+    if (k1 && n2) ANI_FWD_CASE(aev_forward_fast, 8, 4, 1);
+    else if (k1) ANI_FWD_CASE(aev_forward_fast, 8, 4, 3);
+    else if (n2) ANI_FWD_CASE(aev_forward_fast, 4, 8, 1);
+    else ANI_FWD_CASE(aev_forward_fast, 4, 8, 3);
   } else {
     hipLaunchKernelGGL(aev_forward_generic, grid, block, 0, st, p, a);
   }
 }
 
-bool launch_aev_forward_fused(const AevParams& p, const AevArgs& a, int max_numneigh, hipStream_t st) {
+bool launch_aev_forward_fused(const AevParams& p, const AevArgs& a, int max_numneigh, hipStream_t st, const StreamTab* tab) {
   if (a.nrows <= 0 || a.kcount <= 0 || !aev_fast_path(p, max_numneigh) || max_numneigh > 256) return false;
+  tab = usable_tab(p, tab);
   const int cap = radial_cap(p, max_numneigh);
   const int rowf = (p.aev_stride + 63) / 64 * 64;
   const size_t lds = (size_t)fast_wave_floats_row(cap, false, rowf, p.S) * 4 * kWaves;
   const bool k1 = fast_kind(p) == 1;
   const int nch = max_numneigh <= 128 ? 2 : (max_numneigh <= 192 ? 3 : 4);
   if (k1) {
-    if (nch == 2) launch_fast(aev_forward_fused<8, 4, 2>, p, a, kWaves, lds, cap, rowf, st);
-    else if (nch == 3) launch_fast(aev_forward_fused<8, 4, 3>, p, a, kWaves, lds, cap, rowf, st);
-    else launch_fast(aev_forward_fused<8, 4, 4>, p, a, kWaves, lds, cap, rowf, st);
+    if (nch == 2) ANI_FWD_CASE(aev_forward_fused, 8, 4, 2);
+    else if (nch == 3) ANI_FWD_CASE(aev_forward_fused, 8, 4, 3);
+    else ANI_FWD_CASE(aev_forward_fused, 8, 4, 4);
   } else {
-    if (nch == 2) launch_fast(aev_forward_fused<4, 8, 2>, p, a, kWaves, lds, cap, rowf, st);
-    else if (nch == 3) launch_fast(aev_forward_fused<4, 8, 3>, p, a, kWaves, lds, cap, rowf, st);
-    else launch_fast(aev_forward_fused<4, 8, 4>, p, a, kWaves, lds, cap, rowf, st);
-  }
+    if (nch == 2) ANI_FWD_CASE(aev_forward_fused, 4, 8, 2);
+    else if (nch == 3) ANI_FWD_CASE(aev_forward_fused, 4, 8, 3);
+    else ANI_FWD_CASE(aev_forward_fused, 4, 8, 4);
+  }
+#undef ANI_FWD_CASE
   return true;
 }
 
-bool launch_aev_backward(const AevParams& p, const AevArgs& a, int max_numneigh, hipStream_t st, const RepTab* rep, float* avir) {
+bool launch_aev_backward(const AevParams& p, const AevArgs& a, int max_numneigh, hipStream_t st, const RepTab* rep, float* avir,
+                         const StreamTab* tab) {
   if (a.nrows <= 0) return true;
+  tab = usable_tab(p, tab);
   RepTab rt{};
   if (rep) rt = *rep;
   const dim3 grid((a.nrows + kWaves - 1) / kWaves), block(64 * kWaves);
@@ -1653,6 +1826,13 @@
     const bool k1 = fast_kind(p) == 1, n2 = !p.compat, g1 = p.aev_stride <= 256;
 #define ANI_BWD_CASE(NA, NZ, NCH, GR)                                                                              \
   do {                                                                                                             \
+    if constexpr (GR == 1 && NCH == 1) {                 \
+      if (tab && !avir) {                                                                                                         \
+        if (a.virial) launch_fast(aev_backward_fast<NA, NZ, NCH, GR, true, StreamTab>, p, a, kWavesB, lds, cap, rowf, st, rt, *tab);   \
+        else launch_fast(aev_backward_fast<NA, NZ, NCH, GR, false, StreamTab>, p, a, kWavesB, lds, cap, rowf, st, rt, *tab);           \
+        break;                                                                                                                    \
+      }                                                                                                                           \
+    }                                                                                                                             \
     if (avir) launch_fast(aev_backward_fast<NA, NZ, NCH, GR, true, float*>, p, a, kWavesB, lds, cap, rowf, st, rt, avir);  \
     else if (a.virial) launch_fast(aev_backward_fast<NA, NZ, NCH, GR, true>, p, a, kWavesB, lds, cap, rowf, st, rt);      \
     else launch_fast(aev_backward_fast<NA, NZ, NCH, GR, false>, p, a, kWavesB, lds, cap, rowf, st, rt);                   \
```

Result: faster. 64.68, median of 6 (+5.4%).
